# bjkomer/pyratslam

Hardware: AMD Instinct MI355X
Metric: pose-cell steps/sec (64×64×36) + template-compares/sec at 1/2/4/8 GPU (higher is better)
Workload: dtype u8; 1 GPU; configs[1]: 64x64x36 pose-cell grid + 1000 stored 64x32 u8 templates per GPU; a step matches 10 batches of 1024 queries resident in HBM; templates_per_gpu=1000, templates_total=1000, queries_per_batch=1024, parallelism=library sharded over 1 GPU(s), none; pose cells replicated

## Files before the change

### include/ratslam_abi.h

```cpp
#ifndef RATSLAM_ABI_H
#define RATSLAM_ABI_H

#include <stddef.h>
#include <stdint.h>

#ifdef __cplusplus
extern "C" {
#endif

#define RS_OK           0
#define RS_ERR_ARG      1
#define RS_ERR_TYPE     2
#define RS_ERR_LUT_KEY  3
#define RS_ERR_HIP      4
#define RS_ERR_RCCL     5
#define RS_ERR_STATE    6
#define RS_ERR_NOMEM    7
#define RS_ERR_CTL_RANGE 8

#define RS_PREC_F32 0
#define RS_PREC_F64 1

#define RS_FILTER_LEN 7

int rs_version(void);
const char* rs_last_error(void);
int rs_device_count(void);
int rs_dev_malloc(int device, size_t bytes, void** ptr);
int rs_dev_free(void* ptr);
int rs_dev_copy(void* dst, const void* src, size_t bytes);
int rs_host_alloc(size_t bytes, void** ptr);
int rs_host_free(void* ptr);

typedef struct rs_pc rs_pc;

typedef struct rs_pc_params {
    int precision;
    double global_inhibition;
    double ge[RS_FILTER_LEN];
    double gi[RS_FILTER_LEN];
    double k_scale;
    int nfilters;
    const double* xy_filters;
} rs_pc_params;


int rs_pc_create(int X, int Y, int TH, const rs_pc_params* params, int device, rs_pc** out);
int rs_pc_destroy(rs_pc* h);
int rs_pc_shape(const rs_pc* h, int* X, int* Y, int* TH);

int rs_pc_update(rs_pc* h, const int32_t* ox, const int32_t* oy, const int32_t* fidx,
                 const double* zf, int32_t out_xyz[3]);
int rs_pc_run(rs_pc* h, int n, const int32_t* ox, const int32_t* oy, const int32_t* fidx,
              const double* zf, int32_t* out_xyz);
int rs_pc_set_odometry_tables(rs_pc* h, double vtrans_scale, double vrot_scale,
                              const double* cos_a, const double* sin_a, int key_min,
                              int nkeys, const int32_t* key_rows, int zorig_min, int nz,
                              const double* zf_table);
int rs_pc_update_odom(rs_pc* h, double vtrans, double vrot, int32_t out_xyz[3]);
int rs_pc_odom_control(int TH, double vtrans_scale, double vrot_scale, const double* cos_a,
                       const double* sin_a, int key_min, int nkeys, const int32_t* key_rows,
                       int zorig_min, int nz, const double* zf_table, int n, const double* odom,
                       int32_t* ox, int32_t* oy, int32_t* fidx, double* zf, int32_t* status);
int rs_pc_run_odom(rs_pc* h, int n, const double* odom, int32_t* out_xyz, int* first_bad);
int rs_pc_update_odom_read(rs_pc* h, double vtrans, double vrot, int32_t out_xyz[3], double* pinned_xyth);
int rs_pc_excite(rs_pc* h);
int rs_pc_inject(rs_pc* h, double energy, int x, int y, int th);
int rs_pc_get_max(rs_pc* h, int32_t out_xyz[3]);
int rs_pc_set_peak_tables(rs_pc* h, int r, const double* sc_x, const double* sc_y, const double* sc_th);
int rs_pc_get_peak(rs_pc* h, int32_t xyz[3], double sums[6]);
int rs_pc_update_odom_peak(rs_pc* h, double vtrans, double vrot, int32_t out_xyz[3], double sums[6]);
int rs_pc_run_odom_peaks(rs_pc* h, int n, const double* odom, int32_t* out_xyz, double* out_sums,
                         int* first_bad);
int rs_pc_run_peaks(rs_pc* h, int n, const int32_t* ox, const int32_t* oy, const int32_t* fidx,
                    const double* zf, int32_t* out_xyz, double* out_sums);
int rs_pc_peak_host(int X, int Y, int TH, int r, const double* volume_xyth, const int32_t xyz[3],
                    const double* sc_x, const double* sc_y, const double* sc_th, double sums[6]);
#define RS_PC_INJ_AT_PEAK (-1)
#define RS_PC_INJ_SAME_AS (-2)
int rs_pc_run_odom_inject(rs_pc* h, int n, const double* odom, int ni, const int32_t* inj_step,
                          const double* inj_energy, const int32_t* inj_loc, int32_t* out_xyz,
                          int32_t* out_inj_xyz, double* out_sums, int* first_bad);
int rs_pc_run_inject(rs_pc* h, int n, const int32_t* ox, const int32_t* oy, const int32_t* fidx,
                     const double* zf, int ni, const int32_t* inj_step, const double* inj_energy,
                     const int32_t* inj_loc, int32_t* out_xyz, int32_t* out_inj_xyz, double* out_sums);
int rs_pc_read(rs_pc* h, double* host_xyth);
int rs_pc_read_pinned(rs_pc* h, double* pinned_xyth);
int rs_pc_write(rs_pc* h, const double* host_xyth);
int rs_pc_total(rs_pc* h, double* total);
int rs_pc_last_ms(rs_pc* h, double* ms);
int rs_pc_set_profiling(rs_pc* h, int enable);
int rs_pc_kernel_ms(rs_pc* h, double ms[2]);
const char* rs_pc_step_form(const rs_pc* h);
#define RS_PC_DBG_POISON      1
#define RS_PC_DBG_SKIP_EXPORT 2
#define RS_PC_DBG_HALO_SETTLE 3
#define RS_PC_DBG_HALO_AMBIG  4
int rs_pc_debug(rs_pc* h, int op);
int rs_pc_debug_value(rs_pc* h, int op, int64_t* value);

typedef struct rs_vt rs_vt;

int rs_vt_create(int H, int W, int max_offset, uint64_t match_threshold, int64_t capacity,
                 int device, rs_vt** out);
#define RS_VT_METRIC_WRAPPED 0
#define RS_VT_METRIC_SAD     1
int rs_vt_create_metric(int H, int W, int max_offset, uint64_t match_threshold, int64_t capacity,
                        int device, int metric, rs_vt** out);
int rs_vt_metric(const rs_vt* h, int* metric);
int rs_vt_destroy(rs_vt* h);
int rs_vt_count(const rs_vt* h, int64_t* count);
int rs_vt_add(rs_vt* h, int n, const uint8_t* templates, int64_t* first_index);
int rs_vt_read(rs_vt* h, int64_t index, uint8_t* out);

#define RS_VT_FROZEN     0
#define RS_VT_SEQUENTIAL 1

int rs_vt_match_batch(rs_vt* h, int nq, const uint8_t* queries, int mode,
                      uint64_t* best_score, int64_t* best_index, uint8_t* is_new);
int rs_vt_match_stream(rs_vt* h, int nb, int nq, const uint8_t* queries, uint64_t* best_score,
                       int64_t* best_index);
int rs_vt_match(rs_vt* h, const uint8_t* query, uint64_t* best_score, int64_t* best_index,
                int* is_new);
int rs_vt_set_subsample(rs_vt* h, int64_t frame_bytes, const int32_t* pixels);
int rs_vt_match_frames(rs_vt* h, int nf, const uint8_t* frames, int mode, uint64_t* best_score,
                       int64_t* best_index, uint8_t* is_new);
int rs_vt_scores(rs_vt* h, int nq, const uint8_t* queries, int64_t t0, int64_t nt,
                 uint64_t* scores);
int rs_vt_offset_profile(rs_vt* h, int nq, const uint8_t* queries, const int64_t* index,
                         uint32_t* profile, int32_t* offset);
int rs_vt_offset_profile_host(int metric, int H, int W, int max_offset, const uint8_t* tpl,
                              const uint8_t* query, uint32_t* profile, int32_t* offset);
int rs_vt_set_normalise(rs_vt* h, int radius, int gain);
int rs_vt_normalise(const rs_vt* h, int* radius, int* gain);
int rs_vt_normalise_host(int H, int W, int radius, int gain, const uint8_t* src, uint8_t* dst);
int rs_vt_scan_local(rs_vt* h, int nq, const uint8_t* queries, uint64_t* local_keys);
int rs_vt_resolve(rs_vt* h, int nq, const uint64_t* global_keys, int mode, uint64_t* best_score,
                  int64_t* best_index, uint8_t* is_new);
int rs_vt_last_ms(rs_vt* h, double* ms);
int rs_vt_set_timing(rs_vt* h, int enable);
const char* rs_vt_scan_form(const rs_vt* h);
int rs_vt_prune_stats(rs_vt* h, int64_t out[4]);
int rs_vt_prune_verified(rs_vt* h, int64_t* out);

int rs_vt_set_threshold(rs_vt* h, double threshold);

#define RS_DT_F32 0
#define RS_DT_F64 1
int rs_sad_scores(int device, int dtype, int H, int W, int max_offset, int64_t nt,
                  const void* templates, int nq, const void* queries, void* scores);

typedef struct rs_vtf rs_vtf;

int rs_vtf_create(int H, int W, int max_offset, int dtype, int64_t capacity, int device,
                  rs_vtf** out);
int rs_vtf_destroy(rs_vtf* h);
int rs_vtf_count(const rs_vtf* h, int64_t* count);
int rs_vtf_add(rs_vtf* h, int n, const void* templates, int64_t* first_index);
int rs_vtf_read(rs_vtf* h, int64_t index, void* out);
int rs_vtf_scores(rs_vtf* h, int nq, const void* queries, int64_t t0, int64_t nt, void* scores);
int rs_vtf_scan(rs_vtf* h, int nq, const void* queries, int want_inbatch, void* best_score,
                int64_t* best_index, void* inbatch);
int rs_vtf_append_staged(rs_vtf* h, int n, const int32_t* which, int64_t* first_index);
int rs_vtf_set_timing(rs_vtf* h, int enable);
int rs_vtf_last_ms(rs_vtf* h, double* ms);
int rs_sad_plan_sum(int dtype, int64_t n, const void* values, void* out);

typedef struct rs_vo rs_vo;

typedef struct rs_vo_params {
    int trans_y0, trans_y1, trans_x0, trans_x1;
    int rot_y0, rot_y1, rot_x0, rot_x1;
    int max_shift;
    double rad_per_column;
    double vtrans_scale;
    double vtrans_max;
} rs_vo_params;

int rs_vo_create(int im_h, int im_w, const rs_vo_params* params, int device, rs_vo** out);
int rs_vo_destroy(rs_vo* h);
int rs_vo_reset(rs_vo* h);
int rs_vo_run(rs_vo* h, int nf, const uint8_t* frames, double* deltas, uint32_t* tables,
              uint32_t* profiles);
int rs_vo_select(int max_shift, int width, int rows, const uint32_t* table, int* shift,
                 double* mindiff);
int rs_vo_set_timing(rs_vo* h, int enable);
int rs_vo_last_ms(rs_vo* h, double ms[2]);

typedef struct rs_em rs_em;

int rs_em_create(int capacity, double correction, int device, rs_em** out);
int rs_em_destroy(rs_em* h);
int rs_em_count(rs_em* h, int* nexp, int* nlinks);
int rs_em_add_experience(rs_em* h, int from, double d, double heading, double facing, int* id);
int rs_em_add_link(rs_em* h, int from, int to, double d, double heading, double facing, int* id);
int rs_em_relax(rs_em* h, int loops);
int rs_em_read(rs_em* h, int first, int n, double* xyth);
int rs_em_write(rs_em* h, int first, int n, const double* xyth);
int rs_em_set_timing(rs_em* h, int enable);
int rs_em_last_ms(rs_em* h, double* ms);
const char* rs_em_form(rs_em* h);
int rs_em_relax_host(int nexp, int nlinks, const int32_t* from, const int32_t* to, const double* d,
                     const double* heading, const double* facing, double* xyth, int loops,
                     double correction);

#define RS_UNIQUE_ID_BYTES 128
int rs_comm_unique_id(uint8_t id[RS_UNIQUE_ID_BYTES]);
int rs_vt_attach_comm(rs_vt* h, int rank, int nranks, const uint8_t id[RS_UNIQUE_ID_BYTES]);
int rs_vt_set_shard(rs_vt* h, int rank, int nranks);
int rs_vt_rank(const rs_vt* h, int* rank, int* nranks);

#ifdef __cplusplus
}
#endif
#endif
```

### pyratslam_amd/_lib.py

```python
import ctypes
import os
import threading

import numpy as np

HERE = os.path.dirname(os.path.abspath(__file__))
LIB_PATH = os.path.join(HERE, 'libratslam_hip.so')

RS_OK = 0
RS_ERR_ARG = 1
RS_ERR_TYPE = 2
RS_ERR_LUT_KEY = 3
RS_ERR_HIP = 4
RS_ERR_RCCL = 5
RS_ERR_STATE = 6
RS_ERR_NOMEM = 7
RS_ERR_CTL_RANGE = 8
RS_PREC_F32 = 0
RS_PREC_F64 = 1
RS_PC_DBG_POISON = 1
RS_PC_DBG_SKIP_EXPORT = 2
RS_PC_DBG_HALO_SETTLE = 3
RS_PC_DBG_HALO_AMBIG = 4
RS_PC_INJ_AT_PEAK = -1
RS_PC_INJ_SAME_AS = -2
RS_VT_FROZEN = 0
RS_VT_SEQUENTIAL = 1
RS_VT_METRIC_WRAPPED = 0
RS_VT_METRIC_SAD = 1
RS_UNIQUE_ID_BYTES = 128
RS_DT_F32 = 0
RS_DT_F64 = 1
FILTER_LEN = 7

_c_int_p = ctypes.POINTER(ctypes.c_int)
_i32p = ctypes.POINTER(ctypes.c_int32)
_i64p = ctypes.POINTER(ctypes.c_int64)
_u64p = ctypes.POINTER(ctypes.c_uint64)
_u32p = ctypes.POINTER(ctypes.c_uint32)
_u8p = ctypes.POINTER(ctypes.c_uint8)
_f64p = ctypes.POINTER(ctypes.c_double)
_vp = ctypes.c_void_p


class PcParams(ctypes.Structure):
    _fields_ = [
        ('precision', ctypes.c_int),
        ('global_inhibition', ctypes.c_double),
        ('ge', ctypes.c_double * FILTER_LEN),
        ('gi', ctypes.c_double * FILTER_LEN),
        ('k_scale', ctypes.c_double),
        ('nfilters', ctypes.c_int),
        ('xy_filters', _f64p),
    ]


class VoParams(ctypes.Structure):
    _fields_ = [(r + '_' + b, ctypes.c_int) for r in ('trans', 'rot') for b in ('y0', 'y1', 'x0', 'x1')] + [
        ('max_shift', ctypes.c_int),
        ('rad_per_column', ctypes.c_double),
        ('vtrans_scale', ctypes.c_double),
        ('vtrans_max', ctypes.c_double),
    ]


SIGNATURES = {
    'rs_version': (ctypes.c_int, []),
    'rs_last_error': (ctypes.c_char_p, []),
    'rs_device_count': (ctypes.c_int, []),
    'rs_dev_malloc': (ctypes.c_int, [ctypes.c_int, ctypes.c_size_t, ctypes.POINTER(_vp)]),
    'rs_dev_free': (ctypes.c_int, [_vp]),
    'rs_dev_copy': (ctypes.c_int, [_vp, _vp, ctypes.c_size_t]),
    'rs_host_alloc': (ctypes.c_int, [ctypes.c_size_t, ctypes.POINTER(_vp)]),
    'rs_host_free': (ctypes.c_int, [_vp]),
    'rs_pc_create': (ctypes.c_int, [ctypes.c_int, ctypes.c_int, ctypes.c_int,
                                    ctypes.POINTER(PcParams), ctypes.c_int, ctypes.POINTER(_vp)]),
    'rs_pc_destroy': (ctypes.c_int, [_vp]),
    'rs_pc_shape': (ctypes.c_int, [_vp, _c_int_p, _c_int_p, _c_int_p]),
    'rs_pc_update': (ctypes.c_int, [_vp, _i32p, _i32p, _i32p, _f64p, _i32p]),
    'rs_pc_run': (ctypes.c_int, [_vp, ctypes.c_int, _i32p, _i32p, _i32p, _f64p, _i32p]),
    'rs_pc_set_odometry_tables': (ctypes.c_int, [_vp, ctypes.c_double, ctypes.c_double, _f64p, _f64p,
                                                 ctypes.c_int, ctypes.c_int, _i32p, ctypes.c_int,
                                                 ctypes.c_int, _f64p]),
    'rs_pc_update_odom': (ctypes.c_int, [_vp, ctypes.c_double, ctypes.c_double, _i32p]),
    'rs_pc_odom_control': (ctypes.c_int, [ctypes.c_int, ctypes.c_double, ctypes.c_double, _f64p,
                                          _f64p, ctypes.c_int, ctypes.c_int, _i32p, ctypes.c_int,
                                          ctypes.c_int, _f64p, ctypes.c_int, _f64p, _i32p, _i32p,
                                          _i32p, _f64p, _i32p]),
    'rs_pc_run_odom': (ctypes.c_int, [_vp, ctypes.c_int, _f64p, _i32p, _c_int_p]),
    'rs_pc_excite': (ctypes.c_int, [_vp]),
    'rs_pc_inject': (ctypes.c_int, [_vp, ctypes.c_double, ctypes.c_int, ctypes.c_int, ctypes.c_int]),
    'rs_pc_get_max': (ctypes.c_int, [_vp, _i32p]),
    'rs_pc_set_peak_tables': (ctypes.c_int, [_vp, ctypes.c_int, _f64p, _f64p, _f64p]),
    'rs_pc_get_peak': (ctypes.c_int, [_vp, _i32p, _f64p]),
    'rs_pc_update_odom_peak': (ctypes.c_int, [_vp, ctypes.c_double, ctypes.c_double, _i32p, _f64p]),
    'rs_pc_run_odom_peaks': (ctypes.c_int, [_vp, ctypes.c_int, _f64p, _i32p, _f64p, _c_int_p]),
    'rs_pc_run_peaks': (ctypes.c_int, [_vp, ctypes.c_int, _i32p, _i32p, _i32p, _f64p, _i32p, _f64p]),
    'rs_pc_run_odom_inject': (ctypes.c_int, [_vp, ctypes.c_int, _f64p, ctypes.c_int, _i32p, _f64p, _i32p, _i32p,
                                             _i32p, _f64p, _c_int_p]),
    'rs_pc_run_inject': (ctypes.c_int, [_vp, ctypes.c_int, _i32p, _i32p, _i32p, _f64p, ctypes.c_int, _i32p, _f64p,
                                        _i32p, _i32p, _i32p, _f64p]),
    'rs_pc_peak_host': (ctypes.c_int, [ctypes.c_int, ctypes.c_int, ctypes.c_int, ctypes.c_int, _f64p, _i32p,
                                       _f64p, _f64p, _f64p, _f64p]),
    'rs_pc_read': (ctypes.c_int, [_vp, _f64p]),
    'rs_pc_read_pinned': (ctypes.c_int, [_vp, _vp]),
    'rs_pc_update_odom_read': (ctypes.c_int, [_vp, ctypes.c_double, ctypes.c_double, _i32p, _vp]),
    'rs_pc_write': (ctypes.c_int, [_vp, _f64p]),
    'rs_pc_total': (ctypes.c_int, [_vp, _f64p]),
    'rs_pc_last_ms': (ctypes.c_int, [_vp, _f64p]),
    'rs_pc_set_profiling': (ctypes.c_int, [_vp, ctypes.c_int]),
    'rs_pc_kernel_ms': (ctypes.c_int, [_vp, _f64p]),
    'rs_pc_step_form': (ctypes.c_char_p, [_vp]),
    'rs_pc_debug': (ctypes.c_int, [_vp, ctypes.c_int]),
    'rs_pc_debug_value': (ctypes.c_int, [_vp, ctypes.c_int, ctypes.POINTER(ctypes.c_int64)]),
    'rs_vt_create': (ctypes.c_int, [ctypes.c_int, ctypes.c_int, ctypes.c_int, ctypes.c_uint64,
                                    ctypes.c_int64, ctypes.c_int, ctypes.POINTER(_vp)]),
    'rs_vt_create_metric': (ctypes.c_int, [ctypes.c_int, ctypes.c_int, ctypes.c_int, ctypes.c_uint64,
                                           ctypes.c_int64, ctypes.c_int, ctypes.c_int, ctypes.POINTER(_vp)]),
    'rs_vt_metric': (ctypes.c_int, [_vp, _c_int_p]),
    'rs_vt_destroy': (ctypes.c_int, [_vp]),
    'rs_vt_count': (ctypes.c_int, [_vp, _i64p]),
    'rs_vt_add': (ctypes.c_int, [_vp, ctypes.c_int, _u8p, _i64p]),
    'rs_vt_read': (ctypes.c_int, [_vp, ctypes.c_int64, _u8p]),
    'rs_vt_match_batch': (ctypes.c_int, [_vp, ctypes.c_int, _u8p, ctypes.c_int, _u64p, _i64p, _u8p]),
    'rs_vt_match_stream': (ctypes.c_int, [_vp, ctypes.c_int, ctypes.c_int, _vp, _u64p, _i64p]),
    'rs_vt_match': (ctypes.c_int, [_vp, _u8p, _u64p, _i64p, _c_int_p]),
    'rs_vt_scores': (ctypes.c_int, [_vp, ctypes.c_int, _u8p, ctypes.c_int64, ctypes.c_int64, _u64p]),
    'rs_vt_offset_profile': (ctypes.c_int, [_vp, ctypes.c_int, _vp, _i64p, _u32p, _i32p]),
    'rs_vt_offset_profile_host': (ctypes.c_int, [ctypes.c_int, ctypes.c_int, ctypes.c_int, ctypes.c_int, _u8p, _u8p,
                                                 _u32p, _i32p]),
    'rs_vt_set_normalise': (ctypes.c_int, [_vp, ctypes.c_int, ctypes.c_int]),
    'rs_vt_normalise': (ctypes.c_int, [_vp, _c_int_p, _c_int_p]),
    'rs_vt_normalise_host': (ctypes.c_int, [ctypes.c_int, ctypes.c_int, ctypes.c_int, ctypes.c_int, _u8p, _u8p]),
    'rs_vt_set_subsample': (ctypes.c_int, [_vp, ctypes.c_int64, _i32p]),
    'rs_vt_match_frames': (ctypes.c_int, [_vp, ctypes.c_int, _vp, ctypes.c_int, _u64p, _i64p, _u8p]),
    'rs_vt_scan_local': (ctypes.c_int, [_vp, ctypes.c_int, _u8p, _u64p]),
    'rs_vt_resolve': (ctypes.c_int, [_vp, ctypes.c_int, _u64p, ctypes.c_int, _u64p, _i64p, _u8p]),
    'rs_vt_last_ms': (ctypes.c_int, [_vp, _f64p]),
    'rs_vt_set_timing': (ctypes.c_int, [_vp, ctypes.c_int]),
    'rs_vt_scan_form': (ctypes.c_char_p, [_vp]),
    'rs_vt_prune_stats': (ctypes.c_int, [_vp, _i64p]),
    'rs_vt_prune_verified': (ctypes.c_int, [_vp, _i64p]),
    'rs_vt_set_threshold': (ctypes.c_int, [_vp, ctypes.c_double]),
    'rs_sad_scores': (ctypes.c_int, [ctypes.c_int, ctypes.c_int, ctypes.c_int, ctypes.c_int,
                                     ctypes.c_int, ctypes.c_int64, _vp, ctypes.c_int, _vp, _vp]),
    'rs_vtf_create': (ctypes.c_int, [ctypes.c_int, ctypes.c_int, ctypes.c_int, ctypes.c_int,
                                     ctypes.c_int64, ctypes.c_int, ctypes.POINTER(_vp)]),
    'rs_vtf_destroy': (ctypes.c_int, [_vp]),
    'rs_vtf_count': (ctypes.c_int, [_vp, _i64p]),
    'rs_vtf_add': (ctypes.c_int, [_vp, ctypes.c_int, _vp, _i64p]),
    'rs_vtf_read': (ctypes.c_int, [_vp, ctypes.c_int64, _vp]),
    'rs_vtf_scores': (ctypes.c_int, [_vp, ctypes.c_int, _vp, ctypes.c_int64, ctypes.c_int64, _vp]),
    'rs_vtf_scan': (ctypes.c_int, [_vp, ctypes.c_int, _vp, ctypes.c_int, _vp, _i64p, _vp]),
    'rs_vtf_append_staged': (ctypes.c_int, [_vp, ctypes.c_int, _i32p, _i64p]),
    'rs_vtf_set_timing': (ctypes.c_int, [_vp, ctypes.c_int]),
    'rs_vtf_last_ms': (ctypes.c_int, [_vp, _f64p]),
    'rs_sad_plan_sum': (ctypes.c_int, [ctypes.c_int, ctypes.c_int64, _vp, _vp]),
    'rs_vo_create': (ctypes.c_int, [ctypes.c_int, ctypes.c_int, ctypes.POINTER(VoParams), ctypes.c_int,
                                    ctypes.POINTER(_vp)]),
    'rs_vo_destroy': (ctypes.c_int, [_vp]),
    'rs_vo_reset': (ctypes.c_int, [_vp]),
    'rs_vo_run': (ctypes.c_int, [_vp, ctypes.c_int, _vp, _f64p, _u32p, _u32p]),
    'rs_vo_select': (ctypes.c_int, [ctypes.c_int, ctypes.c_int, ctypes.c_int, _u32p, _c_int_p, _f64p]),
    'rs_vo_set_timing': (ctypes.c_int, [_vp, ctypes.c_int]),
    'rs_vo_last_ms': (ctypes.c_int, [_vp, _f64p]),
    'rs_em_create': (ctypes.c_int, [ctypes.c_int, ctypes.c_double, ctypes.c_int, ctypes.POINTER(_vp)]),
    'rs_em_destroy': (ctypes.c_int, [_vp]),
    'rs_em_count': (ctypes.c_int, [_vp, _c_int_p, _c_int_p]),
    'rs_em_add_experience': (ctypes.c_int, [_vp, ctypes.c_int, ctypes.c_double, ctypes.c_double,
                                            ctypes.c_double, _c_int_p]),
    'rs_em_add_link': (ctypes.c_int, [_vp, ctypes.c_int, ctypes.c_int, ctypes.c_double, ctypes.c_double,
                                      ctypes.c_double, _c_int_p]),
    'rs_em_relax': (ctypes.c_int, [_vp, ctypes.c_int]),
    'rs_em_read': (ctypes.c_int, [_vp, ctypes.c_int, ctypes.c_int, _f64p]),
    'rs_em_write': (ctypes.c_int, [_vp, ctypes.c_int, ctypes.c_int, _f64p]),
    'rs_em_set_timing': (ctypes.c_int, [_vp, ctypes.c_int]),
    'rs_em_last_ms': (ctypes.c_int, [_vp, _f64p]),
    'rs_em_form': (ctypes.c_char_p, [_vp]),
    'rs_em_relax_host': (ctypes.c_int, [ctypes.c_int, ctypes.c_int, _i32p, _i32p, _f64p, _f64p, _f64p,
                                        _f64p, ctypes.c_int, ctypes.c_double]),
    'rs_comm_unique_id': (ctypes.c_int, [_u8p]),
    'rs_vt_attach_comm': (ctypes.c_int, [_vp, ctypes.c_int, ctypes.c_int, _u8p]),
    'rs_vt_set_shard': (ctypes.c_int, [_vp, ctypes.c_int, ctypes.c_int]),
    'rs_vt_rank': (ctypes.c_int, [_vp, _c_int_p, _c_int_p]),
}

NEWER_SYMBOLS = {'rs_vt_prune_stats', 'rs_vt_prune_verified', 'rs_vt_create_metric', 'rs_vt_metric',
                 'rs_vt_offset_profile', 'rs_vt_offset_profile_host', 'rs_vt_set_normalise',
                 'rs_vt_normalise', 'rs_vt_normalise_host'}

_lib = None
_lock = threading.Lock()


class HipLibraryError(RuntimeError):
    """The HIP library is missing, failed to load, or reported a runtime error."""


def load(path=LIB_PATH):
    global _lib
    with _lock:
        if _lib is not None:
            return _lib
        if not os.path.exists(path):
            raise HipLibraryError(
                f'{path} not found: build it with `python -m pyratslam_amd._build` '
                '(there is no CPU fallback)')
        lib = ctypes.CDLL(path)
        for name, (res, args) in SIGNATURES.items():
            if name in NEWER_SYMBOLS and not hasattr(lib, name):
                continue
            fn = getattr(lib, name)
            fn.restype = res
            fn.argtypes = args
        _lib = lib
        return lib


def check(status):
    if status == RS_OK:
        return
    msg = (_lib.rs_last_error() or b'').decode(errors='replace') if _lib else ''
    if status == RS_ERR_ARG:
        raise ValueError(msg)
    if status == RS_ERR_TYPE:
        raise TypeError(msg)
    if status == RS_ERR_LUT_KEY:
        raise KeyError(msg)
    if status == RS_ERR_NOMEM:
        raise MemoryError(msg)
    raise HipLibraryError(f'rs status {status}: {msg}')


def require_device():
    lib = load()
    n = lib.rs_device_count()
    if n <= 0:
        raise HipLibraryError('no HIP device visible: the pyratslam_amd hot path runs only on '
                              'an AMD GPU (gfx950); there is no CPU fallback')
    return lib


def ptr(a, ctype):
    if a is None:
        return None
    return a.ctypes.data_as(ctypes.POINTER(ctype))


def as_c(a, dtype):
    return np.ascontiguousarray(a, dtype=dtype)


class DeviceBuffer:

    def __init__(self, nbytes, device=0):
        self._lib = require_device()
        p = ctypes.c_void_p()
        check(self._lib.rs_dev_malloc(int(device), int(nbytes), ctypes.byref(p)))
        self.ptr, self.nbytes = p, int(nbytes)

    def upload(self, array):
        import numpy as np
        a = np.ascontiguousarray(array)
        if a.nbytes > self.nbytes:
            raise ValueError('%d bytes do not fit a %d-byte buffer' % (a.nbytes, self.nbytes))
        check(self._lib.rs_dev_copy(self.ptr, ctypes.c_void_p(a.ctypes.data), a.nbytes))
        return self

    def offset(self, byte_offset):
        if not 0 <= byte_offset <= self.nbytes:
            raise ValueError('offset %d outside the %d-byte buffer' % (byte_offset, self.nbytes))
        return DeviceView(self, int(byte_offset))

    def close(self):
        if getattr(self, 'ptr', None) is not None and self.ptr.value:
            self._lib.rs_dev_free(self.ptr)
        self.ptr = None

    def __del__(self):
        try:
            self.close()
        except Exception:
            pass


class DeviceView:

    def __init__(self, base, byte_offset):
        self._base = base
        self.ptr = ctypes.c_void_p(base.ptr.value + byte_offset)
        self.nbytes = base.nbytes - byte_offset
```

### pyratslam_amd/csrc/view_templates.hip

```cpp
#include <hip/hip_runtime.h>
#include <rccl/rccl.h>

#include <algorithm>
#include <climits>
#include <cstdint>
#include <cstdio>
#include <cstdlib>
#include <cstring>
#include <memory>
#include <vector>

#include "rs_common.h"
#include "vt_norm_rule.h"
#include "vt_offset_rule.h"
#include "vt_plan.h"

namespace {

#include "vt_device.h"
#include "vt_store.h"
#include "vt_carry.h"

static_assert(vt_plan::METRIC_WRAPPED == RS_VT_METRIC_WRAPPED && vt_plan::METRIC_SAD == RS_VT_METRIC_SAD,
              "vt_plan.h restates the ABI's metric codes");
#include "vt_sad.h"
static_assert(rs::VTO_METRIC_WRAPPED == RS_VT_METRIC_WRAPPED && rs::VTO_METRIC_SAD == RS_VT_METRIC_SAD,
              "vt_offset_rule.h restates the ABI's metric codes");
#include "vt_offset.h"
#include "vt_norm.h"

#include "vt_planes.h"
#include "vt_plane_scan.h"
#include "vt_prune.h"

}

struct QueryForms {
    uint32_t *qp = nullptr, *qsum = nullptr, *qsj = nullptr, *qc = nullptr;
};

struct rs_vt {
    int H = 0, W = 0, M = 0, WD = 0, HQ = 0;
    double thr = 0.0;
    int device = 0;
    int rank = 0, nranks = 1;
    ncclComm_t comm = nullptr;
    int64_t count = 0;
    int64_t localCap = 0;
    rs::DevBuf<uint4> dLib;
    hipStream_t stream = nullptr;
    int qCap = 0;
    rs::DevBuf<uint8_t> dQraw;
    rs::PinnedBuf<uint8_t> hQraw;
    bool qrawBusy = false;
    rs::DevBuf<uint2> dQf;
    rs::DevBuf<uint32_t> dQsum;
    rs::DevBuf<unsigned long long> dBest;
    rs::PinnedBuf<unsigned long long> hBest;
    bool stagingBusy = false;
    hipStream_t cstream = nullptr;
    hipEvent_t evScan = nullptr, evComm = nullptr;
    hipStream_t ustream = nullptr;
    hipEvent_t evUp[2] = {nullptr, nullptr}, evUsed[2] = {nullptr, nullptr};
    rs::DevBuf<uint8_t> dUp[2];
    size_t upCap = 0;
    rs::DevBuf<uint32_t> dQpStream;
    rs::DevBuf<uint32_t> dQsumStream;
    size_t qpStreamCap = 0;
    rs::DevBuf<unsigned long long> dStream;
    rs::PinnedBuf<unsigned long long> hStream;
    size_t streamCap = 0;
    bool streamClean = false;
    int bestClean = 0;
    int bestPending = 0;
    int idxCap = 0;
    rs::DevBuf<int32_t> dSrc;
    rs::DevBuf<int64_t> dDst;
    rs::PinnedBuf<int32_t> hSrc;
    rs::PinnedBuf<int64_t> hDst;
    int64_t candCap = 0;
    rs::DevBuf<uint4> dCand;
    size_t matCap = 0;
    rs::DevBuf<uint32_t> dMat;
    rs::PinnedBuf<uint32_t> hMat;
    hipEvent_t ev0 = nullptr, ev1 = nullptr;
    bool timing = false;
    bool timedScan = false;
    float lastMs = 0.f;
    int stagedQ = 0;
    bool planar = false;
    int metric = RS_VT_METRIC_WRAPPED;
    rs::DevBuf<uint32_t> dLibP, dLibTs, dCandP, dCandTs;
    rs::DevBuf<uint32_t> dQp, dQsumRaw;
    int planeSlots = 0;
    rs::DevBuf<unsigned> dCtr;
    rs::DevBuf<unsigned> dDone;
    bool keysFolded = false;
    int prune = 0;
    int front = 1;
    int listNb = VT_LIST_NB;
    rs::DevBuf<uint32_t> dQsj;
    rs::DevBuf<uint32_t> dQsjStream;
    rs::DevBuf<uint32_t> dQc;
    rs::DevBuf<uint32_t> dQcStream;
    bool qpFull = true;
    bool qcValid = false;
    rs::DevBuf<uint32_t> dMinLB;
    rs::DevBuf<uint32_t> dSecond;
    rs::DevBuf<int> dList;
    size_t pruneCap = 0;
    rs::DevBuf<int> dTbStar;
    rs::DevBuf<unsigned> dListCnt;
    int listCntCap = 0;
    rs::DevBuf<unsigned long long> dPruneStat;
    int64_t prunePairs = 0;
    int prunePasses = 0;
    int pruneNtb = 0;
    rs::DevBuf<int32_t> dPix;
    int64_t frameBytes = 0;
    rs::DevBuf<uint8_t> dFrames;
    rs::PinnedBuf<uint8_t> hFrames;
    int frameCap = 0;
    rs::DevBuf<uint8_t> dOffQ;
    rs::PinnedBuf<int64_t> hOffIdx;
    rs::PinnedBuf<uint32_t> hOffProfile;
    rs::PinnedBuf<int32_t> hOffOffset;
    int radius = 0, gain = 0;
    rs::DevBuf<uint8_t> dNormRaw;
    rs::DevBuf<uint8_t> dNormStream;
    rs::DevBuf<uint8_t> dOffRaw;
};

namespace {

size_t tblock_bytes(const rs_vt* h) { return (size_t)h->WD * h->HQ * 64 * 16; }
size_t pblock_bytes(const rs_vt* h) { return (size_t)PL_CG * (h->H / 4) * 128 * 16; }
constexpr size_t TS_BLOCK_BYTES = 16 * 64 * sizeof(uint32_t);
int plane_ns(const rs_vt* h) { return h->H - 2 * h->M + 3; }

template <class T>
int vt_realloc_blocks(rs_vt* h, rs::DevBuf<T>& buf, int64_t keep, int64_t blocks, size_t bb,
                      const char* what = "template buffer growth") {
    rs::DevBuf<T> nb;
    const size_t bytes = (size_t)blocks * bb;
    RS_TRY(nb.reserve(bytes / sizeof(T), what));
    RS_HIP(hipMemsetAsync(nb.get(), 0, bytes, h->stream));
    if (buf.get()) {
        if (keep > 0)
            RS_HIP(hipMemcpyAsync(nb.get(), buf.get(), (size_t)keep * bb, hipMemcpyDeviceToDevice, h->stream));
        RS_HIP(hipStreamSynchronize(h->stream));
    }
    buf = std::move(nb);
    return RS_OK;
}

int64_t local_count_of(const rs_vt* h, int64_t global_count) {
    return vt_plan::local_count_of(h->rank, h->nranks, global_count);
}

int vt_grow_lib(rs_vt* h, int64_t need_slots) {
    if (need_slots <= h->localCap) return RS_OK;
    const int64_t cap = (int64_t)rs::round_up((size_t)rs::grown<int64_t>(h->localCap, need_slots, 64), 64);
    RS_TRY(vt_realloc_blocks(h, h->dLib, h->localCap / 64, cap / 64, tblock_bytes(h), "template library growth"));
    if (h->planar) {
        RS_TRY(vt_realloc_blocks(h, h->dLibP, h->localCap / 64, cap / 64, pblock_bytes(h)));
        RS_TRY(vt_realloc_blocks(h, h->dLibTs, h->localCap / 64, cap / 64, TS_BLOCK_BYTES));
    }
    h->localCap = cap;
    return RS_OK;
}

int vt_qraw_idle(rs_vt* h) {
    if (h->qrawBusy) {
        RS_HIP(hipStreamSynchronize(h->stream));
        h->qrawBusy = false;
    }
    return RS_OK;
}

constexpr unsigned VT_FINE = hipHostMallocMapped | hipHostMallocCoherent;

int vt_grow_queries(rs_vt* h, int nq) {
    if (nq <= h->qCap) return RS_OK;
    const int cap = rs::grown(h->qCap, nq, 64);
    RS_TRY(vt_qraw_idle(h));
    h->qCap = 0;
    h->bestClean = h->bestPending = 0;
    const size_t qb = (size_t)h->H * h->W, n = (size_t)cap;
    if (h->planar) {
        RS_TRY(h->dQp.reserve((size_t)PL_CG * plane_ns(h) * 8 * n));
        RS_TRY(h->dQsumRaw.reserve(n));
        if (h->prune) RS_TRY(h->dQsj.reserve((size_t)PF_NU * 16 * n));
        if (h->prune) RS_TRY(h->dQc.reserve((size_t)QC_Q4 * 4 * n));
    }
    RS_TRY(h->dQraw.reserve(qb * n));
    if (h->radius > 0) RS_TRY(h->dNormRaw.reserve(qb * n));
    RS_TRY(h->hQraw.reserve(qb * n, VT_FINE));
    RS_TRY(h->dQf.reserve((size_t)h->WD * h->H * n));
    RS_TRY(h->dQsum.reserve(n));
    RS_TRY(h->dBest.reserve(n));
    RS_TRY(h->hBest.reserve(n, VT_FINE));
    h->qCap = cap;
    return RS_OK;
}

int vt_grow_index(rs_vt* h, int n) {
    if (n <= h->idxCap) return RS_OK;
    const int cap = rs::grown(h->idxCap, n, 64);
    h->idxCap = 0;
    RS_TRY(h->dSrc.reserve((size_t)cap));
    RS_TRY(h->dDst.reserve((size_t)cap));
    RS_TRY(h->hSrc.reserve((size_t)cap, hipHostMallocDefault));
    RS_TRY(h->hDst.reserve((size_t)cap, hipHostMallocDefault));
    h->idxCap = cap;
    return RS_OK;
}

int vt_grow_matrix(rs_vt* h, size_t elems) {
    if (elems <= h->matCap) return RS_OK;
    const size_t cap = rs::grown<size_t>(h->matCap, elems, 4096);
    h->matCap = 0;
    RS_TRY(h->dMat.reserve(cap));
    RS_TRY(h->hMat.reserve(cap, hipHostMallocDefault));
    h->matCap = cap;
    return RS_OK;
}

int vt_grow_cand(rs_vt* h, int64_t slots) {
    if (slots <= h->candCap) return RS_OK;
    const int64_t cap = rs::grown<int64_t>(h->candCap, slots, 64);
    h->candCap = 0;
    RS_TRY(h->dCand.reserve((size_t)(cap / 64) * tblock_bytes(h) / sizeof(uint4)));
    if (h->planar) {
        RS_TRY(vt_realloc_blocks(h, h->dCandP, 0, cap / 64, pblock_bytes(h)));
        RS_TRY(vt_realloc_blocks(h, h->dCandTs, 0, cap / 64, TS_BLOCK_BYTES));
    }
    h->candCap = cap;
    return RS_OK;
}

QueryForms vt_batch_view(const rs_vt* h) {
    return {h->dQp.get(), h->dQsumRaw.get(), h->dQsj.get(), h->dQc.get()};
}

QueryForms vt_stream_view(const rs_vt* h, size_t q0) {
    const size_t qpq = (size_t)PL_CG * plane_ns(h) * 8;
    QueryForms v{h->dQpStream.get() + qpq * q0, h->dQsumStream.get() + q0, nullptr, nullptr};
    if (h->dQsjStream.get()) v.qsj = h->dQsjStream.get() + (size_t)PF_NU * 16 * q0;
    if (h->dQcStream.get()) v.qc = h->dQcStream.get() + (size_t)QC_Q4 * 4 * q0;
    return v;
}

int vt_build_forms(rs_vt* h, const QueryForms& q, int nq);

bool vt_prunes(const rs_vt* h, const QueryForms& q, bool cand, int64_t tb0, int64_t count, int nq) {
    return vt_plan::prunes(h->H, cand, tb0, q.qsj && q.qc, (count + 63) / 64, h->prune, nq);
}
constexpr int VT_QC_THREADS = 128;
uint32_t* vt_compact_for(rs_vt* h, const QueryForms& q, int nq) {
    const int64_t lc = local_count_of(h, h->count);
    const bool compact = h->planar && lc > 0 && vt_prunes(h, q, false, 0, lc, nq);
    h->qpFull = !compact;
    h->qcValid = compact;
    return compact ? q.qc : nullptr;
}

int vt_normalise(rs_vt* h, const uint8_t* src, uint8_t* dst, size_t n) {
    const int tx = (h->W + VTN_T - 1) / VTN_T, ty = (h->H + VTN_T - 1) / VTN_T;
    hipLaunchKernelGGL(vt_normalise_kernel, dim3((unsigned)(tx * ty), (unsigned)std::min<size_t>(n, 65535)),
                       dim3(VTN_THREADS), 0, h->stream, src, dst, (int)n, h->H, h->W, h->radius, h->gain, tx);
    RS_HIP(hipGetLastError());
    return RS_OK;
}

bool vt_zc_env() { static const bool on = rs::env_on("RS_VT_ZC"); return on; }

int vt_stage_queries(rs_vt* h, int nq, const uint8_t* queries) {
    RS_TRY(vt_grow_queries(h, nq));
    RS_TRY(vt_qraw_idle(h));
    const QueryForms q = vt_batch_view(h);
    const size_t qb = (size_t)h->H * h->W * nq;
    if (h->radius > 0) {
        RS_HIP(hipMemcpyAsync(h->dNormRaw.get(), queries, qb, hipMemcpyHostToDevice, h->stream));
        RS_TRY(vt_normalise(h, h->dNormRaw.get(), h->dQraw.get(), (size_t)nq));
        return vt_build_forms(h, q, nq);
    }
    if (vt_plan::stages_in_place(h->planar, nq, vt_zc_env())) {
        std::memcpy(h->hQraw.get(), queries, qb);
        h->qrawBusy = true;
        uint32_t* const qc = vt_compact_for(h, q, nq);
        hipLaunchKernelGGL(vt_qplane_kernel, dim3(nq), dim3(qc ? VT_QC_THREADS : 256), 0, h->stream, h->hQraw.dev(), h->H,
                           h->M, q.qp, q.qsum, h->dQraw.get(), q.qsj, qc);
        RS_HIP(hipGetLastError());
        return RS_OK;
    }
    RS_HIP(hipMemcpyAsync(h->dQraw.get(), queries, qb, hipMemcpyHostToDevice, h->stream));
    return vt_build_forms(h, q, nq);
}

int vt_build_forms(rs_vt* h, const QueryForms& q, int nq, const uint8_t* src) {
    if (h->metric == RS_VT_METRIC_SAD)
        hipLaunchKernelGGL(vt_qform_sad_kernel, dim3(nq), dim3(256), 0, h->stream, src, h->H, h->W, h->WD,
                           reinterpret_cast<uint32_t*>(h->dQf.get()));
    else if (!h->planar)
        hipLaunchKernelGGL(vt_qform_kernel, dim3(nq), dim3(256), 0, h->stream, src, h->H, h->W,
                           h->WD, h->M, h->dQf.get(), h->dQsum.get());
    else {
        uint32_t* const qc = vt_compact_for(h, q, nq);
        hipLaunchKernelGGL(vt_qplane_kernel, dim3(nq), dim3(qc ? VT_QC_THREADS : 256), 0, h->stream, src, h->H,
                           h->M, q.qp, q.qsum, nullptr, q.qsj, qc);
    }
    RS_HIP(hipGetLastError());
    return RS_OK;
}

int vt_build_forms(rs_vt* h, const QueryForms& q, int nq) { return vt_build_forms(h, q, nq, h->dQraw.get()); }

int vt_stage_frames(rs_vt* h, int nf, const uint8_t* frames) {
    RS_CHECK(h->dPix.get(), RS_ERR_STATE, "no subsampling mask: call rs_vt_set_subsample first");
    RS_TRY(vt_grow_queries(h, nf));
    const bool on_device = rs::on_device(frames);
    const uint8_t* src = frames;
    if (!on_device) {
        if (nf > h->frameCap) {
            const int cap = rs::grown(h->frameCap, nf, 16);
            h->frameCap = 0;
            RS_TRY(h->dFrames.reserve((size_t)h->frameBytes * cap));
            RS_TRY(h->hFrames.reserve((size_t)h->frameBytes * cap, hipHostMallocDefault));
            h->frameCap = cap;
        }
        const size_t fb = (size_t)h->frameBytes * nf;
        std::memcpy(h->hFrames.get(), frames, fb);
        RS_HIP(hipMemcpyAsync(h->dFrames.get(), h->hFrames.get(), fb, hipMemcpyHostToDevice, h->stream));
        src = h->dFrames.get();
    }
    hipLaunchKernelGGL(vt_gather_kernel, dim3(nf), dim3(256), 0, h->stream, src,
                       (size_t)h->frameBytes, h->dPix.get(), h->H * h->W,
                       h->radius > 0 ? h->dNormRaw.get() : h->dQraw.get());
    RS_HIP(hipGetLastError());
    if (h->radius > 0) RS_TRY(vt_normalise(h, h->dNormRaw.get(), h->dQraw.get(), (size_t)nf));
    return vt_build_forms(h, vt_batch_view(h), nf);
}

int vt_store(rs_vt* h, bool cand, const uint8_t* d_raw, int n) {
    if (n == 0) return RS_OK;
    uint4* lib = cand ? h->dCand.get() : h->dLib.get();
    RS_HIP(hipMemcpyAsync(h->dSrc.get(), h->hSrc.get(), sizeof(int32_t) * n, hipMemcpyHostToDevice, h->stream));
    RS_HIP(hipMemcpyAsync(h->dDst.get(), h->hDst.get(), sizeof(int64_t) * n, hipMemcpyHostToDevice, h->stream));
    h->stagingBusy = true;
    const int64_t total = (int64_t)n * h->WD * h->HQ;
    const int grid = (int)std::min<int64_t>((total + 255) / 256, 4096);
    hipLaunchKernelGGL(vt_store_kernel, dim3(grid), dim3(256), 0, h->stream, d_raw, h->dSrc.get(),
                       h->dDst.get(), n, lib, h->H, h->W, h->WD, h->HQ);
    if (h->planar)
        hipLaunchKernelGGL(vt_plane_store_kernel, dim3(n), dim3(256), 0, h->stream, d_raw, h->dSrc.get(),
                           h->dDst.get(), h->H, h->M, cand ? h->dCandP.get() : h->dLibP.get(),
                           cand ? h->dCandTs.get() : h->dLibTs.get());
    RS_HIP(hipGetLastError());
    return RS_OK;
}

template <class F>
__attribute__((always_inline)) inline auto vt_by_h(const rs_vt* h, F&& f) {
    return h->H == 64 ? f(rs::Int<64>{}) : f(rs::Int<32>{});
}

int vt_nqc_env() {
    const char* e = std::getenv("RS_VT_NQC");
    return e ? std::max(1, std::atoi(e)) : 0;
}

int vt_env_switch(const char* name, int* out) {
    const char* e = std::getenv(name);
    if (!e || e[0] == 0 || std::strcmp(e, "1") == 0) *out = 1;
    else if (std::strcmp(e, "force") == 0) *out = 2;
    else {
        RS_CHECK(std::strcmp(e, "0") == 0, RS_ERR_ARG, "%s='%s': expected 0, 1 or force", name, e);
        *out = 0;
    }
    return RS_OK;
}

void vt_launch_keys_export(rs_vt* h, unsigned long long* keys, int n, unsigned long long* host, int max_blocks) {
    hipLaunchKernelGGL(vt_keys_export, dim3((unsigned)vt_plan::export_grid(n, max_blocks)), dim3(256), 0, h->stream,
                       keys, n, host);
}

struct PlaneScan {
    dim3 grid;
    const uint4* planes;
    const uint32_t* ts;
    int ntb;
    int64_t count;
    const QueryForms& q;
    int nq, nqc, rank, nranks;
};
template <int H, bool MATRIX, bool LIST>
void vt_launch_plane_scan(rs_vt* h, const PlaneScan& s, const ScanOut& out, const PlaneList& list) {
    hipLaunchKernelGGL((vt_scan_plane_kernel<H, MATRIX, LIST>), s.grid, dim3(64 * PL_CG * PL_SPLIT), 0, h->stream,
                       s.planes, s.ts, s.ntb, s.count, s.q.qp, s.q.qsum, s.nq, s.nqc, h->dCtr.get(), out, s.rank,
                       s.nranks, list);
}

int vt_ensure_prune_buffers(rs_vt* h, int ntb, int nq) {
    const size_t pairs = (size_t)ntb * nq;
    if (pairs > h->pruneCap) {
        const size_t cap = std::max(pairs, 2 * h->pruneCap);
        h->pruneCap = 0;
        RS_TRY(h->dMinLB.reserve(cap));
        RS_TRY(h->dSecond.reserve(cap));
        RS_TRY(h->dList.reserve(2 * cap));
        h->pruneCap = cap;
    }
    RS_TRY(h->dTbStar.reserve((size_t)nq));
    if (ntb > h->listCntCap) {
        const int cap = std::max(ntb, 2 * h->listCntCap);
        h->listCntCap = 0;
        RS_TRY(h->dListCnt.reserve(2 * (size_t)cap + 1));
        RS_HIP(hipMemsetAsync(h->dListCnt.get(), 0, sizeof(unsigned) * (2 * (size_t)cap + 1), h->stream));
        h->listCntCap = cap;
    }
    if (!h->dPruneStat.get()) {
        RS_TRY(h->dPruneStat.reserve(3));
        RS_HIP(hipMemsetAsync(h->dPruneStat.get(), 0, 3 * sizeof(unsigned long long), h->stream));
    }
    return RS_OK;
}

int vt_launch_pruned(rs_vt* h, const PlaneScan& s, const ScanOut& out) {
    const QueryForms& q = s.q;
    const int ntb = s.ntb, nq = s.nq;
    if (!h->qcValid) {
        hipLaunchKernelGGL(vt_qcompact_kernel, dim3((unsigned)nq), dim3(128), 0, h->stream,
                           reinterpret_cast<const uint4*>(q.qp), reinterpret_cast<uint4*>(q.qc));
        h->qcValid = true;
    }
    RS_TRY(vt_ensure_prune_buffers(h, ntb, nq));
    const size_t pairs = (size_t)ntb * nq;
    unsigned* cnt1 = h->dListCnt.get();
    unsigned* cnt2 = h->dListCnt.get() + h->listCntCap;
    unsigned* verified = h->dListCnt.get() + 2 * (size_t)h->listCntCap;
    int* list1 = h->dList.get();
    int* list2 = h->dList.get() + pairs;
    if (h->front == 2 || (h->front == 1 && vt_plan::front_fused(ntb, PF_WAVES * PF_TPW))) {
        const vt_plan::Grid2 fg = vt_plan::front_grid(nq, PF_NB, VT_PF_GRID_CAP);
        hipLaunchKernelGGL(vt_front_kernel, dim3((unsigned)fg.x, (unsigned)fg.y), dim3(64 * PF_WAVES), 0, h->stream,
                           s.planes, ntb, s.count, reinterpret_cast<const uint4*>(q.qc), q.qsj, nq, h->dMinLB.get(),
                           s.ts, reinterpret_cast<uint4*>(q.qp), q.qsum, out.best, s.rank, s.nranks,
                           h->dTbStar.get());
    } else {
        const vt_plan::Grid2 pf = vt_plan::prefilter_grid(ntb, nq, PF_WAVES * PF_TPW, PF_NB, VT_PF_GRID_CAP);
        hipLaunchKernelGGL(vt_prefilter_kernel, dim3((unsigned)pf.x, (unsigned)pf.y), dim3(64 * PF_WAVES), 0,
                           h->stream, s.planes, ntb, s.count, reinterpret_cast<const uint4*>(q.qc), q.qsj, nq,
                           h->dMinLB.get(), h->dSecond.get());
        hipLaunchKernelGGL(vt_prune_verify_kernel, dim3((unsigned)nq), dim3(64), 0, h->stream, h->dMinLB.get(),
                           h->dSecond.get(), ntb, nq, s.planes, s.ts, reinterpret_cast<const uint4*>(q.qc),
                           reinterpret_cast<uint4*>(q.qp), q.qsum, out.best, s.rank, s.nranks, h->dTbStar.get());
    }
    const dim3 lgrid((unsigned)((nq + VT_LIST_T - 1) / VT_LIST_T), (unsigned)ntb);
    hipLaunchKernelGGL(vt_prune_first_kernel, lgrid, dim3(VT_LIST_T), 0, h->stream, nq, h->dTbStar.get(), cnt1,
                       list1, verified, cnt2, ntb);
    ScanOut po = out;
    po.host = nullptr;
    po.done = nullptr;
    const uint32_t fill = (uint32_t)std::min(65535, std::max(1, h->planeSlots / ntb));
    const uint32_t lnb = (uint32_t)h->listNb;
    vt_launch_plane_scan<64, false, true>(h, s, po,
                                          PlaneList{list1, cnt1, nq, (uint32_t)VT_LIST_PER_B1, lnb, 1u, fill});
    hipLaunchKernelGGL(vt_prune_rest_kernel, lgrid, dim3(VT_LIST_T), 0, h->stream, h->dMinLB.get(), nq,
                       h->dTbStar.get(), out.best, cnt2, list2, cnt1, verified, ntb, h->dPruneStat.get());
#ifdef VT_LIST_PER
    const int per2 = VT_LIST_PER;
#else
    const int per2 = vt_plan::list_per(ntb, h->planeSlots);
#endif
    vt_launch_plane_scan<64, false, true>(h, s, po, PlaneList{list2, cnt2, nq, (uint32_t)per2, lnb, 0u, fill});
    if (out.host) vt_launch_keys_export(h, out.best, nq, out.host, vt_plan::VT_EXPORT_BLOCKS);
    RS_HIP(hipGetLastError());
    h->prunePairs = (int64_t)pairs;
    h->prunePasses = 2;
    h->pruneNtb = ntb;
    return RS_OK;
}

template <bool MATRIX>
int vt_launch_plane(rs_vt* h, const QueryForms& q, bool cand, int64_t count, int nq, ScanOut out, int rank,
                    int nranks, int64_t tb0) {
    const int ntb = (int)((count + 63) / 64);
    const int nqc = vt_plan::plane_split(ntb, (nq + PL_NB - 1) / PL_NB, h->planeSlots, vt_nqc_env());
    if (8 * (size_t)ntb > h->dCtr.capacity()) {
        const size_t cap = std::max(8 * (size_t)ntb, 2 * h->dCtr.capacity());
        RS_TRY(h->dCtr.reserve(cap));
        RS_HIP(hipMemsetAsync(h->dCtr.get(), 0, sizeof(unsigned) * cap, h->stream));
    }
    RS_CHECK((int64_t)ntb * nqc < (1ll << 31), RS_ERR_ARG, "scan grid too large");
    const uint4* planes = reinterpret_cast<const uint4*>(
        reinterpret_cast<const uint8_t*>(cand ? h->dCandP.get() : h->dLibP.get()) + (size_t)tb0 * pblock_bytes(h));
    const uint32_t* ts = (cand ? h->dCandTs.get() : h->dLibTs.get()) + (size_t)tb0 * (TS_BLOCK_BYTES / 4);
    const PlaneScan s{dim3((unsigned)(ntb * nqc)), planes, ts, ntb, count, q, nq, nqc, rank, nranks};
    if constexpr (!MATRIX)
        if (vt_prunes(h, q, cand, tb0, count, nq)) return vt_launch_pruned(h, s, out);
    if (!h->qpFull) {
        hipLaunchKernelGGL(vt_qexpand_kernel, dim3((unsigned)nq), dim3(256), 0, h->stream,
                           reinterpret_cast<const uint4*>(q.qc), reinterpret_cast<uint4*>(q.qp));
        h->qpFull = true;
    }
    vt_by_h(h, [&](auto H) { vt_launch_plane_scan<decltype(H)::value, MATRIX, false>(h, s, out, PlaneList{}); });
    RS_HIP(hipGetLastError());
    return RS_OK;
}

template <bool MATRIX>
int vt_launch_sad(rs_vt* h, const uint4* lib, int ntb, int64_t count, int nq, ScanOut out, int rank, int nranks) {
    const uint32_t* qd = reinterpret_cast<const uint32_t*>(h->dQf.get());
    if (vt_plan::sad_fast(h->H, h->M)) {
        const int nqc = vt_plan::sad_split(ntb, (nq + SAD_NQ - 1) / SAD_NQ);
        RS_CHECK((int64_t)ntb * nqc < (1ll << 31), RS_ERR_ARG, "scan grid too large (%d x %d)", ntb, nqc);
        vt_by_h(h, [&](auto H) {
            hipLaunchKernelGGL((vt_scan_sad_kernel<decltype(H)::value, MATRIX>), dim3((unsigned)(ntb * nqc)),
                               dim3(64 * vt_plan::sad_waves(h->WD)), 0, h->stream, lib, ntb, count, h->WD, qd, nq,
                               nqc, out, rank, nranks);
        });
    } else {
        hipLaunchKernelGGL((vt_scan_sad_generic_kernel<MATRIX>), dim3((unsigned)(ntb * nq)), dim3(64), 0, h->stream,
                           lib, ntb, count, h->H, h->M, h->WD, qd, nq, out, rank, nranks);
    }
    RS_HIP(hipGetLastError());
    return RS_OK;
}

template <bool MATRIX>
int vt_launch_scan(rs_vt* h, const QueryForms& q, bool cand, int64_t count, int nq, ScanOut out, int rank,
                   int nranks, int64_t tb0 = 0) {
    if (count <= 0 || nq <= 0) return RS_OK;
    if (h->planar) return vt_launch_plane<MATRIX>(h, q, cand, count, nq, out, rank, nranks, tb0);
    const uint4* lib = (cand ? h->dCand.get() : h->dLib.get()) + (size_t)tb0 * h->WD * h->HQ * 64;
    const int ntb = (int)((count + 63) / 64);
    const bool fast = h->M == FAST_M && (h->H == 64 || h->H == 32);
    RS_CHECK((int64_t)ntb * nq < (1ll << 31), RS_ERR_ARG, "scan grid too large (%d x %d)", ntb, nq);
    if (h->metric == RS_VT_METRIC_SAD) return vt_launch_sad<MATRIX>(h, lib, ntb, count, nq, out, rank, nranks);
    if (fast && !MATRIX && (int64_t)ntb * nq < 2048 && h->WD <= 8) {
        const dim3 grid((unsigned)((count + 7) / 8), nq);
        vt_by_h(h, [&](auto H) {
            hipLaunchKernelGGL((vt_scan_carry_col_kernel<decltype(H)::value, 1>), grid, dim3(64), 0, h->stream, lib,
                               count, h->WD, h->dQf.get(), h->dQsum.get(), nq, out, rank, nranks);
        });
    } else if (fast) {
        constexpr int NQ = 2;
        const int nqg = (nq + NQ - 1) / NQ;
        const dim3 grid((unsigned)(ntb * ((nqg + 7) / 8) * 8));
        vt_by_h(h, [&](auto H) {
            hipLaunchKernelGGL((vt_scan_carry_kernel<decltype(H)::value, NQ, MATRIX>), grid, dim3(64), 0, h->stream,
                               lib, ntb, count, h->WD, h->dQf.get(), h->dQsum.get(), nq, out, rank, nranks);
        });
    } else {
        hipLaunchKernelGGL((vt_scan_generic_kernel<MATRIX>), dim3((unsigned)(ntb * nq)), dim3(64),
                           0, h->stream, lib, ntb, count, h->H, h->M, h->WD, h->dQf.get(), nq, out, rank,
                           nranks);
    }
    RS_HIP(hipGetLastError());
    return RS_OK;
}

constexpr unsigned long long KEY_PENDING = 0xFFFFFFFF00000000ull;
bool vt_poll_env() { static const bool on = rs::env_on("RS_VT_POLL"); return on; }
bool vt_poll_keys(const unsigned long long* w_, int n) {
    const volatile unsigned long long* w = w_;
    return rs::spin_until(n, [w](int i) { return w[i] != KEY_PENDING; });
}

int vt_staging_idle(rs_vt* h) {
    if (h->stagingBusy) {
        RS_HIP(hipStreamSynchronize(h->stream));
        h->stagingBusy = false;
    }
    return RS_OK;
}

int vt_allreduce_min(rs_vt* h, unsigned long long* buf, size_t n, hipStream_t stream) {
    ncclResult_t r = ncclAllReduce(buf, buf, n, ncclUint64, ncclMin, h->comm, stream);
    RS_CHECK(r == ncclSuccess, RS_ERR_RCCL, "ncclAllReduce(min) failed: %s", ncclGetErrorString(r));
    return RS_OK;
}

template <class Run>
int vt_timed_scan(rs_vt* h, bool timed, Run run) {
    if (timed) RS_HIP(hipEventRecord(h->ev0, h->stream));
    RS_TRY(run());
    if (timed) RS_HIP(hipEventRecord(h->ev1, h->stream));
    h->timedScan = timed;
    return RS_OK;
}

void vt_decode_keys(const unsigned long long* key, size_t n, uint64_t* best_score, int64_t* best_index) {
    for (size_t i = 0; i < n; ++i) {
        const unsigned long long k = key[i];
        if (best_index) best_index[i] = k == NO_KEY ? -1 : (int64_t)(k & 0xFFFFFFFFull);
        if (best_score) best_score[i] = k == NO_KEY ? UINT64_MAX : (k >> 32);
    }
}

int vt_append_staged(rs_vt* h, const std::vector<std::pair<int, int64_t>>& news) {
    int mine = 0;
    RS_TRY(vt_staging_idle(h));
    RS_TRY(vt_grow_index(h, (int)news.size() + 1));
    const int64_t new_count = h->count + (int64_t)news.size();
    RS_TRY(vt_grow_lib(h, local_count_of(h, new_count)));
    for (const auto& p : news) {
        if (p.second % h->nranks != h->rank) continue;
        h->hSrc.get()[mine] = p.first;
        h->hDst.get()[mine] = p.second / h->nranks;
        ++mine;
    }
    RS_TRY(vt_store(h, false, h->dQraw.get(), mine));
    h->count = new_count;
    return RS_OK;
}

int vt_scan_local_impl(rs_vt* h, int nq, const uint8_t* queries, bool frames = false, bool fold_ok = true) {
    RS_CHECK(h, RS_ERR_STATE, "null view-template handle");
    RS_CHECK(nq >= 0, RS_ERR_ARG, "negative query count");
    if (nq == 0) return RS_OK;
    RS_HIP(hipSetDevice(h->device));
    if (frames) {
        RS_CHECK(queries, RS_ERR_ARG, "null frames");
        RS_TRY(vt_stage_frames(h, nq, queries));
    } else if (queries) {
        RS_TRY(vt_stage_queries(h, nq, queries));
    } else {
        RS_CHECK(nq == h->stagedQ, RS_ERR_STATE, "no staged batch of %d queries (have %d)", nq,
                 h->stagedQ);
    }
    if (h->bestClean < nq) {
        RS_HIP(hipMemsetAsync(h->dBest.get(), 0xFF, sizeof(unsigned long long) * nq, h->stream));
        h->bestClean = nq;
    }
    h->bestPending = h->bestClean;
    h->bestClean = 0;
    const int64_t lc = local_count_of(h, h->count);
    ScanOut out{h->dBest.get(), nullptr, 0};
    h->keysFolded = vt_plan::folds_keys(fold_ok, h->planar, lc, vt_poll_env(), h->timing, nq);
    if (h->keysFolded) {
        if (!h->dDone.get()) {
            RS_TRY(h->dDone.reserve(1));
            RS_HIP(hipMemsetAsync(h->dDone.get(), 0, sizeof(unsigned), h->stream));
        }
        for (int i = 0; i < nq; ++i) h->hBest.get()[i] = KEY_PENDING;
        out.host = h->hBest.dev();
        out.done = h->dDone.get();
    }
    RS_TRY(vt_timed_scan(h, h->timing, [&] {
        return vt_launch_scan<false>(h, vt_batch_view(h), false, lc, nq, out, h->rank, h->nranks);
    }));
    h->stagedQ = nq;
    return RS_OK;
}

int vt_resolve_impl(rs_vt* h, int nq, const unsigned long long* keys, int mode,
                    uint64_t* best_score, int64_t* best_index, uint8_t* is_new) {
    RS_CHECK(h, RS_ERR_STATE, "null view-template handle");
    RS_CHECK(mode == RS_VT_FROZEN || mode == RS_VT_SEQUENTIAL, RS_ERR_ARG, "unknown mode %d", mode);
    RS_CHECK(nq == h->stagedQ, RS_ERR_STATE, "resolve of %d queries, %d staged", nq, h->stagedQ);
    if (nq == 0) return RS_OK;
    RS_CHECK(keys, RS_ERR_ARG, "null keys");
    RS_HIP(hipSetDevice(h->device));
    std::vector<unsigned long long> key(keys, keys + nq);
    if (mode == RS_VT_FROZEN) {
        if (is_new) std::memset(is_new, 0, (size_t)nq);
        vt_decode_keys(key.data(), (size_t)nq, best_score, best_index);
        return RS_OK;
    }
    std::vector<int> cand;
    for (int i = 0; i < nq; ++i)
        if (key[i] == NO_KEY || (double)(key[i] >> 32) > h->thr) cand.push_back(i);
    std::vector<int> cpos(nq, -1);
    int64_t ldm = 0;
    if (!cand.empty() && cand.front() < nq - 1) {
        RS_TRY(vt_staging_idle(h));
        const int64_t C = (int64_t)cand.size();
        RS_TRY(vt_grow_cand(h, (int64_t)rs::round_up((size_t)C, 64)));
        RS_TRY(vt_grow_index(h, (int)C));
        for (int64_t j = 0; j < C; ++j) {
            h->hSrc.get()[j] = cand[j];
            h->hDst.get()[j] = j;
            cpos[cand[j]] = (int)j;
        }
        RS_TRY(vt_store(h, true, h->dQraw.get(), (int)C));
        ldm = (int64_t)rs::round_up((size_t)C, 64);
        RS_TRY(vt_grow_matrix(h, (size_t)ldm * nq));
        ScanOut mo{nullptr, h->dMat.get(), ldm};
        RS_TRY(vt_launch_scan<true>(h, vt_batch_view(h), true, C, nq, mo, 0, 1));
        RS_HIP(hipMemcpyAsync(h->hMat.get(), h->dMat.get(), sizeof(uint32_t) * ldm * nq, hipMemcpyDeviceToHost,
                              h->stream));
        RS_HIP(hipStreamSynchronize(h->stream));
        h->stagingBusy = false;
    }
    std::vector<std::pair<int, int64_t>> news;
    for (int i = 0; i < nq; ++i) {
        unsigned long long k = key[i];
        for (size_t a = 0; a < news.size(); ++a) {
            const int j = news[a].first;
            const unsigned long long kj =
                ((unsigned long long)h->hMat.get()[(size_t)i * ldm + cpos[j]] << 32) |
                (unsigned long long)news[a].second;
            k = kj < k ? kj : k;
        }
        if (k == NO_KEY || (double)(k >> 32) > h->thr) {
            const int64_t g = h->count + (int64_t)news.size();
            news.emplace_back(i, g);
            if (is_new) is_new[i] = 1;
            if (best_index) best_index[i] = g;
        } else {
            if (is_new) is_new[i] = 0;
            if (best_index) best_index[i] = (int64_t)(k & 0xFFFFFFFFull);
        }
        if (best_score) best_score[i] = k == NO_KEY ? UINT64_MAX : (k >> 32);
    }
    RS_TRY(vt_append_staged(h, news));
    return RS_OK;
}

int vt_fetch_keys(rs_vt* h, int nq, bool allreduce) {
    if (allreduce && h->nranks > 1) {
        RS_CHECK(h->comm, RS_ERR_STATE, "sharded handle without a communicator: use "
                 "rs_vt_scan_local + an external min-reduction + rs_vt_resolve");
        RS_TRY(vt_allreduce_min(h, h->dBest.get(), (size_t)nq, h->stream));
    }
    const bool poll = vt_plan::polls_keys(vt_poll_env(), h->timedScan, nq);
    if (h->keysFolded) {
        h->keysFolded = false;
    } else {
        if (poll)
            for (int i = 0; i < nq; ++i) h->hBest.get()[i] = KEY_PENDING;
        vt_launch_keys_export(h, h->dBest.get(), nq, h->hBest.dev(), vt_plan::VT_EXPORT_BLOCKS);
        RS_HIP(hipGetLastError());
    }
    if (!(poll && vt_poll_keys(h->hBest.get(), nq))) {
        RS_HIP(hipStreamSynchronize(h->stream));
        h->stagingBusy = false;
    }
    h->qrawBusy = false;
    h->bestClean = h->bestPending;
    if (h->timedScan) RS_HIP(hipEventElapsedTime(&h->lastMs, h->ev0, h->ev1));
    return RS_OK;
}


int vt_grow_stream_forms(rs_vt* h, size_t total) {
    if (total <= h->qpStreamCap) return RS_OK;
    h->qpStreamCap = 0;
    RS_TRY(h->dQpStream.reserve((size_t)PL_CG * plane_ns(h) * 8 * total));
    RS_TRY(h->dQsumStream.reserve(total));
    if (h->prune) RS_TRY(h->dQsjStream.reserve((size_t)PF_NU * 16 * total));
    if (h->prune) RS_TRY(h->dQcStream.reserve((size_t)QC_Q4 * 4 * total));
    h->qpStreamCap = total;
    return RS_OK;
}

int vt_stream_fused(rs_vt* h, size_t total, const uint8_t* queries, int64_t lc) {
    RS_TRY(vt_grow_stream_forms(h, total));
    const QueryForms q = vt_stream_view(h, 0);
    if (h->radius > 0) {
        RS_TRY(h->dNormStream.reserve((size_t)h->H * h->W * total));
        RS_TRY(vt_normalise(h, queries, h->dNormStream.get(), total));
        queries = h->dNormStream.get();
    }
    RS_TRY(vt_build_forms(h, q, (int)total, queries));
    const ScanOut out{h->dStream.get(), nullptr, 0};
    RS_TRY(vt_timed_scan(h, h->timing, [&] {
        return vt_launch_scan<false>(h, q, false, lc, (int)total, out, h->rank, h->nranks);
    }));
    if (h->comm) RS_TRY(vt_allreduce_min(h, h->dStream.get(), total, h->stream));
    return RS_OK;
}

int vt_stream_host_groups(rs_vt* h, int nb, int nq, const uint8_t* queries, int64_t lc) {
    const size_t total = (size_t)nb * nq, qb = (size_t)h->H * h->W * nq;
    RS_TRY(vt_grow_stream_forms(h, total));
    const vt_plan::HostGroups plan = vt_plan::host_groups(nb);
    if (h->radius > 0) RS_TRY(h->dNormStream.reserve(qb * nb));
    if (!h->ustream) {
        RS_HIP(hipStreamCreateWithFlags(&h->ustream, hipStreamNonBlocking));
        for (int i = 0; i < 2; ++i) {
            RS_HIP(hipEventCreateWithFlags(&h->evUp[i], hipEventDisableTiming));
            RS_HIP(hipEventCreateWithFlags(&h->evUsed[i], hipEventDisableTiming));
        }
    }
    if (qb * plan.gb > h->upCap) {
        RS_HIP(hipStreamSynchronize(h->ustream));
        h->upCap = 0;
        for (int i = 0; i < 2; ++i) RS_TRY(h->dUp[i].reserve(qb * plan.gb));
        h->upCap = qb * plan.gb;
    }
    for (int g = 0;; ++g) {
        const vt_plan::HostGroup grp = plan.group(g);
        if (grp.n == 0) break;
        const int bi = grp.buf;
        if (grp.waits) RS_HIP(hipStreamWaitEvent(h->ustream, h->evUsed[bi], 0));
        RS_HIP(hipMemcpyAsync(h->dUp[bi].get(), queries + qb * grp.b0, qb * grp.n, hipMemcpyHostToDevice, h->ustream));
        RS_HIP(hipEventRecord(h->evUp[bi], h->ustream));
        RS_HIP(hipStreamWaitEvent(h->stream, h->evUp[bi], 0));
        const QueryForms q = vt_stream_view(h, (size_t)grp.b0 * nq);
        const uint8_t* src = h->dUp[bi].get();
        if (h->radius > 0) {
            uint8_t* const dn = h->dNormStream.get() + qb * grp.b0;
            RS_TRY(vt_normalise(h, src, dn, (size_t)grp.n * nq));
            src = dn;
        }
        RS_TRY(vt_build_forms(h, q, grp.n * nq, src));
        RS_HIP(hipEventRecord(h->evUsed[bi], h->stream));
        const ScanOut out{h->dStream.get() + (size_t)grp.b0 * nq, nullptr, 0};
        RS_TRY(vt_launch_scan<false>(h, q, false, lc, grp.n * nq, out, h->rank, h->nranks));
    }
    if (h->comm) RS_TRY(vt_allreduce_min(h, h->dStream.get(), total, h->stream));
    return RS_OK;
}

int vt_stream_per_batch(rs_vt* h, int nb, int nq, const uint8_t* queries, bool on_device, int64_t lc) {
    const size_t qb = (size_t)h->H * h->W * nq;
    for (int b = 0; b < nb; ++b) {
        unsigned long long* keys = h->dStream.get() + (size_t)b * nq;
        const ScanOut out{keys, nullptr, 0};
        const uint8_t* src = queries + qb * b;
        if (!on_device) {
            uint8_t* const up = h->radius > 0 ? h->dNormRaw.get() : h->dQraw.get();
            RS_HIP(hipMemcpyAsync(up, src, qb, hipMemcpyHostToDevice, h->stream));
            src = up;
        }
        if (h->radius > 0) {
            RS_TRY(vt_normalise(h, src, h->dQraw.get(), (size_t)nq));
            src = h->dQraw.get();
        }
        RS_TRY(vt_build_forms(h, vt_batch_view(h), nq, src));
        RS_TRY(vt_launch_scan<false>(h, vt_batch_view(h), false, lc, nq, out, h->rank, h->nranks));
        if (h->comm) {
            RS_HIP(hipEventRecord(h->evScan, h->stream));
            RS_HIP(hipStreamWaitEvent(h->cstream, h->evScan, 0));
            RS_TRY(vt_allreduce_min(h, keys, (size_t)nq, h->cstream));
        }
    }
    if (h->comm) {
        RS_HIP(hipEventRecord(h->evComm, h->cstream));
        RS_HIP(hipStreamWaitEvent(h->stream, h->evComm, 0));
    }
    return RS_OK;
}

int vt_match_stream_impl(rs_vt* h, int nb, int nq, const uint8_t* queries, uint64_t* best_score,
                         int64_t* best_index) {
    RS_CHECK(h, RS_ERR_STATE, "null view-template handle");
    RS_CHECK(nb >= 0 && nq >= 0, RS_ERR_ARG, "negative batch or query count");
    if (nb == 0 || nq == 0) return RS_OK;
    RS_CHECK(queries, RS_ERR_ARG, "null queries");
    RS_CHECK(h->nranks == 1 || h->comm, RS_ERR_STATE, "sharded handle without a communicator: "
             "rs_vt_match_stream needs the RCCL reduction (rs_vt_attach_comm)");
    if (h->comm && !h->cstream) {
        RS_HIP(hipStreamCreateWithFlags(&h->cstream, hipStreamNonBlocking));
        RS_HIP(hipEventCreateWithFlags(&h->evScan, hipEventDisableTiming));
        RS_HIP(hipEventCreateWithFlags(&h->evComm, hipEventDisableTiming));
    }
    RS_HIP(hipSetDevice(h->device));
    RS_TRY(vt_grow_queries(h, nq));
    const size_t total = (size_t)nb * nq;
    RS_CHECK(total <= INT32_MAX, RS_ERR_ARG, "too many queries in one stream");
    if (total > h->streamCap) {
        h->streamCap = 0;
        RS_TRY(h->hStream.reserve(total, hipHostMallocDefault));
        RS_TRY(h->dStream.reserve(total));
        h->streamCap = total;
        h->streamClean = false;
    }
    const bool on_device = rs::on_device(queries);
    RS_CHECK(!on_device || reinterpret_cast<uintptr_t>(queries) % 8 == 0, RS_ERR_ARG,
             "device-resident queries must be 8-byte aligned");
    if (!h->streamClean)
        RS_HIP(hipMemsetAsync(h->dStream.get(), 0xFF, sizeof(unsigned long long) * h->streamCap, h->stream));
    h->streamClean = false;
    h->stagedQ = 0;
    h->timedScan = false;
    const int64_t lc = local_count_of(h, h->count);
    switch (vt_plan::stream_path(on_device, h->planar, nb)) {
    case vt_plan::StreamPath::Fused: RS_TRY(vt_stream_fused(h, total, queries, lc)); break;
    case vt_plan::StreamPath::HostGroups: RS_TRY(vt_stream_host_groups(h, nb, nq, queries, lc)); break;
    case vt_plan::StreamPath::PerBatch: RS_TRY(vt_stream_per_batch(h, nb, nq, queries, on_device, lc)); break;
    }
    vt_launch_keys_export(h, h->dStream.get(), (int)total, h->hStream.dev(), vt_plan::VT_EXPORT_BLOCKS_STREAM);
    RS_HIP(hipGetLastError());
    RS_HIP(hipStreamSynchronize(h->stream));
    h->streamClean = true;
    if (h->timedScan) RS_HIP(hipEventElapsedTime(&h->lastMs, h->ev0, h->ev1));
    vt_decode_keys(h->hStream.get(), total, best_score, best_index);
    return RS_OK;
}

int vt_match_impl(rs_vt* h, int nq, const uint8_t* queries, int mode, uint64_t* best_score,
                  int64_t* best_index, uint8_t* is_new, bool frames = false) {
    RS_CHECK(mode == RS_VT_FROZEN || mode == RS_VT_SEQUENTIAL, RS_ERR_ARG, "unknown mode %d", mode);
    RS_TRY(vt_scan_local_impl(h, nq, queries, frames, h->nranks == 1));
    if (nq == 0) return RS_OK;
    RS_TRY(vt_fetch_keys(h, nq, true));
    return vt_resolve_impl(h, nq, h->hBest.get(), mode, best_score, best_index, is_new);
}

}

extern "C" {

int rs_vt_create(int H, int W, int max_offset, uint64_t thr, int64_t capacity, int device,
                 rs_vt** out) {
    return rs_vt_create_metric(H, W, max_offset, thr, capacity, device, RS_VT_METRIC_WRAPPED, out);
}

int rs_vt_create_metric(int H, int W, int max_offset, uint64_t thr, int64_t capacity, int device,
                        int metric, rs_vt** out) {
    rs::clear_error();
    RS_CHECK(out, RS_ERR_ARG, "null output handle pointer");
    *out = nullptr;
    RS_CHECK(vt_plan::metric_known(metric), RS_ERR_ARG, "unknown metric %d: expected RS_VT_METRIC_WRAPPED or "
             "RS_VT_METRIC_SAD", metric);
    RS_CHECK(H > 0 && W > 0 && H <= 4096 && W <= 4096, RS_ERR_ARG, "bad template shape (%d, %d)", H, W);
    RS_CHECK(max_offset >= 1 && max_offset <= 64, RS_ERR_ARG, "max_offset %d outside [1, 64]", max_offset);
    RS_CHECK(capacity >= 0, RS_ERR_ARG, "negative capacity");
    RS_CHECK((uint64_t)H * W * 255u < 0xFFFFFFFFull, RS_ERR_ARG, "template too large");
    int ndev = 0;
    RS_HIP(hipGetDeviceCount(&ndev));
    RS_CHECK(device >= 0 && device < ndev, RS_ERR_ARG, "device %d not in [0, %d)", device, ndev);
    RS_HIP(hipSetDevice(device));
    std::unique_ptr<rs_vt, int (*)(rs_vt*)> owner(new rs_vt(), rs_vt_destroy);
    rs_vt* const h = owner.get();
    h->H = H; h->W = W; h->M = max_offset; h->thr = (double)thr; h->device = device;
    h->WD = (W + 3) / 4;
    h->HQ = (H + 3) / 4;
    h->metric = metric;
    const bool wrapped = metric == RS_VT_METRIC_WRAPPED;
    h->planar = wrapped && W == 8 * PL_CG && (H == 64 || H == 32) && max_offset == FAST_M;
    if (const char* e = wrapped ? std::getenv("RS_VT_SCAN") : nullptr) {
        if (std::strcmp(e, "carry") == 0) h->planar = false;
        else RS_CHECK(std::strcmp(e, "plane") == 0 || e[0] == 0, RS_ERR_ARG, "RS_VT_SCAN='%s': expected plane or carry", e);
    }
    if (h->planar && h->H == 64) {
        RS_TRY(vt_env_switch("RS_VT_PRUNE", &h->prune));
        RS_TRY(vt_env_switch("RS_VT_FRONT", &h->front));
        if (const char* nb = std::getenv("RS_VT_LIST_NB"); nb && nb[0]) {
            RS_CHECK((nb[0] == '1' || nb[0] == '2' || nb[0] == '4') && nb[1] == 0, RS_ERR_ARG,
                     "RS_VT_LIST_NB='%s': expected 1, 2 or 4", nb);
            h->listNb = nb[0] - '0';
        }
    }
    if (h->planar) {
        int per_cu = 0, cus = 0;
        hipFuncAttributes fa{};
        const void* fn = vt_by_h(h, [](auto H) {
            return reinterpret_cast<const void*>(vt_scan_plane_kernel<decltype(H)::value, false>);
        });
        hipError_t oe = hipOccupancyMaxActiveBlocksPerMultiprocessor(&per_cu, fn, 64 * PL_CG * PL_SPLIT, 0);
        if (oe == hipSuccess) oe = hipFuncGetAttributes(&fa, fn);
        if (oe == hipSuccess) oe = hipDeviceGetAttribute(&cus, hipDeviceAttributeMultiprocessorCount, device);
        RS_CHECK(oe == hipSuccess, RS_ERR_HIP, "occupancy query failed: %s", hipGetErrorString(oe));
        const int vg = std::max(8, (fa.numRegs + 7) / 8 * 8);
        const int by_vgpr = (512 / vg) * 4 / (PL_CG * PL_SPLIT);
        const int by_lds = fa.sharedSizeBytes > 0 ? (int)(160 * 1024 / fa.sharedSizeBytes) : per_cu;
        const int api = per_cu;
        per_cu = std::max(1, std::min({api, by_vgpr, by_lds}));
        h->planeSlots = std::max(1, per_cu * cus);
    }
    hipError_t e = hipStreamCreateWithFlags(&h->stream, hipStreamNonBlocking);
    if (e == hipSuccess) e = hipEventCreate(&h->ev0);
    if (e == hipSuccess) e = hipEventCreate(&h->ev1);
    RS_CHECK(e == hipSuccess, RS_ERR_HIP, "stream/event creation failed: %s", hipGetErrorString(e));
    RS_TRY(vt_grow_lib(h, capacity > 0 ? capacity : 64));
    RS_TRY(vt_grow_queries(h, 64));
    RS_TRY(vt_grow_index(h, 64));
    *out = owner.release();
    return RS_OK;
}

int rs_vt_destroy(rs_vt* h) {
    if (!h) return RS_OK;
    (void)hipSetDevice(h->device);
    hipError_t se = hipSuccess;
    for (hipStream_t st : {h->stream, h->cstream, h->ustream})
        if (st) {
            const hipError_t e = hipStreamSynchronize(st);
            if (se == hipSuccess) se = e;
        }
    if (h->comm) (void)ncclCommDestroy(h->comm);
    if (h->ev0) (void)hipEventDestroy(h->ev0);
    if (h->ev1) (void)hipEventDestroy(h->ev1);
    if (h->evScan) (void)hipEventDestroy(h->evScan);
    if (h->evComm) (void)hipEventDestroy(h->evComm);
    if (h->cstream) (void)hipStreamDestroy(h->cstream);
    for (int i = 0; i < 2; ++i) {
        if (h->evUp[i]) (void)hipEventDestroy(h->evUp[i]);
        if (h->evUsed[i]) (void)hipEventDestroy(h->evUsed[i]);
    }
    if (h->ustream) (void)hipStreamDestroy(h->ustream);
    if (h->stream) (void)hipStreamDestroy(h->stream);
    delete h;
    RS_CHECK(se == hipSuccess, RS_ERR_HIP, "work queued before rs_vt_destroy failed: %s", hipGetErrorString(se));
    return RS_OK;
}

int rs_vt_count(const rs_vt* h, int64_t* count) {
    RS_CHECK(h && count, RS_ERR_ARG, "null argument");
    *count = h->count;
    return RS_OK;
}

int rs_vt_add(rs_vt* h, int n, const uint8_t* templates, int64_t* first_index) {
    rs::clear_error();
    RS_CHECK(h, RS_ERR_STATE, "null view-template handle");
    RS_CHECK(n >= 0 && (n == 0 || templates), RS_ERR_ARG, "bad template batch");
    RS_HIP(hipSetDevice(h->device));
    if (first_index) *first_index = h->count;
    if (n == 0) return RS_OK;
    RS_TRY(vt_grow_queries(h, n));
    const size_t qb = (size_t)h->H * h->W * n;
    hipPointerAttribute_t attr{};
    const bool direct_dma = hipPointerGetAttributes(&attr, templates) == hipSuccess &&
                            (attr.type == hipMemoryTypeHost || attr.type == hipMemoryTypeDevice ||
                             attr.type == hipMemoryTypeManaged);
    (void)hipGetLastError();
    RS_HIP(hipMemcpyAsync(h->radius > 0 ? h->dNormRaw.get() : h->dQraw.get(), templates, qb,
                          attr.type == hipMemoryTypeDevice && direct_dma ? hipMemcpyDeviceToDevice
                                                                         : hipMemcpyHostToDevice,
                          h->stream));
    int s = h->radius > 0 ? vt_normalise(h, h->dNormRaw.get(), h->dQraw.get(), (size_t)n) : RS_OK;
    h->stagedQ = 0;
    std::vector<std::pair<int, int64_t>> news;
    news.reserve(n);
    for (int i = 0; i < n; ++i) news.emplace_back(i, h->count + i);
    if (s == RS_OK) s = vt_append_staged(h, news);
    if (direct_dma) {
        const hipError_t e = hipStreamSynchronize(h->stream);
        RS_CHECK(s != RS_OK || e == hipSuccess, RS_ERR_HIP, "hipStreamSynchronize failed: %s", hipGetErrorString(e));
    }
    return s;
}

int rs_vt_read(rs_vt* h, int64_t index, uint8_t* out) {
    rs::clear_error();
    RS_CHECK(h && out, RS_ERR_ARG, "null argument");
    RS_CHECK(index >= 0 && index < h->count, RS_ERR_ARG, "template index %lld outside [0, %lld)",
             (long long)index, (long long)h->count);
    RS_CHECK(index % h->nranks == h->rank, RS_ERR_ARG, "template %lld lives on rank %lld",
             (long long)index, (long long)(index % h->nranks));
    RS_HIP(hipSetDevice(h->device));
    const int64_t slot = index / h->nranks;
    const int64_t tb = slot >> 6, tl = slot & 63;
    std::vector<uint4> chunks((size_t)h->WD * h->HQ);
    for (int c = 0; c < h->WD; ++c)
        for (int q = 0; q < h->HQ; ++q)
            RS_HIP(hipMemcpyAsync(&chunks[(size_t)c * h->HQ + q],
                                  h->dLib.get() + ((tb * h->WD + c) * h->HQ + q) * 64 + tl, sizeof(uint4),
                                  hipMemcpyDeviceToHost, h->stream));
    RS_HIP(hipStreamSynchronize(h->stream));
    for (int r = 0; r < h->H; ++r)
        for (int col = 0; col < h->W; ++col) {
            const uint4& ch = chunks[(size_t)(col / 4) * h->HQ + r / 4];
            const uint32_t w[4] = {ch.x, ch.y, ch.z, ch.w};
            out[(size_t)r * h->W + col] = (uint8_t)(w[r & 3] >> (8 * (col & 3)));
        }
    return RS_OK;
}

int rs_vt_match_batch(rs_vt* h, int nq, const uint8_t* queries, int mode, uint64_t* best_score,
                      int64_t* best_index, uint8_t* is_new) {
    rs::clear_error();
    return vt_match_impl(h, nq, queries, mode, best_score, best_index, is_new);
}

int rs_vt_match_stream(rs_vt* h, int nb, int nq, const uint8_t* queries, uint64_t* best_score,
                       int64_t* best_index) {
    rs::clear_error();
    return vt_match_stream_impl(h, nb, nq, queries, best_score, best_index);
}

int rs_vt_match(rs_vt* h, const uint8_t* query, uint64_t* best_score, int64_t* best_index,
                int* is_new) {
    rs::clear_error();
    uint8_t nw = 0;
    const int s = vt_match_impl(h, 1, query, RS_VT_SEQUENTIAL, best_score, best_index, &nw);
    if (is_new) *is_new = nw;
    return s;
}

int rs_vt_set_subsample(rs_vt* h, int64_t frame_bytes, const int32_t* pixels) {
    rs::clear_error();
    RS_CHECK(h && pixels, RS_ERR_ARG, "null argument");
    RS_CHECK(frame_bytes > 0 && frame_bytes <= INT32_MAX, RS_ERR_ARG, "bad frame size %lld",
             (long long)frame_bytes);
    const int npix = h->H * h->W;
    for (int i = 0; i < npix; ++i)
        RS_CHECK(pixels[i] >= 0 && pixels[i] < frame_bytes, RS_ERR_ARG,
                 "pixel offset %d of entry %d outside the %lld-byte frame", pixels[i], i,
                 (long long)frame_bytes);
    RS_HIP(hipSetDevice(h->device));
    RS_TRY(h->dPix.reserve((size_t)npix));
    RS_HIP(hipMemcpyAsync(h->dPix.get(), pixels, sizeof(int32_t) * npix, hipMemcpyHostToDevice, h->stream));
    RS_HIP(hipStreamSynchronize(h->stream));
    if (frame_bytes != h->frameBytes) {
        h->frameCap = 0;
        h->dFrames.reset();
        h->hFrames.reset();
    }
    h->frameBytes = frame_bytes;
    return RS_OK;
}

int rs_vt_match_frames(rs_vt* h, int nf, const uint8_t* frames, int mode, uint64_t* best_score,
                       int64_t* best_index, uint8_t* is_new) {
    rs::clear_error();
    RS_CHECK(h, RS_ERR_STATE, "null view-template handle");
    return vt_match_impl(h, nf, frames, mode, best_score, best_index, is_new, true);
}

int rs_vt_scan_local(rs_vt* h, int nq, const uint8_t* queries, uint64_t* local_keys) {
    rs::clear_error();
    RS_TRY(vt_scan_local_impl(h, nq, queries));
    if (nq == 0) return RS_OK;
    RS_TRY(vt_fetch_keys(h, nq, false));
    if (local_keys) std::memcpy(local_keys, h->hBest.get(), sizeof(uint64_t) * nq);
    return RS_OK;
}

int rs_vt_resolve(rs_vt* h, int nq, const uint64_t* global_keys, int mode, uint64_t* best_score,
                  int64_t* best_index, uint8_t* is_new) {
    rs::clear_error();
    static_assert(sizeof(uint64_t) == sizeof(unsigned long long), "key width");
    return vt_resolve_impl(h, nq, reinterpret_cast<const unsigned long long*>(global_keys), mode,
                           best_score, best_index, is_new);
}

int rs_vt_set_shard(rs_vt* h, int rank, int nranks) {
    rs::clear_error();
    RS_CHECK(h, RS_ERR_STATE, "null view-template handle");
    RS_CHECK(nranks >= 1 && rank >= 0 && rank < nranks, RS_ERR_ARG, "bad rank %d of %d", rank, nranks);
    RS_CHECK(h->count == 0 && h->comm == nullptr, RS_ERR_STATE,
             "set the shard before adding templates, once");
    h->rank = rank;
    h->nranks = nranks;
    return RS_OK;
}

int rs_vt_set_normalise(rs_vt* h, int radius, int gain) {
    rs::clear_error();
    RS_CHECK(h, RS_ERR_STATE, "null view-template handle");
    RS_CHECK(radius >= 0 && radius <= rs::VTN_MAX_RADIUS, RS_ERR_ARG, "radius %d outside [0, %d]", radius,
             rs::VTN_MAX_RADIUS);
    RS_CHECK(radius == 0 || (gain >= 1 && gain <= rs::VTN_MAX_GAIN), RS_ERR_ARG, "gain %d outside [1, %d]", gain,
             rs::VTN_MAX_GAIN);
    RS_CHECK(h->count == 0 && h->stagedQ == 0, RS_ERR_STATE,
             "set the normalisation before adding templates or staging a batch");
    RS_HIP(hipSetDevice(h->device));
    if (radius > 0) {
        RS_TRY(h->dNormRaw.reserve((size_t)h->H * h->W * h->qCap));
    } else {
        RS_HIP(hipStreamSynchronize(h->stream));
        h->dNormRaw.reset();
        h->dNormStream.reset();
        h->dOffRaw.reset();
    }
    h->radius = radius;
    h->gain = radius > 0 ? gain : 0;
    return RS_OK;
}

int rs_vt_normalise(const rs_vt* h, int* radius, int* gain) {
    RS_CHECK(h, RS_ERR_STATE, "null view-template handle");
    if (radius) *radius = h->radius;
    if (gain) *gain = h->gain;
    return RS_OK;
}

int rs_vt_normalise_host(int H, int W, int radius, int gain, const uint8_t* src, uint8_t* dst) {
    rs::clear_error();
    RS_CHECK(H > 0 && W > 0 && H <= 4096 && W <= 4096, RS_ERR_ARG, "bad image shape (%d, %d)", H, W);
    RS_CHECK(radius >= 1 && radius <= rs::VTN_MAX_RADIUS, RS_ERR_ARG, "radius %d outside [1, %d]", radius,
             rs::VTN_MAX_RADIUS);
    RS_CHECK(gain >= 1 && gain <= rs::VTN_MAX_GAIN, RS_ERR_ARG, "gain %d outside [1, %d]", gain, rs::VTN_MAX_GAIN);
    RS_CHECK(src && dst && src != dst, RS_ERR_ARG, "null or aliased image");
    rs::vtn_normalise_host(H, W, radius, gain, src, dst);
    return RS_OK;
}

int rs_vt_rank(const rs_vt* h, int* rank, int* nranks) {
    RS_CHECK(h, RS_ERR_STATE, "null view-template handle");
    if (rank) *rank = h->rank;
    if (nranks) *nranks = h->nranks;
    return RS_OK;
}

int rs_vt_scores(rs_vt* h, int nq, const uint8_t* queries, int64_t t0, int64_t nt,
                 uint64_t* scores) {
    rs::clear_error();
    RS_CHECK(h, RS_ERR_STATE, "null view-template handle");
    RS_CHECK(h->nranks == 1, RS_ERR_STATE, "rs_vt_scores needs an unsharded library");
    RS_CHECK(nq >= 0 && t0 >= 0 && nt >= 0 && t0 + nt <= h->count, RS_ERR_ARG,
             "template range [%lld, %lld) outside [0, %lld)", (long long)t0,
             (long long)(t0 + nt), (long long)h->count);
    if (nq == 0 || nt == 0) return RS_OK;
    RS_CHECK(queries && scores, RS_ERR_ARG, "null argument");
    RS_HIP(hipSetDevice(h->device));
    RS_TRY(vt_stage_queries(h, nq, queries));
    h->stagedQ = 0;
    const int64_t tb0 = t0 / 64, lo = t0 - tb0 * 64, span = lo + nt;
    const int64_t ld = (int64_t)rs::round_up((size_t)span, 64);
    RS_TRY(vt_grow_matrix(h, (size_t)ld * nq));
    ScanOut mo{nullptr, h->dMat.get(), ld};
    RS_TRY(vt_timed_scan(h, true, [&] {
        return vt_launch_scan<true>(h, vt_batch_view(h), false, span, nq, mo, 0, 1, tb0);
    }));
    RS_HIP(hipMemcpy2DAsync(h->hMat.get(), sizeof(uint32_t) * nt, h->dMat.get() + lo, sizeof(uint32_t) * ld,
                            sizeof(uint32_t) * nt, nq, hipMemcpyDeviceToHost, h->stream));
    RS_HIP(hipStreamSynchronize(h->stream));
    RS_HIP(hipEventElapsedTime(&h->lastMs, h->ev0, h->ev1));
    for (size_t i = 0; i < (size_t)nq * nt; ++i) scores[i] = h->hMat.get()[i];
    return RS_OK;
}

int rs_vt_offset_profile(rs_vt* h, int nq, const uint8_t* queries, const int64_t* index, uint32_t* profile,
                         int32_t* offset) {
    rs::clear_error();
    RS_CHECK(h, RS_ERR_STATE, "null view-template handle");
    RS_CHECK(h->nranks == 1, RS_ERR_STATE, "rs_vt_offset_profile needs an unsharded library");
    RS_CHECK(nq >= 0, RS_ERR_ARG, "negative query count");
    if (nq == 0) return RS_OK;
    RS_CHECK(index && offset, RS_ERR_ARG, "null argument");
    for (int i = 0; i < nq; ++i)
        RS_CHECK(index[i] >= -1 && index[i] < h->count, RS_ERR_ARG,
                 "template index %lld of query %d outside [-1, %lld)", (long long)index[i], i,
                 (long long)h->count);
    RS_CHECK(queries || nq == h->stagedQ, RS_ERR_STATE, "no staged batch of %d queries (have %d)", nq,
             h->stagedQ);
    RS_HIP(hipSetDevice(h->device));
    const size_t n = (size_t)nq, no = (size_t)(2 * h->M - 1), qb = (size_t)h->H * h->W * n;
    RS_TRY(h->hOffIdx.reserve(rs::grown<size_t>(h->hOffIdx.capacity(), n, 64), VT_FINE));
    RS_TRY(h->hOffProfile.reserve(rs::grown<size_t>(h->hOffProfile.capacity(), n * no, 64 * no), VT_FINE));
    RS_TRY(h->hOffOffset.reserve(rs::grown<size_t>(h->hOffOffset.capacity(), n, 64), VT_FINE));
    const uint8_t* src = h->dQraw.get();
    const size_t offq = rs::grown<size_t>(h->dOffQ.capacity(), qb, 64 * (size_t)h->H * h->W);
    if (queries && h->radius > 0) {
        RS_TRY(h->dOffQ.reserve(offq));
        const uint8_t* raw = queries;
        if (!rs::on_device(queries)) {
            RS_TRY(h->dOffRaw.reserve(h->dOffQ.capacity()));
            RS_HIP(hipMemcpyAsync(h->dOffRaw.get(), queries, qb, hipMemcpyHostToDevice, h->stream));
            raw = h->dOffRaw.get();
        }
        RS_TRY(vt_normalise(h, raw, h->dOffQ.get(), n));
        src = h->dOffQ.get();
    } else if (queries && rs::on_device(queries)) {
        src = queries;
    } else if (queries) {
        RS_TRY(h->dOffQ.reserve(offq));
        RS_HIP(hipMemcpyAsync(h->dOffQ.get(), queries, qb, hipMemcpyHostToDevice, h->stream));
        src = h->dOffQ.get();
    }
    std::memcpy(h->hOffIdx.get(), index, sizeof(int64_t) * n);
    const bool sad = h->metric == RS_VT_METRIC_SAD, fast = h->M == FAST_M;
    auto launch = [&](auto kernel) {
        hipLaunchKernelGGL(kernel, dim3(nq), dim3(64), 0, h->stream, h->dLib.get(), h->count, h->H, h->W,
                           h->WD, h->HQ, h->M, src, h->hOffIdx.dev(), h->hOffProfile.dev(),
                           h->hOffOffset.dev());
    };
    if (sad && fast) launch(vt_offset_profile_kernel<rs::VTO_METRIC_SAD, true>);
    else if (sad) launch(vt_offset_profile_kernel<rs::VTO_METRIC_SAD, false>);
    else if (fast) launch(vt_offset_profile_kernel<rs::VTO_METRIC_WRAPPED, true>);
    else launch(vt_offset_profile_kernel<rs::VTO_METRIC_WRAPPED, false>);
    RS_HIP(hipGetLastError());
    RS_HIP(hipStreamSynchronize(h->stream));
    h->stagingBusy = false;
    h->qrawBusy = false;
    if (profile) std::memcpy(profile, h->hOffProfile.get(), sizeof(uint32_t) * n * no);
    std::memcpy(offset, h->hOffOffset.get(), sizeof(int32_t) * n);
    return RS_OK;
}

int rs_vt_offset_profile_host(int metric, int H, int W, int max_offset, const uint8_t* tpl, const uint8_t* query,
                              uint32_t* profile, int32_t* offset) {
    rs::clear_error();
    RS_CHECK(vt_plan::metric_known(metric), RS_ERR_ARG, "unknown metric %d", metric);
    RS_CHECK(H > 0 && W > 0 && max_offset >= 1 && H >= 2 * max_offset, RS_ERR_ARG,
             "bad shape (%d, %d) for max_offset %d", H, W, max_offset);
    RS_CHECK((uint64_t)H * W * 255u < 0xFFFFFFFFull, RS_ERR_ARG, "template too large");
    RS_CHECK(tpl && query && profile && offset, RS_ERR_ARG, "null argument");
    *offset = rs::vto_profile_host(metric, H, W, max_offset, tpl, query, profile);
    return RS_OK;
}

int rs_vt_set_threshold(rs_vt* h, double threshold) {
    rs::clear_error();
    RS_CHECK(h, RS_ERR_STATE, "null view-template handle");
    h->thr = threshold;
    return RS_OK;
}

int rs_vt_metric(const rs_vt* h, int* metric) {
    RS_CHECK(h && metric, RS_ERR_ARG, "null argument");
    *metric = h->metric;
    return RS_OK;
}

const char* rs_vt_scan_form(const rs_vt* h) {
    if (!h) return nullptr;
    if (h->metric == RS_VT_METRIC_SAD) return vt_plan::sad_form(h->H, h->M);
    if (h->planar) return h->prune ? "plane-pruned" : "plane";
    if (h->M != FAST_M || (h->H != 64 && h->H != 32)) return "generic";
    return "carry";
}

int rs_vt_prune_stats(rs_vt* h, int64_t out[4]) {
    rs::clear_error();
    RS_CHECK(h && out, RS_ERR_ARG, "null argument");
    out[0] = out[1] = out[2] = out[3] = 0;
    if (h->prunePasses == 0) return RS_OK;
    RS_HIP(hipSetDevice(h->device));
    unsigned long long s0 = 0ull;
    std::vector<unsigned> c2((size_t)h->pruneNtb);
    RS_HIP(hipMemcpyAsync(&s0, h->dPruneStat.get(), sizeof(s0), hipMemcpyDeviceToHost, h->stream));
    RS_HIP(hipMemcpyAsync(c2.data(), h->dListCnt.get() + h->listCntCap, sizeof(unsigned) * c2.size(), hipMemcpyDeviceToHost,
                          h->stream));
    RS_HIP(hipStreamSynchronize(h->stream));
    out[0] = (int64_t)s0;
    for (const unsigned c : c2) out[1] += (int64_t)c;
    out[2] = h->prunePairs;
    out[3] = h->prunePasses;
    return RS_OK;
}

int rs_vt_prune_verified(rs_vt* h, int64_t* out) {
    rs::clear_error();
    RS_CHECK(h && out, RS_ERR_ARG, "null argument");
    *out = 0;
    if (h->prunePasses == 0) return RS_OK;
    RS_HIP(hipSetDevice(h->device));
    unsigned long long v = 0ull;
    RS_HIP(hipMemcpyAsync(&v, h->dPruneStat.get() + 2, sizeof(v), hipMemcpyDeviceToHost, h->stream));
    RS_HIP(hipStreamSynchronize(h->stream));
    *out = (int64_t)v;
    return RS_OK;
}

int rs_vt_last_ms(rs_vt* h, double* ms) {
    RS_CHECK(h && ms, RS_ERR_ARG, "null argument");
    *ms = h->timedScan ? h->lastMs : -1.0;
    return RS_OK;
}

int rs_vt_set_timing(rs_vt* h, int enable) {
    rs::clear_error();
    RS_CHECK(h, RS_ERR_STATE, "null view-template handle");
    h->timing = enable != 0;
    return RS_OK;
}

int rs_comm_unique_id(uint8_t id[RS_UNIQUE_ID_BYTES]) {
    rs::clear_error();
    RS_CHECK(id, RS_ERR_ARG, "null id buffer");
    static_assert(sizeof(ncclUniqueId) == RS_UNIQUE_ID_BYTES, "ncclUniqueId size");
    ncclUniqueId u;
    ncclResult_t r = ncclGetUniqueId(&u);
    RS_CHECK(r == ncclSuccess, RS_ERR_RCCL, "ncclGetUniqueId failed: %s", ncclGetErrorString(r));
    std::memcpy(id, &u, sizeof(u));
    return RS_OK;
}

int rs_vt_attach_comm(rs_vt* h, int rank, int nranks, const uint8_t id[RS_UNIQUE_ID_BYTES]) {
    rs::clear_error();
    RS_CHECK(h && id, RS_ERR_ARG, "null argument");
    RS_CHECK(nranks >= 1 && rank >= 0 && rank < nranks, RS_ERR_ARG, "bad rank %d of %d", rank, nranks);
    RS_CHECK(h->count == 0 && h->comm == nullptr, RS_ERR_STATE,
             "attach the communicator before adding templates, once");
    RS_HIP(hipSetDevice(h->device));
    {
        ncclUniqueId u;
        std::memcpy(&u, id, sizeof(u));
        ncclComm_t comm = nullptr;
        ncclResult_t r = ncclCommInitRank(&comm, nranks, u, rank);
        RS_CHECK(r == ncclSuccess, RS_ERR_RCCL, "ncclCommInitRank failed: %s", ncclGetErrorString(r));
        h->comm = comm;
    }
    h->rank = rank;
    h->nranks = nranks;
    return RS_OK;
}

}
```

### pyratslam_amd/csrc/vt_plan.h

```cpp
#pragma once

#include <algorithm>
#include <cstdint>

namespace vt_plan {

inline int64_t local_count_of(int rank, int nranks, int64_t global_count) {
    if (global_count <= rank) return 0;
    return (global_count - rank + nranks - 1) / nranks;
}

inline int plane_split(int ntb, int nbatch, int slots, int nqc_override) {
    int nqc = nqc_override;
    if (nqc_override <= 0) {
        const int fill = (slots + ntb - 1) / ntb;
        nqc = std::max(32, std::min(4 * fill, std::max(128, fill)));
    }
    nqc = std::min(nqc, std::max(1, nbatch));
    if (nqc >= 8) nqc &= ~7;
    return nqc;
}

#if defined(__HIPCC__)
#define VT_PLAN_HD __host__ __device__
#else
#define VT_PLAN_HD
#endif
struct Take {
    int nbatch;
    int nstat;
    int sb;
    int ndyn;
    bool takes;
    unsigned last;
};
VT_PLAN_HD inline int take_groups(int nblk) { return nblk >= 8 ? 8 : 1; }
VT_PLAN_HD inline int take_group_of(int l, int nblk) { return nblk >= 8 ? (l & 7) : 0; }
struct BlockId {
    int tb, l;
};
VT_PLAN_HD inline BlockId block_id(unsigned bid, int ntb, int nqc, bool lfirst) {
    if (lfirst) {
        const unsigned l = bid / (unsigned)ntb;
        return {(int)(bid - l * (unsigned)ntb), (int)l};
    }
    const unsigned tb = bid / (unsigned)nqc;
    return {(int)tb, (int)(bid - tb * (unsigned)nqc)};
}
VT_PLAN_HD inline int list_use(int nq, int nb, int per, int nqc) {
    const int use = ((nq + nb - 1) / nb + per - 1) / per;
    if (nqc >= 8) {
        const int u8 = (use + 7) & ~7;
        return u8 < 8 ? 8 : (u8 > nqc ? nqc : u8);
    }
    return use < 1 ? 1 : (use > nqc ? nqc : use);
}
VT_PLAN_HD inline int list_width(int entries, int per, int fill, int nqc) {
    if (list_use(entries, 4, per, nqc) >= fill) return 4;
    if (list_use(entries, 2, per, nqc) >= fill) return 2;
    return 1;
}
VT_PLAN_HD inline int list_round(int use, int fill, int nqc) {
    int cap = fill < 1 ? 1 : fill;
    if (nqc >= 8) cap = (cap + 7) & ~7;
    return use < cap ? use : cap;
}
VT_PLAN_HD inline int spec_width(int lane) { return (lane & 7) < 4 ? 4 : (lane & 7) < 6 ? 2 : 1; }
VT_PLAN_HD inline int spec_entry(int lane) { return (lane & 7) < 4 ? (lane & 7) : (lane & 7) < 6 ? (lane & 7) - 4 : 0; }
VT_PLAN_HD inline int spec_index(int batch, int lane, int ld) {
    const int i = batch * spec_width(lane) + spec_entry(lane);
    return i < ld - 1 ? i : ld - 1;
}
VT_PLAN_HD inline int spec_lane(int w) { return w == 4 ? 0 : w == 2 ? 4 : 6; }
inline int list_per(int ntb, int resident_blocks) { return ntb < resident_blocks ? 4 : 3; }
VT_PLAN_HD inline Take take_plan(int nq, int nb, int l, int nblk) {
    const int G = take_groups(nblk), g = take_group_of(l, nblk);
    Take t;
    t.nbatch = ((nq + nb - 1) / nb - g + G - 1) / G;
    t.nstat = nblk / G;
    t.sb = G == 8 ? (l >> 3) : l;
    t.ndyn = t.nbatch > t.nstat ? t.nbatch - t.nstat : 0;
    t.takes = t.ndyn > 0 && t.sb < t.nbatch;
    t.last = (unsigned)(t.ndyn + (t.nstat < t.nbatch ? t.nstat : t.nbatch) - 1);
    return t;
}
VT_PLAN_HD inline int take_batch(const Take& t, unsigned take) { return t.nstat + (int)take; }

constexpr int VT_PRUNE_MIN_Q = 512;
constexpr int64_t VT_PRUNE_MAX_TB = 65535;

inline bool prunes(int H, bool cand, int64_t tb0, bool forms, int64_t ntb, int prune, int nq) {
    return H == 64 && !cand && tb0 == 0 && forms && ntb <= VT_PRUNE_MAX_TB &&
           (prune == 2 || (prune == 1 && nq >= VT_PRUNE_MIN_Q && ntb >= 2));
}

struct Grid2 {
    int x, y;
};
inline Grid2 prefilter_grid(int ntb, int nq, int tb_per_block, int q_per_batch, int cap) {
    const int nqb = (nq + q_per_batch - 1) / q_per_batch, pfx = (ntb + tb_per_block - 1) / tb_per_block;
    return {pfx, std::min(nqb, std::max(1, cap / pfx))};
}

inline bool front_fused(int ntb, int tb_per_block) { return ntb <= tb_per_block; }
inline Grid2 front_grid(int nq, int q_per_batch, int cap) {
    return {1, std::max(1, std::min((nq + q_per_batch - 1) / q_per_batch, cap))};
}

constexpr int VT_EXPORT_BLOCKS = 64, VT_EXPORT_BLOCKS_STREAM = 256;
inline int export_grid(int64_t n, int max_blocks) { return (int)std::min<int64_t>((n + 255) / 256, max_blocks); }

constexpr int VT_ZC_MAX = 64;
inline bool stages_in_place(bool planar, int nq, bool zc_on) { return planar && nq <= VT_ZC_MAX && zc_on; }

constexpr int VT_POLL_MAX = 4096;
inline bool polls_keys(bool poll_on, bool timed, int nq) { return poll_on && !timed && nq <= VT_POLL_MAX; }
inline bool folds_keys(bool fold_ok, bool planar, int64_t local_count, bool poll_on, bool timing, int nq) {
    return fold_ok && planar && local_count > 0 && polls_keys(poll_on, timing, nq);
}

enum class StreamPath { Fused, HostGroups, PerBatch };
inline StreamPath stream_path(bool on_device, bool planar, int nb) {
    if (!planar) return StreamPath::PerBatch;
    if (!on_device) return StreamPath::HostGroups;
    return nb > 1 ? StreamPath::Fused : StreamPath::PerBatch;
}

constexpr int VT_UP_GROUP = 16;
struct HostGroup {
    int b0, n;
    int buf;
    bool waits;
};
struct HostGroups {
    int gb;
    int first;
    int nb;
    HostGroup group(int g) const {
        const int b0 = g == 0 ? 0 : std::min(nb, first + (g - 1) * gb);
        return {b0, std::min(g == 0 ? first : gb, nb - b0), g & 1, g >= 2};
    }
};
inline HostGroups host_groups(int nb) {
    const int gb = std::min(nb, std::max(2, std::min(VT_UP_GROUP, (nb - 1) / 3)));
    return {gb, nb >= 4 ? 1 : gb, nb};
}

constexpr int METRIC_WRAPPED = 0, METRIC_SAD = 1;
inline bool metric_known(int metric) { return metric == METRIC_WRAPPED || metric == METRIC_SAD; }
inline bool sad_fast(int H, int max_offset) { return max_offset == 8 && (H == 64 || H == 32); }
inline const char* sad_form(int H, int max_offset) { return sad_fast(H, max_offset) ? "sad" : "sad-generic"; }
constexpr int SAD_NQ = 2;
constexpr int SAD_NW = 8;
inline int sad_waves(int WD) { return std::min(WD, SAD_NW); }
constexpr int SAD_TARGET_BLOCKS = 4096, SAD_MIN_GROUPS = 8;
inline int sad_split(int ntb, int ngroups) {
    const int want = (SAD_TARGET_BLOCKS + ntb - 1) / ntb;
    return std::max(1, std::min(want, ngroups / SAD_MIN_GROUPS));
}

}
```

### pyratslam_amd/csrc/vt_plane_scan.h

```cpp
#pragma once

constexpr int PL_SPLIT = 2;

template <int H, int HALF>
struct PlaneRange {
    static constexpr int M = FAST_M, NU = H / 4, S0 = M - 3, S1 = H - M - 1, NS = S1 - S0 + 1;
    static constexpr int NSH = (NS + PL_SPLIT - 1) / PL_SPLIT;
    static constexpr int SA = S0 + HALF * NSH;
    static constexpr int SB = (SA + NSH - 1) < S1 ? SA + NSH - 1 : S1;
    static constexpr int ja(int s) { return (s - (M - 1)) > 0 ? (s - (M - 1) + 3) / 4 : 0; }
    static constexpr int jb(int s) { return (s + (M - 1)) / 4 < NU - 1 ? (s + (M - 1)) / 4 : NU - 1; }
    static constexpr int JLO = ja(SA), JHI = jb(SB), NUH = JHI - JLO + 1;
};

constexpr int PL_NO = 2 * FAST_M - 1;
constexpr int PL_NA = (PL_NO + 3) / 4;
constexpr int pl_class(int x) { return ((FAST_M - 1 - x) % 4 + 4) % 4; }
constexpr int pl_class_n(int rho) {
    const int base = ((FAST_M - 1 - rho) % 4 + 4) % 4;
    return base < PL_NO ? (PL_NO - 1 - base) / 4 + 1 : 0;
}
constexpr int pl_class_slot(int rho) {
    int s = 0;
    for (int r = 0; r < rho; ++r) s += (pl_class_n(r) + 1) / 2;
    return s;
}
constexpr int pl_slot(int x) { return pl_class_slot(pl_class(x)) + x / 8; }
constexpr int pl_half(int x) { return (x / 4) & 1; }

struct QRow {
    uint32_t v[8];
};

template <int H, int HALF>
struct PlaneWalk {
    using R = PlaneRange<H, HALF>;
    static constexpr int NR = R::SB - R::SA + 1;
    static constexpr int first(int rho) { return R::SA + ((rho - R::SA) % 4 + 4) % 4; }
    static constexpr int rows(int rho) { return first(rho) <= R::SB ? (R::SB - first(rho)) / 4 + 1 : 0; }
    static constexpr int row(int i) {
        for (int rho = 0; rho < 4; ++rho) {
            if (i < rows(rho)) return first(rho) + 4 * i;
            i -= rows(rho);
        }
        return -1;
    }
    static constexpr bool last(int i) { return i + 1 == NR || (row(i + 1) & 3) != (row(i) & 3); }
    static constexpr bool units_ok() {
        for (int s = R::SA; s <= R::SB; ++s) {
            const int nj = R::jb(s) - R::ja(s) + 1;
            if (nj < 1 || nj > PL_NA || R::ja(s) < R::JLO || R::jb(s) > R::JHI) return false;
        }
        return true;
    }
    static_assert(units_ok(), "units per query row");
    static_assert(rows(0) && rows(1) && rows(2) && rows(3), "every class has a row");
};

template <int H, int HALF, int S>
__device__ __forceinline__ void plane_row(const uint32_t (&P)[PlaneRange<H, HALF>::NUH][8],
                                          const QRow& q, uint32_t (&a)[PL_NA]) {
    using R = PlaneRange<H, HALF>;
    constexpr int M = FAST_M, JA = R::ja(S), NJ = R::jb(S) - JA + 1;
    uint32_t b[NJ];
#pragma unroll
    for (int k = 0; k < 8; ++k)
#pragma unroll
        for (int j = 0; j < NJ; ++j)
            b[j] = __builtin_amdgcn_bitop3_b32(P[JA - R::JLO + j][k], q.v[k], k ? b[j] : 0u, 0x8E);
#pragma unroll
    for (int j = 0; j < NJ; ++j) {
        uint32_t& c = a[(4 * (JA + j) - S + M - 1) / 4];
        asm("v_bcnt_u32_b32 %0, %1, %2" : "=v"(c) : "v"(b[j]), "v"(c));
    }
}

template <int H, int HALF, int S>
__device__ __forceinline__ QRow plane_read(const uint32_t* sq) {
    using R = PlaneRange<H, HALF>;
    const uint4 lo = *reinterpret_cast<const uint4*>(sq + (S - R::S0) * 8);
    const uint4 hi = *reinterpret_cast<const uint4*>(sq + (S - R::S0) * 8 + 4);
    return QRow{{lo.x, lo.y, lo.z, lo.w, hi.x, hi.y, hi.z, hi.w}};
}

template <int H, int HALF, int I>
__device__ __forceinline__ void plane_walk(const uint32_t (&P)[PlaneRange<H, HALF>::NUH][8],
                                           const uint32_t* sq, const uint32_t* sqn, QRow& q,
                                           uint32_t (&a)[PL_NA], uint32_t (&part)[pl_class_slot(4)][64],
                                           int lane) {
    using WK = PlaneWalk<H, HALF>;
    constexpr int S = WK::row(I);
    constexpr bool wrap = I + 1 == WK::NR;
    const QRow qn = plane_read<H, HALF, WK::row(wrap ? 0 : I + 1)>(wrap ? sqn : sq);
    __builtin_amdgcn_sched_barrier(0);
    plane_row<H, HALF, S>(P, q, a);
    if constexpr (WK::last(I)) {
        constexpr int rho = S & 3, n = pl_class_n(rho);
#pragma unroll
        for (int k = 0; k < (n + 1) / 2; ++k)
            atomicAdd(&part[pl_class_slot(rho) + k][lane], a[2 * k] | (2 * k + 1 < n ? a[2 * k + 1] << 16 : 0u));
#pragma unroll
        for (int k = 0; k < PL_NA; ++k) a[k] = 0u;
    }
    q = qn;
    if constexpr (!wrap) plane_walk<H, HALF, I + 1>(P, sq, sqn, q, a, part, lane);
}


template <int H>
struct PlaneLds {
    static constexpr int M = FAST_M, NS = H - 2 * M + 3, NO = 2 * M - 1, NK = (NO + 1) / 2;
    static constexpr int QW = PL_CG * NS * 8;
    static constexpr int NW = PL_CG * PL_SPLIT;
    static constexpr int QP = (PL_NB * QW / 4 + 63) / 64 * 64;
};

constexpr int PL_NK = PlaneLds<64>::NK;
static_assert(PlaneLds<32>::NK == PL_NK, "partial-count slots independent of H");
static_assert(pl_class_slot(4) == PL_NK, "the classes' u16 pairs fill the same slots");
template <int H>
__shared__ uint4 vt_pl_qa[PlaneLds<H>::QP];
template <int H>
__shared__ uint4 vt_pl_qb[PlaneLds<H>::QP];
__shared__ uint32_t vt_pl_part0[PL_NB][PL_NK][64];
__shared__ uint32_t vt_pl_part1[PL_NB][PL_NK][64];
__shared__ int vt_pl_bidx[3];
alignas(16) __shared__ uint32_t vt_pl_ts[16][64];
template <int H, int CUR>
__device__ __forceinline__ uint4* pl_q() {
    if constexpr (CUR == 0) return vt_pl_qa<H>;
    else return vt_pl_qb<H>;
}
template <int CUR>
__device__ __forceinline__ uint32_t (&pl_part())[PL_NB][PL_NK][64] {
    if constexpr (CUR == 0) return vt_pl_part0;
    else return vt_pl_part1;
}

template <int H, int HALF>
__device__ __forceinline__ void plane_load_units(const uint4* __restrict__ planes, int tb, int cg,
                                                 int lane, uint32_t (&P)[PlaneRange<H, HALF>::NUH][8]) {
    using R = PlaneRange<H, HALF>;
    const uint4* src = planes + ((size_t)(tb * PL_CG + cg) * (H / 4) + R::JLO) * 128 + lane;
#pragma unroll
    for (int j = 0; j < R::NUH; ++j) {
        const uint4 a = src[(2 * j) * 64], b = src[(2 * j + 1) * 64];
        P[j][0] = a.x; P[j][1] = a.y; P[j][2] = a.z; P[j][3] = a.w;
        P[j][4] = b.x; P[j][5] = b.y; P[j][6] = b.z; P[j][7] = b.w;
    }
}

struct PlaneIds {
    int qc[PL_NB];
    int qnv;
};
__device__ __forceinline__ int plane_take(unsigned* __restrict__ ctr, const vt_plan::Take& tk, unsigned& failed) {
    if (!tk.takes) return tk.nbatch;
    const unsigned t = atomicAdd(ctr, 1u);
    const int b = vt_plan::take_batch(tk, t);
    if (b >= tk.nbatch) failed = t;
    return b;
}
template <int H, bool LIST>
__device__ __forceinline__ void plane_stage(const uint4* __restrict__ qp4, int qn, int nbn, const int (&qx)[PL_NB],
                                            uint4* dst, int wave, int lane) {
    using LD = PlaneLds<H>;
    constexpr int NT = 64 * LD::NW;
    const int lim = nbn * LD::QW / 4;
    const uint4* src = qp4 + (size_t)qn * (LD::QW / 4);
#pragma unroll
    for (int k = 0; k < (LD::QP + NT - 1) / NT; ++k) {
        const int i0 = wave * 64 + k * NT;
        if (i0 < lim) {
            const uint4* from;
            if constexpr (LIST) {
                const int i = min(i0 + lane, lim - 1), e = i / (LD::QW / 4);
                const int id = e == 0 ? qx[0] : e == 1 ? qx[1] : e == 2 ? qx[2] : qx[3];
                from = qp4 + (size_t)id * (LD::QW / 4) + (i - e * (LD::QW / 4));
            } else {
                from = src + min(i0 + lane, lim - 1);
            }
            __builtin_amdgcn_global_load_lds((__attribute__((address_space(1))) const void*)from,
                                             (__attribute__((address_space(3))) void*)(dst + i0), 16, 0, 0);
        }
    }
}
template <int H, int HALF, bool MATRIX, int CUR, bool LIST, bool FIRST = false>
__device__ __forceinline__ bool plane_batch(const uint32_t (&P)[PlaneRange<H, HALF>::NUH][8], int it,
                                            int& bi, const vt_plan::Take& tk, int64_t slot, int64_t count,
                                            const uint4* __restrict__ qp4, const uint32_t* __restrict__ qsum,
                                            int nq, unsigned* __restrict__ ctr, int G, int g, ScanOut out,
                                            int rank, int nranks, int wave, int cg, int lane,
                                            unsigned& failed, const int* __restrict__ ids, PlaneIds& pid,
                                            int w) {
    using R = PlaneRange<H, HALF>;
    using LD = PlaneLds<H>;
    constexpr int NO = LD::NO, NK = LD::NK, NS = LD::NS;
    constexpr bool DEFER = FIRST && LIST;
    const int W = LIST ? w : PL_NB;
    const int nbatch = tk.nbatch;
    if (bi >= nbatch) return false;
    const uint4* qcur = pl_q<H, CUR>();
    uint4* qnxt = pl_q<H, CUR ^ 1>();
    uint32_t(&part)[PL_NB][PL_NK][64] = pl_part<CUR>();
    const int tid = wave * 64 + lane;
    const int r1 = (it + 1) % 3, r2 = (it + 2) % 3;
    const int bn = vt_pl_bidx[r1];
    const int qb = (bi * G + g) * W, nb = min(W, nq - qb);
    if (tid == 0)
        vt_pl_bidx[r2] = bn < nbatch ? plane_take(ctr, tk, failed) : nbatch;
    int qnx[PL_NB] = {0, 0, 0, 0};
    auto stage_next = [&]() {
        if (bn < nbatch) {
            const int qn = (bn * G + g) * W, nbn = min(W, nq - qn);
            if constexpr (LIST) {
                static_assert(PL_NB == 4, "four ids per batch");
#pragma unroll
                for (int e = 0; e < PL_NB; ++e) qnx[e] = __builtin_amdgcn_readlane(pid.qnv, e);
            }
            plane_stage<H, LIST>(qp4, qn, nbn, qnx, qnxt, wave, lane);
        }
    };
    if constexpr (!DEFER) stage_next();
    const uint32_t* sq0 = reinterpret_cast<const uint32_t*>(qcur) + cg * NS * 8;
    QRow q = plane_read<H, HALF, PlaneWalk<H, HALF>::row(0)>(sq0);
    auto walk = [&](int b) {
        uint32_t a[PL_NA];
#pragma unroll
        for (int k = 0; k < PL_NA; ++k) a[k] = 0u;
        plane_walk<H, HALF, 0>(P, sq0 + b * (PL_CG * NS * 8), sq0 + min(b + 1, nb - 1) * (PL_CG * NS * 8), q, a,
                               part[b], lane);
    };
    if constexpr (DEFER) {
        walk(0);
        stage_next();
    }
#pragma unroll 1
    for (int b = DEFER ? 1 : 0; b < nb; ++b) walk(b);
    if constexpr (FIRST) VT_STAMP(4);
    __builtin_amdgcn_s_waitcnt(0x0F70);
    __syncthreads();
    if (wave < nb) {
        const int qi = !LIST ? qb + wave
                             : wave == 0 ? pid.qc[0] : wave == 1 ? pid.qc[1] : wave == 2 ? pid.qc[2] : pid.qc[3];
        uint32_t best = 0xFFFFFFFFu, t[NK];
#pragma unroll
        for (int k = 0; k < NK; ++k) {
            t[k] = part[wave][k][lane];
            part[wave][k][lane] = 0u;
        }
#pragma unroll
        for (int x = 0; x < NO; ++x)
            best = min(best, vt_pl_ts[x][lane] + 256u * (pl_half(x) ? t[pl_slot(x)] >> 16 : t[pl_slot(x)] & 0xFFFFu));
        emit_score<MATRIX>(out, slot, count, qi, LIST ? qi + 1 : nq, best - qsum[qi], rank, nranks, lane == 0);
    }
    if constexpr (LIST) {
#pragma unroll
        for (int e = 0; e < PL_NB; ++e) pid.qc[e] = qnx[e];
        const int b2 = vt_pl_bidx[r2];
        pid.qnv = b2 < nbatch ? ids[min((b2 * G + g) * W + (lane & 3), nq - 1)] : 0;
    }
    bi = bn;
    return true;
}

template <int H, int HALF, bool MATRIX, bool LIST>
__device__ __forceinline__ void plane_wave(const uint4* __restrict__ planes, const uint32_t* __restrict__ tsum,
                                           int tb, int64_t count, const uint4* __restrict__ qp4,
                                           const uint32_t* __restrict__ qsum, int nq,
                                           unsigned* __restrict__ ctr, int G, int g, ScanOut out,
                                           int rank, int nranks, int wave, int cg, int lane,
                                           unsigned& failed, const int* __restrict__ ids,
                                           const vt_plan::Take& tk, int v0, int w) {
    using R = PlaneRange<H, HALF>;
    const int nbatch = tk.nbatch, tid = wave * 64 + lane;
    const int W = LIST ? w : PL_NB;
    int bi = tk.sb, b1 = nbatch;
    if (tid == 0) b1 = plane_take(ctr, tk, failed);
    for (int i = tid; i < PL_NB * PL_NK * 64; i += 64 * PL_CG * PL_SPLIT) {
        (&vt_pl_part0[0][0][0])[i] = 0u;
        (&vt_pl_part1[0][0][0])[i] = 0u;
    }
    PlaneIds pid{{0, 0, 0, 0}, 0};
    if constexpr (LIST) {
#pragma unroll
        for (int e = 0; e < PL_NB; ++e) pid.qc[e] = __builtin_amdgcn_readlane(v0, vt_plan::spec_lane(W) + e);
    }
    {
        const int qb = (bi * G + g) * W;
        plane_stage<H, LIST>(qp4, qb, min(W, nq - qb), pid.qc, vt_pl_qa<H>, wave, lane);
    }
    uint32_t P[R::NUH][8];
    plane_load_units<H, HALF>(planes, tb, cg, lane, P);
    static_assert(sizeof(vt_pl_ts) == 4 * 64 * 16, "TS: one 1 KiB DMA piece from each of four waves");
    if (wave < 4)
        __builtin_amdgcn_global_load_lds(
            (__attribute__((address_space(1))) const void*)(reinterpret_cast<const uint4*>(tsum) +
                                                            (size_t)tb * 256 + wave * 64 + lane),
            (__attribute__((address_space(3))) void*)(reinterpret_cast<uint4*>(&vt_pl_ts[0][0]) + wave * 64), 16, 0,
            0);
    if (tid == 0) {
        vt_pl_bidx[0] = bi;
        vt_pl_bidx[1] = b1;
    }
    VT_STAMP(1);
    __builtin_amdgcn_s_waitcnt(0x0F70);
    VT_STAMP(3);
    __syncthreads();
    VT_STAMP(2);
    const int64_t slot = (int64_t)tb * 64 + lane;
    if constexpr (LIST) {
        b1 = vt_pl_bidx[1];
        pid.qnv = b1 < nbatch ? ids[min((b1 * G + g) * W + (lane & 3), nq - 1)] : 0;
    }
    if (plane_batch<H, HALF, MATRIX, 0, LIST, true>(P, 0, bi, tk, slot, count, qp4, qsum, nq, ctr, G, g, out, rank,
                                                    nranks, wave, cg, lane, failed, ids, pid, W))
        for (int it = 1;; it += 2) {
            if (!plane_batch<H, HALF, MATRIX, 1, LIST>(P, it, bi, tk, slot, count, qp4, qsum, nq, ctr, G, g, out,
                                                       rank, nranks, wave, cg, lane, failed, ids, pid, W))
                break;
            if (!plane_batch<H, HALF, MATRIX, 0, LIST>(P, it + 1, bi, tk, slot, count, qp4, qsum, nq, ctr, G, g,
                                                       out, rank, nranks, wave, cg, lane, failed, ids, pid, W))
                break;
        }
    VT_STAMP(5);
}

#ifndef VT_LIST_PER_B1
#define VT_LIST_PER_B1 1
#endif
struct PlaneList {
    const int* ids = nullptr;
    const unsigned* cnt = nullptr;
    int ld = 0;
    uint32_t per : 8;
    uint32_t nb : 7;
    uint32_t lfirst : 1;
    uint32_t fill : 16;
};
static_assert(sizeof(PlaneList) == 24, "the plane scan's kernel arguments keep their layout");
#ifdef VT_LIST_NB
static_assert(VT_LIST_NB == 1 || VT_LIST_NB == 2 || VT_LIST_NB == 4, "entries per batch: 1, 2 or 4");
#else
#define VT_LIST_NB 0
#endif

template <int H, bool MATRIX, bool LIST = false>
__global__ __launch_bounds__(64 * PL_CG * PL_SPLIT) __attribute__((amdgpu_waves_per_eu(4, 4)))
void vt_scan_plane_kernel(const uint4* __restrict__ planes, const uint32_t* __restrict__ tsum,
                          int ntb, int64_t count, const uint32_t* __restrict__ qp,
                          const uint32_t* __restrict__ qsum, int nq, int nqc,
                          unsigned* __restrict__ next_batch, ScanOut out, int rank, int nranks,
                          PlaneList pl) {
    static_assert(PL_SPLIT == 2, "two row ranges");
    static_assert(!(LIST && MATRIX), "lists feed the key scan only");
    VT_STAMP_BEGIN();
    const vt_plan::BlockId bid = vt_plan::block_id(blockIdx.x, ntb, nqc, LIST && pl.lfirst);
    const int tb = bid.tb;
    const int l = bid.l;
    const int G = vt_plan::take_groups(nqc), g = vt_plan::take_group_of(l, nqc);
    unsigned* ctr = next_batch + (size_t)tb * 8 + g;
    const int lane = threadIdx.x & 63;
    const int* ids = nullptr;
    int v0 = 0;
    int W = PL_NB;
    if constexpr (LIST) {
        ids = pl.ids + (size_t)tb * pl.ld;
        v0 = ids[vt_plan::spec_index((G == 8 ? l >> 3 : l) * G + g, lane, pl.ld)];
        nq = (int)pl.cnt[tb];
        if (nq == 0) return;
        W = pl.nb ? (int)pl.nb : vt_plan::list_width(nq, pl.per, pl.fill, nqc);
        int use = vt_plan::list_use(nq, W, pl.per, nqc);
        if (!pl.nb && W < PL_NB) use = vt_plan::list_round(use, pl.fill, nqc);
        if (l >= use) return;
        nqc = use;
    }
    const vt_plan::Take tk = vt_plan::take_plan(nq, W, l, nqc);
    VT_STAMP_KNOWN();
    const int wave = __builtin_amdgcn_readfirstlane(threadIdx.x >> 6);
    const int cg = wave % PL_CG, half = wave / PL_CG;
    unsigned failed = 0u;
    const uint4* qp4 = reinterpret_cast<const uint4*>(qp);
    if (tk.sb >= tk.nbatch) {
    } else if (half == 0)
        plane_wave<H, 0, MATRIX, LIST>(planes, tsum, tb, count, qp4, qsum, nq, ctr, G, g, out, rank, nranks,
                                       wave, cg, lane, failed, ids, tk, v0, W);
    else
        plane_wave<H, 1, MATRIX, LIST>(planes, tsum, tb, count, qp4, qsum, nq, ctr, G, g, out, rank, nranks,
                                       wave, cg, lane, failed, ids, tk, v0, W);
    if (threadIdx.x == 0 && tk.takes && failed == tk.last) *ctr = 0u;
    if constexpr (!MATRIX) {
        if (out.host) {
            __shared__ int s_last;
            asm volatile("s_waitcnt vmcnt(0)" ::: "memory");
            __syncthreads();
            if (threadIdx.x == 0) {
                __builtin_amdgcn_fence(__ATOMIC_RELEASE, "agent");
                s_last = __hip_atomic_fetch_add(out.done, 1u, __ATOMIC_RELAXED, __HIP_MEMORY_SCOPE_AGENT) ==
                         gridDim.x - 1;
                if (s_last) __builtin_amdgcn_fence(__ATOMIC_ACQUIRE, "agent");
            }
            __syncthreads();
            if (s_last) {
                for (int i = threadIdx.x; i < nq; i += blockDim.x) {
                    const unsigned long long k =
                        __hip_atomic_load(out.best + i, __ATOMIC_RELAXED, __HIP_MEMORY_SCOPE_AGENT);
                    __hip_atomic_store(out.best + i, ~0ull, __ATOMIC_RELAXED, __HIP_MEMORY_SCOPE_AGENT);
                    __hip_atomic_store(out.host + i, k, __ATOMIC_RELAXED, __HIP_MEMORY_SCOPE_SYSTEM);
                }
                if (threadIdx.x == 0) __hip_atomic_store(out.done, 0u, __ATOMIC_RELAXED, __HIP_MEMORY_SCOPE_AGENT);
            }
        }
    }
    VT_STAMP(6);
}
```

### pyratslam_amd/csrc/vt_prune.h

```cpp
#pragma once

constexpr int PF_WAVES = 4;
#ifndef VT_PF_TPW
#define VT_PF_TPW (VT_PF_UNITS == 1 ? 8 / (VT_PF_CGS) : 1)
#endif
constexpr int PF_TPW = VT_PF_TPW;
#ifndef VT_PF_CPS
#define VT_PF_CPS (VT_PF_TPW >= 4 ? 1 : 2)
#endif
constexpr int PF_CPS = VT_PF_CPS;
#ifndef VT_PF_GRID_CAP
#define VT_PF_GRID_CAP 4096
#endif
constexpr int PF_NB = 4;
constexpr int PF_QW4 = PF_NU * PF_CGS * PL_NO * 2;
constexpr uint32_t PF_NONE = (1u << 26) - 1u;

constexpr uint32_t PF_BIAS = PF_CGS * 32 * 256;
static_assert(PF_NU * (PF_CGS * 32 * 256 + PF_BIAS) < (1u << 31), "the biased bounds do not wrap");

__device__ __forceinline__ void pf_load(const uint4* __restrict__ planes, int ntb, int64_t count, int tb0, int lane,
                                        uint32_t (&P)[PF_TPW][PF_NU][PF_CGS][8], uint32_t (&tsb)[PF_TPW],
                                        bool (&valid)[PF_TPW]) {
    constexpr int NU = 64 / 4;
#pragma unroll
    for (int t = 0; t < PF_TPW; ++t) {
        const int tbc = min(tb0 + t, ntb - 1);
        valid[t] = tb0 + t < ntb && (int64_t)(tb0 + t) * 64 + lane < count;
        tsb[t] = 0u - PF_NU * PF_BIAS;
#pragma unroll
        for (int u = 0; u < PF_NU; ++u) {
#pragma unroll
            for (int cg = 0; cg < PF_CGS; ++cg) {
                const uint4* src = planes + ((size_t)(tbc * PL_CG + cg) * NU + pf_unit(u)) * 128 + lane;
                const uint4 a = src[0], b = src[64];
                uint32_t(&p)[8] = P[t][u][cg];
                p[0] = a.x; p[1] = a.y; p[2] = a.z; p[3] = a.w;
                p[4] = b.x; p[5] = b.y; p[6] = b.z; p[7] = b.w;
#pragma unroll
                for (int k = 0; k < 8; ++k) tsb[t] += (uint32_t)__builtin_popcount(p[k]) << k;
            }
        }
    }
}

__device__ __forceinline__ void pf_stage(const uint4* __restrict__ qc4, const uint32_t* __restrict__ qsj, int q0, int nb,
                                         uint4 (&s_q)[PF_NB][PF_NU][PF_CGS][PL_NO][2],
                                         uint32_t (&s_qs)[PF_NB][PF_NU][16]) {
    constexpr int M = FAST_M, S0 = M - 3;
    for (int i = threadIdx.x; i < nb * PF_QW4; i += blockDim.x) {
        const int qq = i / PF_QW4, r = i - qq * PF_QW4;
        const int u = r / (PF_CGS * PL_NO * 2), r2 = r - u * (PF_CGS * PL_NO * 2);
        const int cg = r2 / (PL_NO * 2), w = r2 - cg * (PL_NO * 2);
        (&s_q[0][0][0][0][0])[i] = qc_unit(qc4 + (size_t)(q0 + qq) * QC_Q4, cg,
                                           4 * pf_unit(u) - (M - 1) - S0 + (w >> 1), w & 1);
    }
    if ((int)threadIdx.x < nb * PF_NU * 16)
        (&s_qs[0][0][0])[threadIdx.x] = PF_BIAS - qsj[(size_t)q0 * PF_NU * 16 + threadIdx.x];
}

__device__ __forceinline__ void pf_walk(const uint32_t (&P)[PF_TPW][PF_NU][PF_CGS][8], const uint32_t (&tsb)[PF_TPW],
                                        const bool (&valid)[PF_TPW], const uint4 (&sq)[PF_NU][PF_CGS][PL_NO][2],
                                        const uint32_t (&sqs)[PF_NU][16], int lane, uint32_t (&v)[PF_TPW],
                                        uint32_t (&w)[PF_TPW]) {
    uint32_t m[PF_TPW];
#pragma unroll
    for (int t = 0; t < PF_TPW; ++t) m[t] = 0xFFFFFFFFu;
    auto read_q = [&](int x, int u, int cp, uint32_t(&q)[PF_CPS][8]) {
#pragma unroll
        for (int i = 0; i < PF_CPS; ++i) {
            const uint4 lo = sq[u][cp + i][PL_NO - 1 - x][0];
            const uint4 hi = sq[u][cp + i][PL_NO - 1 - x][1];
            q[i][0] = lo.x; q[i][1] = lo.y; q[i][2] = lo.z; q[i][3] = lo.w;
            q[i][4] = hi.x; q[i][5] = hi.y; q[i][6] = hi.z; q[i][7] = hi.w;
        }
    };
#pragma unroll
    for (int x = 0; x < PL_NO; ++x) {
        uint32_t lb[PF_TPW];
#pragma unroll
        for (int t = 0; t < PF_TPW; ++t) lb[t] = 0u;
#pragma unroll
        for (int u = 0; u < PF_NU; ++u) {
            uint32_t c[PF_TPW];
#pragma unroll
            for (int t = 0; t < PF_TPW; ++t) c[t] = 0u;
#pragma unroll
            for (int cp = 0; cp < PF_CGS; cp += PF_CPS) {
                uint32_t q[PF_CPS][8], b[PF_TPW][PF_CPS];
                read_q(x, u, cp, q);
#pragma unroll
                for (int k = 0; k < 8; ++k)
#pragma unroll
                    for (int t = 0; t < PF_TPW; ++t)
#pragma unroll
                        for (int i = 0; i < PF_CPS; ++i)
                            b[t][i] = __builtin_amdgcn_bitop3_b32(P[t][u][cp + i][k], q[i][k],
                                                                  k ? b[t][i] : 0u, 0x8E);
#pragma unroll
                for (int t = 0; t < PF_TPW; ++t)
#pragma unroll
                    for (int i = 0; i < PF_CPS; ++i)
                        asm("v_bcnt_u32_b32 %0, %1, %2" : "=v"(c[t]) : "v"(b[t][i]), "v"(c[t]));
                __builtin_amdgcn_sched_barrier(0);
            }
            const uint32_t qsb = sqs[u][x];
#pragma unroll
            for (int t = 0; t < PF_TPW; ++t) lb[t] += (c[t] << 8) + qsb;
        }
#pragma unroll
        for (int t = 0; t < PF_TPW; ++t) m[t] = min(m[t], lb[t]);
    }
#pragma unroll
    for (int t = 0; t < PF_TPW; ++t) {
        const uint32_t lbt = m[t] + tsb[t];
        v[t] = wave_min_u32_dpp(valid[t] ? (lbt << 6) | (uint32_t)lane : 0xFFFFFFFFu);
        w[t] = wave_min_u32_dpp(valid[t] && lane != (int)(v[t] & 63u) ? lbt : PF_NONE);
    }
}

__global__ __launch_bounds__(64 * PF_WAVES) __attribute__((amdgpu_waves_per_eu(4)))
void vt_prefilter_kernel(const uint4* __restrict__ planes, int ntb,
                                                                    int64_t count,
                                                                    const uint4* __restrict__ qc4,
                                                                    const uint32_t* __restrict__ qsj, int nq,
                                                                    uint32_t* __restrict__ minlb,
                                                                    uint32_t* __restrict__ second) {
    static_assert(PF_CGS % PF_CPS == 0 && PF_CGS >= 1 && PF_CGS <= PL_CG, "whole steps of column groups, of the unit");
    static_assert(PF_NU * PF_CGS * 32 * 255 < (int)PF_NONE, "a bound and a lane fit one word");
    __shared__ uint4 s_q[PF_NB][PF_NU][PF_CGS][PL_NO][2];
    __shared__ uint32_t s_qs[PF_NB][PF_NU][16];
    const int wave = __builtin_amdgcn_readfirstlane(threadIdx.x >> 6), lane = threadIdx.x & 63;
    const int tb0 = (blockIdx.x * PF_WAVES + wave) * PF_TPW;
    const bool live = tb0 < ntb;
    uint32_t P[PF_TPW][PF_NU][PF_CGS][8], tsb[PF_TPW];
    bool valid[PF_TPW];
    pf_load(planes, ntb, count, tb0, lane, P, tsb, valid);
    for (int q0 = blockIdx.y * PF_NB; q0 < nq; q0 += gridDim.y * PF_NB) {
        const int nb = min(PF_NB, nq - q0);
        __syncthreads();
        pf_stage(qc4, qsj, q0, nb, s_q, s_qs);
        __syncthreads();
        if (!live) continue;
#pragma unroll 1
        for (int qq = 0; qq < nb; ++qq) {
            uint32_t v[PF_TPW], w[PF_TPW];
            pf_walk(P, tsb, valid, s_q[qq], s_qs[qq], lane, v, w);
            if (lane == 0) {
#pragma unroll
                for (int t = 0; t < PF_TPW; ++t)
                    if (tb0 + t < ntb) {
                        minlb[(size_t)(tb0 + t) * nq + q0 + qq] = v[t] >> 6;
                        second[(size_t)(tb0 + t) * nq + q0 + qq] = (w[t] << 6) | (v[t] & 63u);
                    }
            }
        }
    }
}

constexpr int VT_LIST_T = 1024;
__device__ __forceinline__ void list_append(bool in, int q, unsigned* __restrict__ cnt, int* __restrict__ list) {
    __shared__ unsigned s_w[VT_LIST_T / 64];
    __shared__ unsigned s_base;
    const int lane = threadIdx.x & 63, wave = threadIdx.x >> 6;
    const unsigned long long mask = __ballot(in);
    if (lane == 0) s_w[wave] = (unsigned)__popcll(mask);
    __syncthreads();
    if (threadIdx.x == 0) {
        unsigned t = 0u;
        for (int w = 0; w < VT_LIST_T / 64; ++w) {
            const unsigned c = s_w[w];
            s_w[w] = t;
            t += c;
        }
        s_base = t ? atomicAdd(cnt, t) : 0u;
    }
    __syncthreads();
    if (in) list[s_base + s_w[wave] + (unsigned)__popcll(mask & ((1ull << lane) - 1ull))] = q;
}

constexpr int VT_VQ4 = PlaneLds<64>::QW / 4;
constexpr int VT_VR = QC_NA + 7;
constexpr int VT_VQS = PL_CG * VT_VR * 2, VT_VTS = PL_CG * (64 / 4) * 2;
template <bool WAVE_LDS, class Pick>
__device__ __forceinline__ void vt_verify_query(int q, int lane, Pick&& pick, int nq,
                                                const uint4* __restrict__ planes,
                                                const uint32_t* __restrict__ tsum,
                                                const uint4* __restrict__ qc4, uint4* __restrict__ qp4,
                                                const uint32_t* __restrict__ qsum,
                                                unsigned long long* __restrict__ best, int rank, int nranks,
                                                int* __restrict__ tbstar, uint4* s_q, uint4* s_t) {
    constexpr int M = FAST_M, NU = 64 / 4, NS = PlaneLds<64>::NS, S0 = M - 3, S1 = 64 - M - 1;
    static_assert(PL_NO * PL_CG <= 64, "one lane per (offset, column group)");
    constexpr int QK = (QC_Q4 + 63) / 64;
    const int x = lane >> 2, cg = lane & 3, o = x - (M - 1);
    uint4 qv[QK];
#pragma unroll
    for (int k = 0; k < QK; ++k) qv[k] = qc4[(size_t)q * QC_Q4 + min(lane + 64 * k, QC_Q4 - 1)];
    const uint32_t qs = qsum[q];
    unsigned long long pk = ~0ull;
    uint32_t sec = 0u, m2 = 0xFFFFFFFFu;
    pick(pk, sec, m2);
#pragma unroll
    for (int k = 0; k < QK; ++k) asm volatile("" : "+v"(qv[k].x), "+v"(qv[k].y), "+v"(qv[k].z), "+v"(qv[k].w));
    const unsigned long long mk = wave_min_u64(pk);
    const int tbs = (int)(unsigned)mk;
    uint32_t other = pk == mk ? m2 : (uint32_t)(pk >> 32);
#pragma unroll
    for (int off = 32; off > 0; off >>= 1) other = min(other, (uint32_t)__shfl_xor((int)other, off));
    sec = (uint32_t)__shfl((int)sec, __ffsll((unsigned long long)__ballot(pk == mk)) - 1);
    const int tl = (int)(sec & 63u);
    const uint32_t ts = x < PL_NO ? tsum[((size_t)tbs * 16 + x) * 64 + tl] : 0u;
    static_assert(PL_CG * NU * 2 == 128, "two template chunks per lane");
    const uint4 t0 = planes[((size_t)tbs * 128 + lane) * 64 + tl];
    const uint4 t1 = planes[((size_t)tbs * 128 + 64 + lane) * 64 + tl];
    s_t[lane] = t0;
    s_t[64 + lane] = t1;
#pragma unroll
    for (int k = 0; k < QK; ++k) {
        const int c = lane + 64 * k, g = c / (QC_NA * 2);
        if (c < QC_Q4) s_q[(g * VT_VR + 3) * 2 + (c - g * (QC_NA * 2))] = qv[k];
    }
    if (lane < 2 * PL_CG) s_q[((lane >> 1) * VT_VR + 3 + QC_NA) * 2 + (lane & 1)] = make_uint4(0u, 0u, 0u, 0u);
    if constexpr (WAVE_LDS) {
        asm volatile("s_waitcnt lgkmcnt(0)" ::: "memory");
        __builtin_amdgcn_wave_barrier();
    } else {
        __syncthreads();
    }
    uint32_t cnt = 0u;
    if (x < PL_NO) {
        const int a = (-o - S0) >> 2;
        const uint32_t sh = 8u * (uint32_t)((-o - S0) & 3);
        const uint4* sq = s_q + (cg * VT_VR + 3 + a) * 2;
        uint4 la = sq[0], lc = sq[1];
#pragma unroll 4
        for (int j = 0; j < NU; ++j) {
            const bool in = 4 * j - o >= S0 && 4 * j - o <= S1;
            const uint4 ta = s_t[(cg * NU + j) * 2], tc = s_t[(cg * NU + j) * 2 + 1];
            const uint4 ha = sq[(j + 1) * 2], hc = sq[(j + 1) * 2 + 1];
            const uint4 qa = qc_shift(la, ha, sh), qc = qc_shift(lc, hc, sh);
            la = ha;
            lc = hc;
            uint32_t b = __builtin_amdgcn_bitop3_b32(ta.x, qa.x, 0u, 0x8E);
            b = __builtin_amdgcn_bitop3_b32(ta.y, qa.y, b, 0x8E);
            b = __builtin_amdgcn_bitop3_b32(ta.z, qa.z, b, 0x8E);
            b = __builtin_amdgcn_bitop3_b32(ta.w, qa.w, b, 0x8E);
            b = __builtin_amdgcn_bitop3_b32(tc.x, qc.x, b, 0x8E);
            b = __builtin_amdgcn_bitop3_b32(tc.y, qc.y, b, 0x8E);
            b = __builtin_amdgcn_bitop3_b32(tc.z, qc.z, b, 0x8E);
            b = __builtin_amdgcn_bitop3_b32(tc.w, qc.w, b, 0x8E);
            cnt += in ? (uint32_t)__builtin_popcount(b) : 0u;
        }
    }
    cnt += __shfl_xor(cnt, 1);
    cnt += __shfl_xor(cnt, 2);
    uint32_t u0 = x < PL_NO ? ts + 256u * cnt : 0xFFFFFFFFu;
#pragma unroll
    for (int off = 32; off > 0; off >>= 1) u0 = min(u0, (uint32_t)__shfl_xor(u0, off));
    u0 -= qs;
    const bool settled = (sec >> 6) > u0;
    if (!settled || other <= u0) {
#pragma unroll
        for (int k = 0; k < (VT_VQ4 + 63) / 64; ++k) {
            const int i = lane + 64 * k, g = i / (NS * 2), r = i - g * (NS * 2), si = r >> 1;
            if (i < VT_VQ4) {
                const uint4* su = s_q + (g * VT_VR + 3 + (si >> 2)) * 2 + (r & 1);
                qp4[(size_t)q * VT_VQ4 + i] = qc_shift(su[0], su[2], 8u * (uint32_t)(si & 3));
            }
        }
    }
    if (lane == 0) {
        if (settled) {
            const unsigned long long g = ((unsigned long long)tbs * 64 + tl) * nranks + rank;
            atomicMin(best + q, ((unsigned long long)u0 << 32) | g);
        }
        tbstar[q] = settled ? ~tbs : tbs;
    }
}

__global__ __launch_bounds__(64) void vt_prune_verify_kernel(const uint32_t* __restrict__ minlb,
                                                             const uint32_t* __restrict__ second, int ntb, int nq,
                                                             const uint4* __restrict__ planes,
                                                             const uint32_t* __restrict__ tsum,
                                                             const uint4* __restrict__ qc4,
                                                             uint4* __restrict__ qp4,
                                                             const uint32_t* __restrict__ qsum,
                                                             unsigned long long* __restrict__ best, int rank,
                                                             int nranks, int* __restrict__ tbstar) {
    __shared__ uint4 s_q[VT_VQS];
    __shared__ uint4 s_t[VT_VTS];
    const int q = blockIdx.x, lane = threadIdx.x;
    vt_verify_query<false>(q, lane, [&](unsigned long long& pk, uint32_t& sec, uint32_t& m2) {
        for (int tb = lane; tb < ntb; tb += 64) {
            const unsigned long long k = ((unsigned long long)minlb[(size_t)tb * nq + q] << 32) | (unsigned)tb;
            const uint32_t s2 = second[(size_t)tb * nq + q];
            const bool lt = k < pk;
            m2 = min(m2, (uint32_t)((lt ? pk : k) >> 32));
            pk = lt ? k : pk;
            sec = lt ? s2 : sec;
        }
    }, nq, planes, tsum, qc4, qp4, qsum, best, rank, nranks, tbstar, s_q, s_t);
}

__global__ __launch_bounds__(64 * PF_WAVES) __attribute__((amdgpu_waves_per_eu(4)))
void vt_front_kernel(const uint4* __restrict__ planes, int ntb, int64_t count, const uint4* __restrict__ qc4,
                     const uint32_t* __restrict__ qsj, int nq, uint32_t* __restrict__ minlb,
                     const uint32_t* __restrict__ tsum, uint4* __restrict__ qp4,
                     const uint32_t* __restrict__ qsum, unsigned long long* __restrict__ best, int rank,
                     int nranks, int* __restrict__ tbstar) {
    constexpr int CH = PF_WAVES * PF_TPW;
    static_assert(PF_WAVES == PF_NB, "one wave per query of the group in the tail");
    static_assert(CH <= 64, "one lane per block of a chunk");
    __shared__ uint4 s_q[PF_NB][PF_NU][PF_CGS][PL_NO][2];
    __shared__ uint32_t s_qs[PF_NB][PF_NU][16];
    __shared__ uint2 s_pick[2][PF_NB][CH];
    __shared__ uint4 s_vq[PF_WAVES][VT_VQS];
    __shared__ uint4 s_vt[PF_WAVES][VT_VTS];
    const int wave = __builtin_amdgcn_readfirstlane(threadIdx.x >> 6), lane = threadIdx.x & 63;
    int par = 0;
    for (int q0 = blockIdx.y * PF_NB; q0 < nq; q0 += gridDim.y * PF_NB) {
        const int nb = min(PF_NB, nq - q0);
        const int qw = min(wave, nb - 1);
        __syncthreads();
        pf_stage(qc4, qsj, q0, nb, s_q, s_qs);
        __syncthreads();
        unsigned long long pk = ~0ull;
        uint32_t sec = 0u, m2 = 0xFFFFFFFFu;
        for (int c0 = 0; c0 < ntb; c0 += CH) {
            const int tb0 = c0 + wave * PF_TPW;
            if (tb0 < ntb) {
                uint32_t P[PF_TPW][PF_NU][PF_CGS][8], tsb[PF_TPW];
                bool valid[PF_TPW];
                pf_load(planes, ntb, count, tb0, lane, P, tsb, valid);
#pragma unroll 1
                for (int qq = 0; qq < nb; ++qq) {
                    uint32_t v[PF_TPW], w[PF_TPW];
                    pf_walk(P, tsb, valid, s_q[qq], s_qs[qq], lane, v, w);
                    if (lane == 0) {
#pragma unroll
                        for (int t = 0; t < PF_TPW; ++t)
                            if (tb0 + t < ntb) {
                                minlb[(size_t)(tb0 + t) * nq + q0 + qq] = v[t] >> 6;
                                s_pick[par][qq][wave * PF_TPW + t] = make_uint2(v[t] >> 6, (w[t] << 6) | (v[t] & 63u));
                            }
                    }
                }
            }
            __syncthreads();
            if (lane < CH && c0 + lane < ntb) {
                const uint2 e = s_pick[par][qw][lane];
                const unsigned long long k = ((unsigned long long)e.x << 32) | (unsigned)(c0 + lane);
                const bool lt = k < pk;
                m2 = min(m2, (uint32_t)((lt ? pk : k) >> 32));
                pk = lt ? k : pk;
                sec = lt ? e.y : sec;
            }
            par ^= 1;
        }
        int vl = lane;
        asm volatile("" : "+v"(vl));
        if (wave < nb)
            vt_verify_query<true>(q0 + wave, vl, [&](unsigned long long& pk_, uint32_t& sec_, uint32_t& m2_) {
                pk_ = pk;
                sec_ = sec;
                m2_ = m2;
            }, nq, planes, tsum, qc4, qp4, qsum, best, rank, nranks, tbstar, s_vq[wave], s_vt[wave]);
    }
}

__global__ __launch_bounds__(VT_LIST_T) void vt_prune_first_kernel(int nq, const int* __restrict__ tbstar,
                                                                   unsigned* __restrict__ cnt,
                                                                   int* __restrict__ list,
                                                                   unsigned* __restrict__ verified,
                                                                   unsigned* __restrict__ cnt2, int ntb) {
    const int q = blockIdx.x * VT_LIST_T + threadIdx.x, tb = blockIdx.y;
    const int ts = q < nq ? tbstar[q] : INT_MAX;
    if (blockIdx.x == 0 && tb == 0)
        for (int b = threadIdx.x; b < ntb; b += VT_LIST_T) cnt2[b] = 0u;
    if (tb == 0) {
        const int n = __syncthreads_count(ts < 0);
        if (threadIdx.x == 0 && n) atomicAdd(verified, (unsigned)n);
    }
    list_append(ts == tb, q, cnt + tb, list + (size_t)tb * nq);
}

__global__ __launch_bounds__(VT_LIST_T) void vt_prune_rest_kernel(const uint32_t* __restrict__ minlb, int nq,
                                                                  const int* __restrict__ tbstar,
                                                                  const unsigned long long* __restrict__ best,
                                                                  unsigned* __restrict__ cnt,
                                                                  int* __restrict__ list,
                                                                  unsigned* __restrict__ cnt1,
                                                                  unsigned* __restrict__ verified, int ntb,
                                                                  unsigned long long* __restrict__ stat) {
    const int q = blockIdx.x * VT_LIST_T + threadIdx.x, tb = blockIdx.y;
    const int ts = q < nq ? tbstar[q] : 0;
    const bool in = q < nq && tb != (ts < 0 ? ~ts : ts) && minlb[(size_t)tb * nq + q] <= (uint32_t)(best[q] >> 32);
    list_append(in, q, cnt + tb, list + (size_t)tb * nq);
    if (blockIdx.x == 0 && tb == 0) {
        __shared__ unsigned long long s_sum;
        if (threadIdx.x == 0) s_sum = 0ull;
        __syncthreads();
        unsigned long long a = 0ull;
        for (int b = threadIdx.x; b < ntb; b += VT_LIST_T) {
            a += cnt1[b];
            cnt1[b] = 0u;
        }
        if (a) atomicAdd(&s_sum, a);
        __syncthreads();
        if (threadIdx.x == 0) {
            const unsigned v = *verified;
            *verified = 0u;
            stat[0] = s_sum + v;
            stat[2] = v;
        }
    }
}

__global__ __launch_bounds__(256) void vt_keys_export(unsigned long long* __restrict__ keys, int n,
                                                      unsigned long long* host) {
    for (int i = blockIdx.x * 256 + threadIdx.x; i < n; i += gridDim.x * 256) {
        __hip_atomic_store(host + i, keys[i], __ATOMIC_RELAXED, __HIP_MEMORY_SCOPE_SYSTEM);
        keys[i] = ~0ull;
    }
}
```

### pyratslam_amd/view_templates.py

```python
import ctypes
import threading

import numpy as np

from . import _lib

MAX_OFFSET = 8
METRICS = {'wrapped': _lib.RS_VT_METRIC_WRAPPED, 'sad': _lib.RS_VT_METRIC_SAD}
_FLOAT_CODES = {np.dtype(np.float32): _lib.RS_DT_F32, np.dtype(np.float64): _lib.RS_DT_F64}


def sad_scores(templates, queries, max_offset=MAX_OFFSET, device=0):
    t = np.asarray(templates)
    q = np.asarray(queries)
    dt = np.result_type(t.dtype, q.dtype)
    if dt not in _FLOAT_CODES:
        raise TypeError('ViewTemplate.match takes uint8 (wrapping) or float32/float64 arrays; '
                        'got %s and %s' % (t.dtype, q.dtype))
    if t.ndim != 3 or q.ndim != 3 or t.shape[1:] != q.shape[1:]:
        raise ValueError('template / query shapes %r, %r differ' % (t.shape[1:], q.shape[1:]))
    t = np.ascontiguousarray(t, dtype=dt)
    q = np.ascontiguousarray(q, dtype=dt)
    out = np.empty((q.shape[0], t.shape[0]), dtype=dt)
    lib = _lib.require_device()
    _lib.check(lib.rs_sad_scores(int(device), _FLOAT_CODES[dt], t.shape[1], t.shape[2], int(max_offset),
                                 t.shape[0], ctypes.c_void_p(t.ctypes.data), q.shape[0],
                                 ctypes.c_void_p(q.ctypes.data), ctypes.c_void_p(out.ctypes.data)))
    return out


def numpy_sad_u8_scores(library, query, max_offset=MAX_OFFSET):
    lib = np.asarray(library)
    q = np.asarray(query)
    if lib.dtype != np.uint8 or q.dtype != np.uint8:
        raise TypeError('numpy_sad_u8_scores takes uint8 arrays, got %s and %s' % (lib.dtype, q.dtype))
    t, h, _ = lib.shape
    if t == 0:
        return np.zeros(0, dtype=np.uint64)
    q = q[max_offset:h - max_offset][None]
    best = None
    for o in range(-max_offset + 1, max_offset):
        a = lib[:, max_offset + o:h - max_offset + o, :]
        d = (np.maximum(a, q) - np.minimum(a, q)).sum(axis=(1, 2), dtype=np.uint64)
        best = d if best is None else np.minimum(best, d)
    return best


def numpy_offset_profile(template, query, max_offset=MAX_OFFSET, metric='wrapped'):
    t = np.asarray(template).astype(np.int64)
    q = np.asarray(query).astype(np.int64)
    h, m = t.shape[0], int(max_offset)
    _metric_code(metric)
    prof = np.zeros(2 * m - 1, dtype=np.uint32)
    for k, o in enumerate(range(-m + 1, m)):
        d = t[m + o:h - m + o] - q[m:h - m]
        prof[k] = (np.abs(d) if metric == 'sad' else d % 256).sum()
    return int(np.argmin(prof)) - (m - 1), prof


def refine_offset(profile):
    p = np.asarray(profile, dtype=np.float64)
    if p.ndim == 2:
        return np.array([refine_offset(row) for row in p], dtype=np.float64)
    if p.ndim != 1 or p.size % 2 != 1:
        raise ValueError('a profile has 2 * max_offset - 1 entries, got shape %r' % (p.shape,))
    k = int(np.argmin(p))
    o = float(k - (p.size - 1) // 2)
    if k == 0 or k == p.size - 1:
        return o
    den = p[k - 1] - 2.0 * p[k] + p[k + 1]
    if not den > 0.0:
        return o
    return o + 0.5 * (p[k - 1] - p[k + 1]) / den


MAX_NORM_RADIUS, MAX_NORM_GAIN = 7, 127


def _normalise_arg(normalise):
    if normalise is None:
        return None
    try:
        radius, gain = normalise
        ok = int(radius) == radius and int(gain) == gain
    except (TypeError, ValueError):
        ok = False
    if not ok or not 1 <= radius <= MAX_NORM_RADIUS or not 1 <= gain <= MAX_NORM_GAIN:
        raise ValueError('normalise=%r: expected None or (radius in [1, %d], gain in [1, %d])'
                         % (normalise, MAX_NORM_RADIUS, MAX_NORM_GAIN))
    return int(radius), int(gain)


def _u8_images(images, what):
    a = np.asarray(images)
    if a.dtype != np.uint8:
        raise TypeError('%s takes uint8 images, got %s' % (what, a.dtype))
    if a.ndim not in (2, 3):
        raise ValueError('%s takes (H, W) or (n, H, W) images, got shape %r' % (what, a.shape))
    return a


def normalise_u8(images, radius, gain):
    R, G = _normalise_arg((radius, gain))
    a = _u8_images(images, 'normalise_u8')
    p = a.reshape((-1,) + a.shape[-2:]).astype(np.int64)
    n_img, h, w = p.shape
    r0, r1 = np.maximum(np.arange(h) - R, 0)[:, None], (np.minimum(np.arange(h) + R, h - 1) + 1)[:, None]
    c0, c1 = np.maximum(np.arange(w) - R, 0)[None, :], (np.minimum(np.arange(w) + R, w - 1) + 1)[None, :]

    def window_sum(x):
        sat = np.zeros((n_img, h + 1, w + 1), dtype=np.int64)
        sat[:, 1:, 1:] = x.cumsum(axis=1).cumsum(axis=2)
        return sat[:, r1, c1] - sat[:, r0, c1] - sat[:, r1, c0] + sat[:, r0, c0]

    n = (r1 - r0) * (c1 - c0)
    S, S2 = window_sum(p), window_sum(p * p)
    D, N = n * S2 - S * S, n * p - S
    s = np.sqrt(D.astype(np.float64)).astype(np.int64)
    s -= s * s > D
    s += (s + 1) * (s + 1) <= D
    q = (G * np.abs(N) + s // 2) // np.maximum(s, 1)
    out = np.where(s == 0, 128, np.clip(128 + np.sign(N) * q, 0, 255))
    return out.astype(np.uint8).reshape(a.shape)


def normalise_host(images, radius, gain):
    R, G = _normalise_arg((radius, gain))
    a = np.ascontiguousarray(_u8_images(images, 'normalise_host'))
    out = np.empty_like(a)
    lib = _lib.load()
    src, dst = a.reshape((-1,) + a.shape[-2:]), out.reshape((-1,) + a.shape[-2:])
    for i in range(src.shape[0]):
        _lib.check(lib.rs_vt_normalise_host(a.shape[-2], a.shape[-1], R, G, _lib.ptr(src[i], ctypes.c_uint8),
                                            _lib.ptr(dst[i], ctypes.c_uint8)))
    return out


def _metric_code(metric):
    if metric not in METRICS:
        raise ValueError('unknown metric %r: expected one of %s' % (metric, sorted(METRICS)))
    return METRICS[metric]


def _u8_scores(templates, queries, device=0, metric='wrapped'):
    t = np.ascontiguousarray(templates, dtype=np.uint8)
    lib = ViewTemplates._from_shape(t.shape[1:], np.inf, device=device, capacity=len(t), metric=metric)
    try:
        lib.add(t)
        return lib.scores(queries)
    finally:
        lib.close()


def py2_mask(x_range, y_range, x_step, y_step, im_x, im_y):
    pix = np.arange(im_x * im_y)
    r, c = np.divmod(pix, im_x)
    keep = (r > y_range[0]) & (r < y_range[1]) & (c > x_range[0]) & (c < x_range[1])
    keep &= ((r - y_range[0]) % y_step != 0) & ((c - x_range[0]) % x_step != 0)
    shape = ((x_range[1] - x_range[0]) // x_step, (y_range[1] - y_range[0]) // y_step)
    return keep.reshape((im_x, im_y)), shape


class ViewTemplate:

    def __init__(self, pc_x, pc_y, pc_th, index, template, _owner=None):
        self.pc_x = pc_x
        self.pc_y = pc_y
        self.pc_th = pc_th
        self.template = template
        self.index = index
        self.max_offset = MAX_OFFSET
        self._owner = _owner
        self._solo = None

    def match(self, new_template):
        if self.template is None:
            owner = self._owner
            raise ValueError('the bytes of template %d live on rank %d (template g is stored on '
                             'rank g %% %d): score it there' % (self.index, self.index % owner.nranks,
                                                                owner.nranks))
        q = np.ascontiguousarray(new_template)
        t = np.asarray(self.template)
        dev = self._owner.device if self._owner is not None else 0
        norm = self._owner.normalise if self._owner is not None else None
        if norm is not None:
            self._owner._normalise_take(q)
        if t.dtype != np.uint8 or q.dtype != np.uint8:
            return sad_scores(t[None], q[None], self.max_offset, dev)[0, 0]
        owner = self._owner
        if owner is not None and owner.nranks == 1 and not owner._float:
            return owner.scores(q[None], self.index, 1)[0, 0]
        if norm is not None:
            q = normalise_host(q, *norm)
        if self._solo is None:
            t = np.ascontiguousarray(t)
            self._solo = ViewTemplates._from_shape(t.shape, np.inf, device=dev,
                                                   metric=owner.metric if owner is not None else 'wrapped')
            self._solo.add(t[None])
        return self._solo.scores(q[None], 0, 1)[0, 0]

    refine_offset = staticmethod(refine_offset)

    def location(self):
        return (self.pc_x, self.pc_y, self.pc_th)

    def get_index(self):
        return self.index


class ViewTemplates:

    def __init__(self, x_range, y_range, x_step, y_step, im_x, im_y, match_threshold,
                 device=0, capacity=1024, metric='wrapped', offsets=False, shift_axis='rows', normalise=None):
        normalise = _normalise_arg(normalise)
        self._set_geometry(x_range, y_range, x_step, y_step, im_x, im_y, shift_axis)
        self._init_device(self.shape, match_threshold, device, capacity, metric, offsets, normalise)

    def _set_geometry(self, x_range, y_range, x_step, y_step, im_x, im_y, shift_axis='rows'):
        if shift_axis not in ('rows', 'cols'):
            raise ValueError("shift_axis %r: expected 'rows' or 'cols'" % (shift_axis,))
        self.mask, shape = py2_mask(x_range, y_range, x_step, y_step, im_x, im_y)
        self.shift_axis = shift_axis
        self._gathered_shape = shape
        self.shape = shape if shift_axis == 'rows' else shape[::-1]
        return self

    @classmethod
    def _from_shape(cls, shape, match_threshold, device=0, capacity=64, metric='wrapped', offsets=False,
                    normalise=None):
        self = cls.__new__(cls)
        self.mask = None
        self.shape = tuple(int(s) for s in shape)
        self._init_device(self.shape, match_threshold, device, capacity, metric, offsets, normalise)
        return self

    shift_axis = 'rows'

    normalise = None

    def _init_device(self, shape, match_threshold, device, capacity, metric='wrapped', offsets=False,
                     normalise=None):
        code = _metric_code(metric)
        normalise = _normalise_arg(normalise)
        self.metric = metric
        self.offsets = bool(offsets)
        self.last_offsets = self.last_profiles = None
        self.shape = (int(shape[0]), int(shape[1]))
        self.match_threshold = match_threshold
        self.templates = []
        self.device = int(device)
        self.rank, self.nranks = 0, 1
        self._float = False
        self._vtf = None
        self._fdtype = None
        self._capacity = int(capacity)
        self._timing = False
        self._mutex = threading.Lock()
        self._h = None
        self._lib = _lib.require_device()
        h = ctypes.c_void_p()
        if code == _lib.RS_VT_METRIC_WRAPPED:
            _lib.check(self._lib.rs_vt_create(self.shape[0], self.shape[1], MAX_OFFSET, 0,
                                              int(capacity), self.device, ctypes.byref(h)))
        else:
            _lib.check(self._lib.rs_vt_create_metric(self.shape[0], self.shape[1], MAX_OFFSET, 0,
                                                     int(capacity), self.device, code, ctypes.byref(h)))
        self._h = h
        _lib.check(self._lib.rs_vt_set_threshold(h, float(match_threshold)))
        if normalise is not None:
            _lib.check(self._lib.rs_vt_set_normalise(h, normalise[0], normalise[1]))
        self.normalise = normalise

    def close(self):
        st = 0
        if getattr(self, '_h', None) is not None and self._h.value:
            st = self._lib.rs_vt_destroy(self._h)
        self._h = None
        sf = self._drop_resident()
        _lib.check(st or sf)

    def __del__(self):
        try:
            self.close()
        except Exception:
            pass

    def __len__(self):
        return len(self.templates)

    def __getitem__(self, index):
        return self.templates[index]

    def subsample(self, image):
        im = np.asarray(image)
        if im.dtype != np.uint8 and im.dtype not in _FLOAT_CODES:
            raise TypeError('ViewTemplates matches uint8 (mono8, ros_simulate.py:100-101) or '
                            'float32/float64 frames; got %s' % im.dtype)
        if im.shape != self.mask.shape:
            raise ValueError('frame shape %r does not match the mask %r' % (im.shape, self.mask.shape))
        cache = getattr(self, '_mask_take', None)
        if cache is None or cache[0] is not self.mask:
            cache = (self.mask, np.flatnonzero(self.mask.ravel()))
            self._mask_take = cache
        if self.shift_axis == 'rows':
            return im.reshape(-1).take(cache[1]).reshape(self.shape)
        return np.ascontiguousarray(im.reshape(-1).take(cache[1]).reshape(self._gathered_shape).T)

    def gather_pixels(self):
        if self.mask is None:
            raise ValueError('no subsampling mask: construct with the frame geometry')
        pix = np.flatnonzero(self.mask.ravel())
        if self.shift_axis == 'cols':
            pix = pix.reshape(self._gathered_shape).T
        return np.ascontiguousarray(pix.reshape(-1), dtype=np.int32)

    def _check_templates(self, t):
        t = np.asarray(t)
        if t.dtype != np.uint8:
            raise TypeError('templates must be uint8, got %s' % t.dtype)
        if t.shape[-2:] != self.shape:
            raise ValueError('template shape %r != %r' % (t.shape[-2:], self.shape))
        return np.ascontiguousarray(t.reshape((-1,) + self.shape))

    def count(self):
        c = ctypes.c_int64()
        if self._vtf is not None:
            _lib.check(self._lib.rs_vtf_count(self._vtf, ctypes.byref(c)))
        else:
            _lib.check(self._lib.rs_vt_count(self._h, ctypes.byref(c)))
        return c.value

    def _normalise_take(self, arrays):
        if self.normalise is not None and np.asarray(arrays).dtype != np.uint8:
            raise TypeError('normalise=%r normalises uint8 frames only; got %s'
                            % (self.normalise, np.asarray(arrays).dtype))

    def _stored(self, t):
        return t if self.normalise is None else normalise_host(t, *self.normalise)

    def _refuse_float(self, what):
        if self._float or self._vtf is not None:
            raise TypeError('this library has matched float frames: %s works on uint8 '
                            'device libraries only; use match() / match_batch()' % what)

    _resident_ok = True

    def _resident_for(self, dtype):
        if self._float or dtype not in _FLOAT_CODES:
            return False
        if self._vtf is not None:
            return dtype == self._fdtype
        with self._mutex:
            if self._vtf is not None:
                return dtype == self._fdtype
            if not self._resident_ok or self.nranks != 1 or self.templates:
                return False
            h = ctypes.c_void_p()
            _lib.check(self._lib.rs_vtf_create(self.shape[0], self.shape[1], MAX_OFFSET,
                                               _FLOAT_CODES[dtype], int(self._capacity), self.device,
                                               ctypes.byref(h)))
            if self._timing:
                _lib.check(self._lib.rs_vtf_set_timing(h, 1))
            self._vtf, self._fdtype = h, dtype
        return True

    def _use_resident(self, arrays):
        return self._vtf is not None or self._resident_for(np.asarray(arrays).dtype)

    def _drop_resident(self):
        st = 0
        if getattr(self, '_vtf', None) is not None and self._vtf.value:
            st = self._lib.rs_vtf_destroy(self._vtf)
        self._vtf = None
        return st

    def _check_float(self, t, what):
        t = np.asarray(t)
        if t.dtype != self._fdtype:
            raise TypeError('this library has matched float frames and holds %s templates: '
                            '%s takes %s arrays, got %s' % (self._fdtype, what, self._fdtype, t.dtype))
        if t.shape[-2:] != self.shape:
            raise ValueError('template shape %r != %r' % (t.shape[-2:], self.shape))
        return np.ascontiguousarray(t.reshape((-1,) + self.shape))

    def _resident_match(self, q, pcs):
        n = q.shape[0]
        best = np.empty(n, dtype=self._fdtype)
        bidx = np.empty(n, dtype=np.int64)
        inb = np.empty((n, n), dtype=self._fdtype) if n > 1 else None
        _lib.check(self._lib.rs_vtf_scan(
            self._vtf, n, ctypes.c_void_p(q.ctypes.data), int(n > 1), ctypes.c_void_p(best.ctypes.data),
            _lib.ptr(bidx, ctypes.c_int64), None if inb is None else ctypes.c_void_p(inb.ctypes.data)))
        base = len(self.templates)
        idx = np.empty(n, dtype=np.int64)
        score = np.empty(n, dtype=self._fdtype)
        new = np.zeros(n, dtype=bool)
        added = []
        for i in range(n):
            m, arg = best[i], int(bidx[i])
            if added:
                s = inb[i, added]
                k = int(np.argmin(s))
                if arg < 0 or s[k] < m:
                    m, arg = s[k], base + k
            score[i] = m
            if arg < 0 or m > self.match_threshold:
                idx[i], new[i] = base + len(added), True
                added.append(i)
            else:
                idx[i] = arg
        if added:
            first = ctypes.c_int64()
            which = np.asarray(added, dtype=np.int32)
            _lib.check(self._lib.rs_vtf_append_staged(self._vtf, len(added), _lib.ptr(which, ctypes.c_int32),
                                                      ctypes.byref(first)))
            assert first.value == base, (first.value, base)
            for k, i in enumerate(added):
                p = pcs[i]
                self.templates.append(ViewTemplate(p[0], p[1], p[2], base + k, q[i].copy(), _owner=self))
        return idx, score, new

    def add(self, templates, locations=None):
        self._offsets_take(templates)
        self._normalise_take(templates)
        if self._use_resident(templates):
            t = self._check_float(templates, 'add()')
            first = ctypes.c_int64()
            with self._mutex:
                _lib.check(self._lib.rs_vtf_add(self._vtf, t.shape[0], ctypes.c_void_p(t.ctypes.data),
                                                ctypes.byref(first)))
                for i in range(t.shape[0]):
                    loc = locations[i] if locations is not None else (0, 0, 0)
                    self.templates.append(ViewTemplate(loc[0], loc[1], loc[2], first.value + i, t[i],
                                                       _owner=self))
            return first.value
        self._refuse_float('add()')
        t = self._check_templates(templates)
        first = ctypes.c_int64()
        with self._mutex:
            _lib.check(self._lib.rs_vt_add(self._h, t.shape[0], _lib.ptr(t, ctypes.c_uint8),
                                           ctypes.byref(first)))
            t = self._stored(t)
            for i in range(t.shape[0]):
                loc = locations[i] if locations is not None else (0, 0, 0)
                self.templates.append(ViewTemplate(loc[0], loc[1], loc[2], first.value + i, t[i],
                                                   _owner=self))
        return first.value

    def scores(self, queries, t0=0, nt=None):
        self._normalise_take(queries)
        if self._use_resident(queries):
            q = self._check_float(queries, 'scores()')
            nt = self.count() - t0 if nt is None else nt
            out = np.empty((q.shape[0], nt), dtype=self._fdtype)
            with self._mutex:
                _lib.check(self._lib.rs_vtf_scores(self._vtf, q.shape[0], ctypes.c_void_p(q.ctypes.data),
                                                   int(t0), int(nt), ctypes.c_void_p(out.ctypes.data)))
            return out
        self._refuse_float('scores()')
        q = self._check_templates(queries)
        nt = self.count() - t0 if nt is None else nt
        out = np.empty((q.shape[0], nt), dtype=np.uint64)
        with self._mutex:
            _lib.check(self._lib.rs_vt_scores(self._h, q.shape[0], _lib.ptr(q, ctypes.c_uint8),
                                              int(t0), int(nt), _lib.ptr(out, ctypes.c_uint64)))
        return out

    def _offset_profile(self, index, qptr):
        index = np.ascontiguousarray(index, dtype=np.int64).reshape(-1)
        n = index.shape[0]
        offset = np.zeros(n, dtype=np.int32)
        profile = np.zeros((n, 2 * MAX_OFFSET - 1), dtype=np.uint32)
        _lib.check(self._lib.rs_vt_offset_profile(self._h, n, qptr, _lib.ptr(index, ctypes.c_int64),
                                                  _lib.ptr(profile, ctypes.c_uint32),
                                                  _lib.ptr(offset, ctypes.c_int32)))
        return offset, profile

    def _refuse_offsets(self, what):
        self._refuse_float(what)
        if self.nranks > 1:
            raise TypeError('%s is not supported by a sharded library: the template of a match '
                            'lives on one rank' % what)

    def offset_profile(self, index, queries=None):
        self._refuse_offsets('offset_profile()')
        index = np.ascontiguousarray(index, dtype=np.int64).reshape(-1)
        keep = None
        if queries is None:
            qptr = None
        elif isinstance(queries, tuple):
            n, keep = int(queries[0]), queries[1]
            if n != index.shape[0]:
                raise ValueError('%d queries for %d indices' % (n, index.shape[0]))
            if n * self.shape[0] * self.shape[1] > keep.nbytes:
                raise ValueError('%d queries exceed the %d-byte device buffer' % (n, keep.nbytes))
            qptr = keep.ptr
        else:
            keep = self._check_templates(queries)
            if keep.shape[0] != index.shape[0]:
                raise ValueError('%d queries for %d indices' % (keep.shape[0], index.shape[0]))
            qptr = ctypes.c_void_p(keep.ctypes.data)
        with self._mutex:
            out = self._offset_profile(index, qptr)
        del keep
        return out

    def _record_offsets(self, idx, new):
        if not self.offsets:
            return
        off, prof = self._offset_profile(idx, None)
        off[np.asarray(new, dtype=bool)] = 0
        self.last_offsets, self.last_profiles = off, prof

    def _record(self, q, pcs, idx, new):
        for i in range(q.shape[0]):
            if new[i]:
                assert idx[i] == len(self.templates), (idx[i], len(self.templates))
                p = pcs[i]
                self.templates.append(ViewTemplate(p[0], p[1], p[2], int(idx[i]), self._stored(q[i]).copy(),
                                                   _owner=self))
        return [self.templates[int(j)] for j in idx]

    def match_templates(self, queries, pcs=None, mode=_lib.RS_VT_SEQUENTIAL):
        self._offsets_take(queries)
        self._normalise_take(queries)
        if self._use_resident(queries):
            q = self._check_float(queries, 'match_templates()')
            n = q.shape[0]
            with self._mutex:
                if mode == _lib.RS_VT_SEQUENTIAL:
                    return self._resident_match(q, pcs if pcs is not None else [(0, 0, 0)] * n)
                score = np.empty(n, dtype=self._fdtype)
                idx = np.empty(n, dtype=np.int64)
                _lib.check(self._lib.rs_vtf_scan(self._vtf, n, ctypes.c_void_p(q.ctypes.data), 0,
                                                 ctypes.c_void_p(score.ctypes.data),
                                                 _lib.ptr(idx, ctypes.c_int64), None))
            return idx, score, np.zeros(n, dtype=bool)
        self._refuse_float('match_templates()')
        q = self._check_templates(queries)
        n = q.shape[0]
        idx = np.empty(n, dtype=np.int64)
        score = np.empty(n, dtype=np.uint64)
        new = np.zeros(n, dtype=np.uint8)
        with self._mutex:
            _lib.check(self._lib.rs_vt_match_batch(
                self._h, n, _lib.ptr(q, ctypes.c_uint8), mode, _lib.ptr(score, ctypes.c_uint64),
                _lib.ptr(idx, ctypes.c_int64), _lib.ptr(new, ctypes.c_uint8)))
            if mode == _lib.RS_VT_SEQUENTIAL:
                self._record(q, pcs if pcs is not None else [(0, 0, 0)] * n, idx, new)
            self._record_offsets(idx, new)
        return idx, score, new.astype(bool)

    def match_stream(self, queries, nq=None):
        self._refuse_float('match_stream()')
        if isinstance(queries, tuple):
            nb, nq, buf = int(queries[0]), int(queries[1]), queries[2]
            if nb * nq * self.shape[0] * self.shape[1] > buf.nbytes:
                raise ValueError('%d x %d queries exceed the %d-byte device buffer'
                                 % (nb, nq, buf.nbytes))
            qptr, keep = buf.ptr, buf
        else:
            q = np.asarray(queries)
            if q.ndim != 4:
                raise ValueError('match_stream takes (nb, nq, H, W) queries, got %r' % (q.shape,))
            nb = q.shape[0]
            q = self._check_templates(q.reshape((-1,) + q.shape[2:])).reshape(q.shape)
            nq = q.shape[1]
            qptr, keep = ctypes.c_void_p(q.ctypes.data), q
        idx = np.empty((nb, nq), dtype=np.int64)
        score = np.empty((nb, nq), dtype=np.uint64)
        with self._mutex:
            _lib.check(self._lib.rs_vt_match_stream(self._h, nb, nq, qptr,
                                                    _lib.ptr(score, ctypes.c_uint64),
                                                    _lib.ptr(idx, ctypes.c_int64)))
        del keep
        return idx, score

    def _offsets_take(self, arrays):
        if self.offsets and np.asarray(arrays).dtype != np.uint8:
            raise TypeError('offsets=True records row offsets of uint8 frames only; got %s'
                            % np.asarray(arrays).dtype)

    def match(self, input, pc_x, pc_y, pc_th):
        t = self.subsample(input)
        self._offsets_take(t)
        self._normalise_take(t)
        if self._resident_for(t.dtype):
            with self._mutex:
                idx, _, _ = self._resident_match(np.ascontiguousarray(t)[None], [(pc_x, pc_y, pc_th)])
            return self.templates[int(idx[0])]
        if t.dtype != np.uint8 or self._float or self._vtf is not None:
            return self._match_float(t, (pc_x, pc_y, pc_th))
        idx, _, _ = self.match_templates(t[None], [(pc_x, pc_y, pc_th)])
        return self.templates[int(idx[0])]

    def match_batch(self, images, pcs):
        q = [self.subsample(im) for im in images]
        if not q:
            return []
        for x in q:
            self._offsets_take(x)
            self._normalise_take(x)
        if all(x.dtype == q[0].dtype for x in q) and self._resident_for(q[0].dtype):
            with self._mutex:
                idx, _, _ = self._resident_match(np.stack(q), pcs)
            return [self.templates[int(i)] for i in idx]
        if self._float or self._vtf is not None or any(x.dtype != np.uint8 for x in q):
            return [self._match_float(x, pc) for x, pc in zip(q, pcs)]
        idx, _, _ = self.match_templates(np.stack(q), pcs)
        return [self.templates[int(i)] for i in idx]

    def _match_float(self, template, pc):
        if self.nranks > 1:
            raise TypeError('float frames are not supported by a sharded library')
        with self._mutex:
            self._float = True
            _lib.check(self._drop_resident())
            match_val = [None] * len(self.templates)
            groups = {}
            for i, tm in enumerate(self.templates):
                groups.setdefault(np.asarray(tm.template).dtype, []).append(i)
            for dt, ids in groups.items():
                lib = np.stack([np.asarray(self.templates[i].template) for i in ids])
                if dt == np.uint8 and template.dtype == np.uint8:
                    sc = _u8_scores(lib, template[None], self.device, self.metric)[0]
                else:
                    sc = sad_scores(lib, template[None], MAX_OFFSET, self.device)[0]
                for i, v in zip(ids, sc):
                    match_val[i] = v
            if len(match_val) == 0 or min(match_val) > self.match_threshold:
                new = ViewTemplate(pc[0], pc[1], pc[2], len(self.templates), np.array(template),
                                   _owner=self)
                self.templates.append(new)
                return new
            return self.templates[int(np.argmin(match_val))]

    def _ensure_gather(self):
        if getattr(self, '_gather_ready', False):
            return
        pix = self.gather_pixels()
        assert pix.size == self.shape[0] * self.shape[1]
        _lib.check(self._lib.rs_vt_set_subsample(self._h, self.mask.size,
                                                 _lib.ptr(pix, ctypes.c_int32)))
        self._gather_ready = True

    def match_frames(self, frames, pcs, mode=_lib.RS_VT_SEQUENTIAL):
        self._refuse_float('match_frames()')
        self._ensure_gather()
        dev = isinstance(frames, tuple)
        if dev:
            n, buf = int(frames[0]), frames[1]
            if n * self.mask.size > buf.nbytes:
                raise ValueError('%d frames of %d bytes exceed the %d-byte device buffer'
                                 % (n, self.mask.size, buf.nbytes))
            fptr = buf.ptr
        else:
            f = np.asarray(frames)
            if f.dtype != np.uint8:
                raise TypeError('ViewTemplates matches uint8 frames (mono8, ros_simulate.py:100-101); '
                                'got %s' % f.dtype)
            if f.shape[1:] != self.mask.shape:
                raise ValueError('frame shape %r does not match the mask %r' % (f.shape[1:], self.mask.shape))
            f = np.ascontiguousarray(f)
            n = f.shape[0]
            fptr = ctypes.c_void_p(f.ctypes.data)
        idx = np.empty(n, dtype=np.int64)
        score = np.empty(n, dtype=np.uint64)
        new = np.zeros(n, dtype=np.uint8)
        with self._mutex:
            _lib.check(self._lib.rs_vt_match_frames(self._h, n, fptr, mode,
                                                    _lib.ptr(score, ctypes.c_uint64),
                                                    _lib.ptr(idx, ctypes.c_int64),
                                                    _lib.ptr(new, ctypes.c_uint8)))
            if mode == _lib.RS_VT_SEQUENTIAL:
                pcs = pcs if pcs is not None else [(0, 0, 0)] * n
                for i in range(n):
                    if new[i]:
                        if dev:
                            t = np.empty(self.shape, dtype=np.uint8)
                            if int(idx[i]) % self.nranks == self.rank:
                                _lib.check(self._lib.rs_vt_read(self._h, int(idx[i]),
                                                                _lib.ptr(t, ctypes.c_uint8)))
                            else:
                                t = None
                        else:
                            t = self._stored(self.subsample(f[i]))
                        p = pcs[i]
                        assert idx[i] == len(self.templates), (idx[i], len(self.templates))
                        self.templates.append(ViewTemplate(p[0], p[1], p[2], int(idx[i]), t,
                                                           _owner=self))
            self._record_offsets(idx, new)
        return idx, score, new.astype(bool)

    def device_ms(self):
        ms = ctypes.c_double()
        if self._vtf is not None:
            _lib.check(self._lib.rs_vtf_last_ms(self._vtf, ctypes.byref(ms)))
        else:
            _lib.check(self._lib.rs_vt_last_ms(self._h, ctypes.byref(ms)))
        return ms.value

    def set_timing(self, enable=True):
        _lib.check(self._lib.rs_vt_set_timing(self._h, int(bool(enable))))
        self._timing = bool(enable)
        if self._vtf is not None:
            _lib.check(self._lib.rs_vtf_set_timing(self._vtf, int(self._timing)))

    def scan_form(self):
        if self._vtf is not None:
            return 'sad-resident'
        return self._lib.rs_vt_scan_form(self._h).decode()

    def prune_stats(self):
        out = (ctypes.c_int64 * 4)()
        _lib.check(self._lib.rs_vt_prune_stats(self._h, out))
        return tuple(int(v) for v in out)

    def prune_verified(self):
        out = ctypes.c_int64(0)
        _lib.check(self._lib.rs_vt_prune_verified(self._h, ctypes.byref(out)))
        return int(out.value)


class ShardedViewTemplates(ViewTemplates):
    _resident_ok = False

    def __init__(self, x_range, y_range, x_step, y_step, im_x, im_y, match_threshold,
                 rank, nranks, reducer='rccl', unique_id=None, device=0, capacity=1024, metric='wrapped',
                 offsets=False, normalise=None):
        self._no_offsets(offsets)
        normalise = _normalise_arg(normalise)
        self.mask, self.shape = py2_mask(x_range, y_range, x_step, y_step, im_x, im_y)
        self._init_device(self.shape, match_threshold, device, capacity, metric, normalise=normalise)
        self._attach(rank, nranks, reducer, unique_id)

    @classmethod
    def from_shape(cls, shape, match_threshold, rank, nranks, reducer='rccl', unique_id=None,
                   device=0, capacity=1024, metric='wrapped', offsets=False, normalise=None):
        cls._no_offsets(offsets)
        normalise = _normalise_arg(normalise)
        self = cls.__new__(cls)
        self.mask = None
        self._init_device(shape, match_threshold, device, capacity, metric, normalise=normalise)
        self._attach(rank, nranks, reducer, unique_id)
        return self

    @staticmethod
    def _no_offsets(offsets):
        if offsets:
            raise TypeError('offsets=True is not supported by a sharded library: the template of '
                            'a match lives on one rank')

    def _attach(self, rank, nranks, reducer, unique_id):
        self.rank, self.nranks = int(rank), int(nranks)
        self.reducer = reducer
        if reducer == 'rccl':
            if unique_id is None or len(unique_id) != _lib.RS_UNIQUE_ID_BYTES:
                raise ValueError('reducer="rccl" needs the %d-byte unique id from rank 0'
                                 % _lib.RS_UNIQUE_ID_BYTES)
            uid = np.frombuffer(bytes(unique_id), dtype=np.uint8).copy()
            _lib.check(self._lib.rs_vt_attach_comm(self._h, self.rank, self.nranks,
                                                   _lib.ptr(uid, ctypes.c_uint8)))
        elif callable(reducer):
            _lib.check(self._lib.rs_vt_set_shard(self._h, self.rank, self.nranks))
        else:
            raise ValueError('reducer must be "rccl" or a callable')

    @staticmethod
    def unique_id():
        lib = _lib.require_device()
        buf = np.zeros(_lib.RS_UNIQUE_ID_BYTES, dtype=np.uint8)
        _lib.check(lib.rs_comm_unique_id(_lib.ptr(buf, ctypes.c_uint8)))
        return buf.tobytes()

    def match_templates(self, queries, pcs=None, mode=_lib.RS_VT_SEQUENTIAL):
        if self.reducer == 'rccl':
            return super().match_templates(queries, pcs, mode)
        self._normalise_take(queries)
        q = self._check_templates(queries)
        n = q.shape[0]
        local = np.empty(n, dtype=np.uint64)
        idx = np.empty(n, dtype=np.int64)
        score = np.empty(n, dtype=np.uint64)
        new = np.zeros(n, dtype=np.uint8)
        with self._mutex:
            _lib.check(self._lib.rs_vt_scan_local(self._h, n, _lib.ptr(q, ctypes.c_uint8),
                                                  _lib.ptr(local, ctypes.c_uint64)))
            glob = np.ascontiguousarray(self.reducer(local), dtype=np.uint64)
            _lib.check(self._lib.rs_vt_resolve(
                self._h, n, _lib.ptr(glob, ctypes.c_uint64), mode, _lib.ptr(score, ctypes.c_uint64),
                _lib.ptr(idx, ctypes.c_int64), _lib.ptr(new, ctypes.c_uint8)))
            if mode == _lib.RS_VT_SEQUENTIAL:
                self._record(q, pcs if pcs is not None else [(0, 0, 0)] * n, idx, new)
        return idx, score, new.astype(bool)

    def add(self, templates, locations=None):
        return super().add(templates, locations)
```

Before: 29.72 billion compares/s.

## Build prune candidate lists in the front kernel and scan in a single pass

The pruned template scan now runs as one pass by default. The front/verify kernels append each query to per-block candidate lists (using the first-pass upper bound) and zero the alternate parity counter buffer, which removes the separate prune_first kernel, the first list scan, and the prune_rest kernel. The list scan also records the upper bound for the starred block. Bookkeeping statistics are moved into an on-demand count kernel. The trade-off is that the candidate lists are looser, because they use the front's bound rather than a bound refined after the first pass, so more pairs may be scanned.

```diff
diff --git a/include/ratslam_abi.h b/include/ratslam_abi.h
--- a/include/ratslam_abi.h
+++ b/include/ratslam_abi.h
@@ -141,6 +141,7 @@
 int rs_vt_set_timing(rs_vt* h, int enable);
 const char* rs_vt_scan_form(const rs_vt* h);
 int rs_vt_prune_stats(rs_vt* h, int64_t out[4]);
+int rs_vt_prune_scanned(rs_vt* h, int64_t* out);
 int rs_vt_prune_verified(rs_vt* h, int64_t* out);
 
 int rs_vt_set_threshold(rs_vt* h, double threshold);
diff --git a/pyratslam_amd/_lib.py b/pyratslam_amd/_lib.py
--- a/pyratslam_amd/_lib.py
+++ b/pyratslam_amd/_lib.py
@@ -141,6 +141,7 @@
     'rs_vt_scan_form': (ctypes.c_char_p, [_vp]),
     'rs_vt_prune_stats': (ctypes.c_int, [_vp, _i64p]),
     'rs_vt_prune_verified': (ctypes.c_int, [_vp, _i64p]),
+    'rs_vt_prune_scanned': (ctypes.c_int, [_vp, _i64p]),
     'rs_vt_set_threshold': (ctypes.c_int, [_vp, ctypes.c_double]),
     'rs_sad_scores': (ctypes.c_int, [ctypes.c_int, ctypes.c_int, ctypes.c_int, ctypes.c_int,
                                      ctypes.c_int, ctypes.c_int64, _vp, ctypes.c_int, _vp, _vp]),
@@ -185,7 +186,7 @@
     'rs_vt_rank': (ctypes.c_int, [_vp, _c_int_p, _c_int_p]),
 }
 
-NEWER_SYMBOLS = {'rs_vt_prune_stats', 'rs_vt_prune_verified', 'rs_vt_create_metric', 'rs_vt_metric',
+NEWER_SYMBOLS = {'rs_vt_prune_stats', 'rs_vt_prune_verified', 'rs_vt_prune_scanned', 'rs_vt_create_metric', 'rs_vt_metric',
                  'rs_vt_offset_profile', 'rs_vt_offset_profile_host', 'rs_vt_set_normalise',
                  'rs_vt_normalise', 'rs_vt_normalise_host'}
 
diff --git a/pyratslam_amd/csrc/view_templates.hip b/pyratslam_amd/csrc/view_templates.hip
--- a/pyratslam_amd/csrc/view_templates.hip
+++ b/pyratslam_amd/csrc/view_templates.hip
@@ -8,6 +8,7 @@
 #include <cstdlib>
 #include <cstring>
 #include <memory>
+#include <type_traits>
 #include <vector>
 
 #include "rs_common.h"
@@ -116,6 +117,13 @@
     int64_t prunePairs = 0;
     int prunePasses = 0;
     int pruneNtb = 0;
+    int passes = 1;
+    int pruneMode = 0;
+    int pruneNq = 0;
+    rs::DevBuf<uint32_t> dUblk;
+    rs::DevBuf<unsigned> dCntPar;
+    vt_plan::ParityCounters cntPar;
+    rs::DevBuf<unsigned long long> dCountAcc;
     rs::DevBuf<int32_t> dPix;
     int64_t frameBytes = 0;
     rs::DevBuf<uint8_t> dFrames;
@@ -396,7 +404,7 @@
     int nq, nqc, rank, nranks;
 };
 template <int H, bool MATRIX, bool LIST>
-void vt_launch_plane_scan(rs_vt* h, const PlaneScan& s, const ScanOut& out, const PlaneList& list) {
+void vt_launch_plane_scan(rs_vt* h, const PlaneScan& s, const ScanOut& out, const PlaneListArg<LIST>& list) {
     hipLaunchKernelGGL((vt_scan_plane_kernel<H, MATRIX, LIST>), s.grid, dim3(64 * PL_CG * PL_SPLIT), 0, h->stream,
                        s.planes, s.ts, s.ntb, s.count, s.q.qp, s.q.qsum, s.nq, s.nqc, h->dCtr.get(), out, s.rank,
                        s.nranks, list);
@@ -413,6 +421,16 @@
         h->pruneCap = cap;
     }
     RS_TRY(h->dTbStar.reserve((size_t)nq));
+    RS_TRY(h->dUblk.reserve((size_t)nq));
+    if (vt_plan::parity_grows(h->cntPar, ntb)) {
+        vt_plan::ParityCounters grown = h->cntPar;
+        vt_plan::parity_grown(grown, ntb);
+        h->cntPar = vt_plan::ParityCounters{};
+        RS_TRY(h->dCntPar.reserve(2 * (size_t)grown.cap));
+        RS_HIP(hipMemsetAsync(h->dCntPar.get(), 0, sizeof(unsigned) * 2 * (size_t)grown.cap, h->stream));
+        grown.par = 0;
+        h->cntPar = grown;
+    }
     if (ntb > h->listCntCap) {
         const int cap = std::max(ntb, 2 * h->listCntCap);
         h->listCntCap = 0;
@@ -442,44 +460,60 @@
     unsigned* verified = h->dListCnt.get() + 2 * (size_t)h->listCntCap;
     int* list1 = h->dList.get();
     int* list2 = h->dList.get() + pairs;
+    const bool single = vt_plan::prune_passes(h->passes, ntb, nq) == 1;
+    FrontLists fl{};
+    if (single) {
+        const vt_plan::ParityCall pc = vt_plan::parity_begin(h->cntPar, ntb);
+        fl = FrontLists{h->dCntPar.get() + pc.mine, list1, h->dUblk.get(), h->dCntPar.get() + pc.other, pc.nzero};
+    }
     if (h->front == 2 || (h->front == 1 && vt_plan::front_fused(ntb, PF_WAVES * PF_TPW))) {
         const vt_plan::Grid2 fg = vt_plan::front_grid(nq, PF_NB, VT_PF_GRID_CAP);
         hipLaunchKernelGGL(vt_front_kernel, dim3((unsigned)fg.x, (unsigned)fg.y), dim3(64 * PF_WAVES), 0, h->stream,
                            s.planes, ntb, s.count, reinterpret_cast<const uint4*>(q.qc), q.qsj, nq, h->dMinLB.get(),
                            s.ts, reinterpret_cast<uint4*>(q.qp), q.qsum, out.best, s.rank, s.nranks,
-                           h->dTbStar.get());
+                           h->dTbStar.get(), fl);
     } else {
         const vt_plan::Grid2 pf = vt_plan::prefilter_grid(ntb, nq, PF_WAVES * PF_TPW, PF_NB, VT_PF_GRID_CAP);
         hipLaunchKernelGGL(vt_prefilter_kernel, dim3((unsigned)pf.x, (unsigned)pf.y), dim3(64 * PF_WAVES), 0,
                            h->stream, s.planes, ntb, s.count, reinterpret_cast<const uint4*>(q.qc), q.qsj, nq,
-                           h->dMinLB.get(), h->dSecond.get());
+                           h->dMinLB.get(), h->dSecond.get(), fl);
         hipLaunchKernelGGL(vt_prune_verify_kernel, dim3((unsigned)nq), dim3(64), 0, h->stream, h->dMinLB.get(),
                            h->dSecond.get(), ntb, nq, s.planes, s.ts, reinterpret_cast<const uint4*>(q.qc),
-                           reinterpret_cast<uint4*>(q.qp), q.qsum, out.best, s.rank, s.nranks, h->dTbStar.get());
-    }
-    const dim3 lgrid((unsigned)((nq + VT_LIST_T - 1) / VT_LIST_T), (unsigned)ntb);
-    hipLaunchKernelGGL(vt_prune_first_kernel, lgrid, dim3(VT_LIST_T), 0, h->stream, nq, h->dTbStar.get(), cnt1,
-                       list1, verified, cnt2, ntb);
+                           reinterpret_cast<uint4*>(q.qp), q.qsum, out.best, s.rank, s.nranks, h->dTbStar.get(), fl);
+    }
     ScanOut po = out;
     po.host = nullptr;
     po.done = nullptr;
     const uint32_t fill = (uint32_t)std::min(65535, std::max(1, h->planeSlots / ntb));
     const uint32_t lnb = (uint32_t)h->listNb;
-    vt_launch_plane_scan<64, false, true>(h, s, po,
-                                          PlaneList{list1, cnt1, nq, (uint32_t)VT_LIST_PER_B1, lnb, 1u, fill});
-    hipLaunchKernelGGL(vt_prune_rest_kernel, lgrid, dim3(VT_LIST_T), 0, h->stream, h->dMinLB.get(), nq,
-                       h->dTbStar.get(), out.best, cnt2, list2, cnt1, verified, ntb, h->dPruneStat.get());
 #ifdef VT_LIST_PER
     const int per2 = VT_LIST_PER;
 #else
     const int per2 = vt_plan::list_per(ntb, h->planeSlots);
 #endif
-    vt_launch_plane_scan<64, false, true>(h, s, po, PlaneList{list2, cnt2, nq, (uint32_t)per2, lnb, 0u, fill});
-    if (out.host) vt_launch_keys_export(h, out.best, nq, out.host, vt_plan::VT_EXPORT_BLOCKS);
-    RS_HIP(hipGetLastError());
     h->prunePairs = (int64_t)pairs;
     h->prunePasses = 2;
     h->pruneNtb = ntb;
+    h->pruneNq = nq;
+    h->pruneMode = single ? 1 : 2;
+    if (single) {
+        const uint32_t fill1 = (uint32_t)vt_plan::single_pass_fill((int)fill);
+        vt_launch_plane_scan<64, false, true>(
+            h, s, po, PlaneListU{{list1, fl.cnt, nq, (uint32_t)per2, lnb, 0u, fill1}, h->dTbStar.get(), h->dUblk.get()});
+        if (out.host) vt_launch_keys_export(h, out.best, nq, out.host, vt_plan::VT_EXPORT_BLOCKS);
+        RS_HIP(hipGetLastError());
+        return RS_OK;
+    }
+    const dim3 lgrid((unsigned)((nq + VT_LIST_T - 1) / VT_LIST_T), (unsigned)ntb);
+    hipLaunchKernelGGL(vt_prune_first_kernel, lgrid, dim3(VT_LIST_T), 0, h->stream, nq, h->dTbStar.get(), cnt1,
+                       list1, verified, cnt2, ntb);
+    vt_launch_plane_scan<64, false, true>(h, s, po,
+                                          PlaneListU{{list1, cnt1, nq, (uint32_t)VT_LIST_PER_B1, lnb, 1u, fill}});
+    hipLaunchKernelGGL(vt_prune_rest_kernel, lgrid, dim3(VT_LIST_T), 0, h->stream, h->dMinLB.get(), nq,
+                       h->dTbStar.get(), out.best, cnt2, list2, cnt1, verified, ntb, h->dPruneStat.get());
+    vt_launch_plane_scan<64, false, true>(h, s, po, PlaneListU{{list2, cnt2, nq, (uint32_t)per2, lnb, 0u, fill}});
+    if (out.host) vt_launch_keys_export(h, out.best, nq, out.host, vt_plan::VT_EXPORT_BLOCKS);
+    RS_HIP(hipGetLastError());
     return RS_OK;
 }
 
@@ -941,6 +975,10 @@
     if (h->planar && h->H == 64) {
         RS_TRY(vt_env_switch("RS_VT_PRUNE", &h->prune));
         RS_TRY(vt_env_switch("RS_VT_FRONT", &h->front));
+        if (const char* ps = std::getenv("RS_VT_PASSES"); ps && ps[0]) {
+            RS_CHECK((ps[0] == '1' || ps[0] == '2') && ps[1] == 0, RS_ERR_ARG, "RS_VT_PASSES='%s': expected 1 or 2", ps);
+            h->passes = ps[0] - '0';
+        }
         if (const char* nb = std::getenv("RS_VT_LIST_NB"); nb && nb[0]) {
             RS_CHECK((nb[0] == '1' || nb[0] == '2' || nb[0] == '4') && nb[1] == 0, RS_ERR_ARG,
                      "RS_VT_LIST_NB='%s': expected 1, 2 or 4", nb);
@@ -1310,12 +1348,35 @@
     return "carry";
 }
 
+namespace {
+int vt_prune_count(rs_vt* h, unsigned long long acc[2]) {
+    if (!h->dCountAcc.get()) RS_TRY(h->dCountAcc.reserve(2));
+    RS_HIP(hipMemsetAsync(h->dCountAcc.get(), 0, 2 * sizeof(unsigned long long), h->stream));
+    hipLaunchKernelGGL(vt_prune_count_kernel, dim3((unsigned)((h->pruneNq + 255) / 256)), dim3(256), 0, h->stream,
+                       h->dMinLB.get(), h->pruneNq, h->pruneNtb, h->dTbStar.get(), h->dUblk.get(),
+                       h->dCountAcc.get());
+    RS_HIP(hipGetLastError());
+    RS_HIP(hipMemcpyAsync(acc, h->dCountAcc.get(), 2 * sizeof(unsigned long long), hipMemcpyDeviceToHost, h->stream));
+    RS_HIP(hipStreamSynchronize(h->stream));
+    return RS_OK;
+}
+}
+
 int rs_vt_prune_stats(rs_vt* h, int64_t out[4]) {
     rs::clear_error();
     RS_CHECK(h && out, RS_ERR_ARG, "null argument");
     out[0] = out[1] = out[2] = out[3] = 0;
     if (h->prunePasses == 0) return RS_OK;
     RS_HIP(hipSetDevice(h->device));
+    out[2] = h->prunePairs;
+    out[3] = h->prunePasses;
+    if (h->pruneMode == 1) {
+        unsigned long long acc[2] = {0ull, 0ull};
+        RS_TRY(vt_prune_count(h, acc));
+        out[0] = h->pruneNq;
+        out[1] = (int64_t)acc[0];
+        return RS_OK;
+    }
     unsigned long long s0 = 0ull;
     std::vector<unsigned> c2((size_t)h->pruneNtb);
     RS_HIP(hipMemcpyAsync(&s0, h->dPruneStat.get(), sizeof(s0), hipMemcpyDeviceToHost, h->stream));
@@ -1324,17 +1385,44 @@
     RS_HIP(hipStreamSynchronize(h->stream));
     out[0] = (int64_t)s0;
     for (const unsigned c : c2) out[1] += (int64_t)c;
-    out[2] = h->prunePairs;
-    out[3] = h->prunePasses;
-    return RS_OK;
-}
-
-int rs_vt_prune_verified(rs_vt* h, int64_t* out) {
+    return RS_OK;
+}
+
+int rs_vt_prune_scanned(rs_vt* h, int64_t* out) {
     rs::clear_error();
     RS_CHECK(h && out, RS_ERR_ARG, "null argument");
     *out = 0;
     if (h->prunePasses == 0) return RS_OK;
     RS_HIP(hipSetDevice(h->device));
+    if (h->pruneMode == 1) {
+        std::vector<unsigned> c((size_t)h->pruneNtb);
+        RS_HIP(hipMemcpyAsync(c.data(), h->dCntPar.get() + vt_plan::parity_last_offset(h->cntPar),
+                              sizeof(unsigned) * c.size(), hipMemcpyDeviceToHost, h->stream));
+        RS_HIP(hipStreamSynchronize(h->stream));
+        for (const unsigned n : c) *out += (int64_t)n;
+        return RS_OK;
+    }
+    int64_t st[4];
+    unsigned long long v = 0ull;
+    RS_TRY(rs_vt_prune_stats(h, st));
+    RS_HIP(hipMemcpyAsync(&v, h->dPruneStat.get() + 2, sizeof(v), hipMemcpyDeviceToHost, h->stream));
+    RS_HIP(hipStreamSynchronize(h->stream));
+    *out = st[0] - (int64_t)v + st[1];
+    return RS_OK;
+}
+
+int rs_vt_prune_verified(rs_vt* h, int64_t* out) {
+    rs::clear_error();
+    RS_CHECK(h && out, RS_ERR_ARG, "null argument");
+    *out = 0;
+    if (h->prunePasses == 0) return RS_OK;
+    RS_HIP(hipSetDevice(h->device));
+    if (h->pruneMode == 1) {
+        unsigned long long acc[2] = {0ull, 0ull};
+        RS_TRY(vt_prune_count(h, acc));
+        *out = (int64_t)acc[1];
+        return RS_OK;
+    }
     unsigned long long v = 0ull;
     RS_HIP(hipMemcpyAsync(&v, h->dPruneStat.get() + 2, sizeof(v), hipMemcpyDeviceToHost, h->stream));
     RS_HIP(hipStreamSynchronize(h->stream));
diff --git a/pyratslam_amd/csrc/vt_plan.h b/pyratslam_amd/csrc/vt_plan.h
--- a/pyratslam_amd/csrc/vt_plan.h
+++ b/pyratslam_amd/csrc/vt_plan.h
@@ -94,6 +94,38 @@
            (prune == 2 || (prune == 1 && nq >= VT_PRUNE_MIN_Q && ntb >= 2));
 }
 
+inline int prune_passes(int passes_switch, int , int ) { return passes_switch == 2 ? 2 : 1; }
+#ifndef VT_SINGLE_ROUNDS
+#define VT_SINGLE_ROUNDS 4
+#endif
+inline int single_pass_fill(int fill) { return std::min(65535, VT_SINGLE_ROUNDS * std::max(1, fill)); }
+struct ParityCounters {
+    int cap = 0;
+    int par = 0;
+    int used[2] = {0, 0};
+    int last = -1;
+};
+struct ParityCall {
+    size_t mine, other;
+    int nzero;
+};
+inline bool parity_grows(const ParityCounters& s, int ntb) { return ntb > s.cap; }
+inline void parity_grown(ParityCounters& s, int ntb) {
+    s.cap = std::max(ntb, 2 * s.cap);
+    s.used[0] = s.used[1] = 0;
+    s.last = -1;
+}
+inline ParityCall parity_begin(ParityCounters& s, int ntb) {
+    const int p = s.par;
+    const ParityCall c{(size_t)p * (size_t)s.cap, (size_t)(p ^ 1) * (size_t)s.cap, s.used[p ^ 1]};
+    s.used[p ^ 1] = 0;
+    s.used[p] = ntb;
+    s.last = p;
+    s.par = p ^ 1;
+    return c;
+}
+inline size_t parity_last_offset(const ParityCounters& s) { return (size_t)s.last * (size_t)s.cap; }
+
 struct Grid2 {
     int x, y;
 };
diff --git a/pyratslam_amd/csrc/vt_plane_scan.h b/pyratslam_amd/csrc/vt_plane_scan.h
--- a/pyratslam_amd/csrc/vt_plane_scan.h
+++ b/pyratslam_amd/csrc/vt_plane_scan.h
@@ -153,6 +153,9 @@
 struct PlaneIds {
     int qc[PL_NB];
     int qnv;
+    const int* tbstar = nullptr;
+    uint32_t* ublk = nullptr;
+    int tb = 0;
 };
 __device__ __forceinline__ int plane_take(unsigned* __restrict__ ctr, const vt_plan::Take& tk, unsigned& failed) {
     if (!tk.takes) return tk.nbatch;
@@ -252,7 +255,17 @@
 #pragma unroll
         for (int x = 0; x < NO; ++x)
             best = min(best, vt_pl_ts[x][lane] + 256u * (pl_half(x) ? t[pl_slot(x)] >> 16 : t[pl_slot(x)] & 0xFFFFu));
-        emit_score<MATRIX>(out, slot, count, qi, LIST ? qi + 1 : nq, best - qsum[qi], rank, nranks, lane == 0);
+        if constexpr (LIST) {
+            const unsigned long long g = (unsigned long long)slot * nranks + rank;
+            const unsigned long long key =
+                wave_min_u64(slot < count ? (((unsigned long long)(best - qsum[qi]) << 32) | g) : NO_KEY);
+            if (lane == 0) {
+                atomicMin(out.best + qi, key);
+                if (pid.tbstar && pid.tbstar[qi] == pid.tb) pid.ublk[qi] = (uint32_t)(key >> 32);
+            }
+        } else {
+            emit_score<MATRIX>(out, slot, count, qi, nq, best - qsum[qi], rank, nranks, lane == 0);
+        }
     }
     if constexpr (LIST) {
 #pragma unroll
@@ -271,7 +284,8 @@
                                            unsigned* __restrict__ ctr, int G, int g, ScanOut out,
                                            int rank, int nranks, int wave, int cg, int lane,
                                            unsigned& failed, const int* __restrict__ ids,
-                                           const vt_plan::Take& tk, int v0, int w) {
+                                           const vt_plan::Take& tk, int v0, int w, const int* tbstar,
+                                           uint32_t* ublk) {
     using R = PlaneRange<H, HALF>;
     const int nbatch = tk.nbatch, tid = wave * 64 + lane;
     const int W = LIST ? w : PL_NB;
@@ -281,7 +295,7 @@
         (&vt_pl_part0[0][0][0])[i] = 0u;
         (&vt_pl_part1[0][0][0])[i] = 0u;
     }
-    PlaneIds pid{{0, 0, 0, 0}, 0};
+    PlaneIds pid{{0, 0, 0, 0}, 0, tbstar, ublk, tb};
     if constexpr (LIST) {
 #pragma unroll
         for (int e = 0; e < PL_NB; ++e) pid.qc[e] = __builtin_amdgcn_readlane(v0, vt_plan::spec_lane(W) + e);
@@ -339,6 +353,12 @@
     uint32_t fill : 16;
 };
 static_assert(sizeof(PlaneList) == 24, "the plane scan's kernel arguments keep their layout");
+struct PlaneListU : PlaneList {
+    const int* tbstar = nullptr;
+    uint32_t* ublk = nullptr;
+};
+template <bool LIST>
+using PlaneListArg = std::conditional_t<LIST, PlaneListU, PlaneList>;
 #ifdef VT_LIST_NB
 static_assert(VT_LIST_NB == 1 || VT_LIST_NB == 2 || VT_LIST_NB == 4, "entries per batch: 1, 2 or 4");
 #else
@@ -351,7 +371,7 @@
                           int ntb, int64_t count, const uint32_t* __restrict__ qp,
                           const uint32_t* __restrict__ qsum, int nq, int nqc,
                           unsigned* __restrict__ next_batch, ScanOut out, int rank, int nranks,
-                          PlaneList pl) {
+                          PlaneListArg<LIST> pl) {
     static_assert(PL_SPLIT == 2, "two row ranges");
     static_assert(!(LIST && MATRIX), "lists feed the key scan only");
     VT_STAMP_BEGIN();
@@ -381,13 +401,19 @@
     const int cg = wave % PL_CG, half = wave / PL_CG;
     unsigned failed = 0u;
     const uint4* qp4 = reinterpret_cast<const uint4*>(qp);
+    const int* tbstar = nullptr;
+    uint32_t* ublk = nullptr;
+    if constexpr (LIST) {
+        tbstar = pl.tbstar;
+        ublk = pl.ublk;
+    }
     if (tk.sb >= tk.nbatch) {
     } else if (half == 0)
         plane_wave<H, 0, MATRIX, LIST>(planes, tsum, tb, count, qp4, qsum, nq, ctr, G, g, out, rank, nranks,
-                                       wave, cg, lane, failed, ids, tk, v0, W);
+                                       wave, cg, lane, failed, ids, tk, v0, W, tbstar, ublk);
     else
         plane_wave<H, 1, MATRIX, LIST>(planes, tsum, tb, count, qp4, qsum, nq, ctr, G, g, out, rank, nranks,
-                                       wave, cg, lane, failed, ids, tk, v0, W);
+                                       wave, cg, lane, failed, ids, tk, v0, W, tbstar, ublk);
     if (threadIdx.x == 0 && tk.takes && failed == tk.last) *ctr = 0u;
     if constexpr (!MATRIX) {
         if (out.host) {
diff --git a/pyratslam_amd/csrc/vt_prune.h b/pyratslam_amd/csrc/vt_prune.h
--- a/pyratslam_amd/csrc/vt_prune.h
+++ b/pyratslam_amd/csrc/vt_prune.h
@@ -119,13 +119,26 @@
     }
 }
 
+struct FrontLists {
+    unsigned* cnt = nullptr;
+    int* list = nullptr;
+    uint32_t* ublk = nullptr;
+    unsigned* zero = nullptr;
+    int nzero = 0;
+};
+__device__ __forceinline__ void front_zero(const FrontLists& fl) {
+    if (blockIdx.x == 0 && blockIdx.y == 0)
+        for (int b = threadIdx.x; b < fl.nzero; b += blockDim.x) fl.zero[b] = 0u;
+}
+
 __global__ __launch_bounds__(64 * PF_WAVES) __attribute__((amdgpu_waves_per_eu(4)))
 void vt_prefilter_kernel(const uint4* __restrict__ planes, int ntb,
                                                                     int64_t count,
                                                                     const uint4* __restrict__ qc4,
                                                                     const uint32_t* __restrict__ qsj, int nq,
                                                                     uint32_t* __restrict__ minlb,
-                                                                    uint32_t* __restrict__ second) {
+                                                                    uint32_t* __restrict__ second, FrontLists fl) {
+    front_zero(fl);
     static_assert(PF_CGS % PF_CPS == 0 && PF_CGS >= 1 && PF_CGS <= PL_CG, "whole steps of column groups, of the unit");
     static_assert(PF_NU * PF_CGS * 32 * 255 < (int)PF_NONE, "a bound and a lane fit one word");
     __shared__ uint4 s_q[PF_NB][PF_NU][PF_CGS][PL_NO][2];
@@ -189,7 +202,8 @@
                                                 const uint4* __restrict__ qc4, uint4* __restrict__ qp4,
                                                 const uint32_t* __restrict__ qsum,
                                                 unsigned long long* __restrict__ best, int rank, int nranks,
-                                                int* __restrict__ tbstar, uint4* s_q, uint4* s_t) {
+                                                int* __restrict__ tbstar, uint4* s_q, uint4* s_t,
+                                                const uint32_t* minlb, int ntb, const FrontLists& fl) {
     constexpr int M = FAST_M, NU = 64 / 4, NS = PlaneLds<64>::NS, S0 = M - 3, S1 = 64 - M - 1;
     static_assert(PL_NO * PL_CG <= 64, "one lane per (offset, column group)");
     constexpr int QK = (QC_Q4 + 63) / 64;
@@ -260,6 +274,9 @@
     for (int off = 32; off > 0; off >>= 1) u0 = min(u0, (uint32_t)__shfl_xor(u0, off));
     u0 -= qs;
     const bool settled = (sec >> 6) > u0;
+    const bool lists = fl.cnt && (!settled || other <= u0);
+    uint32_t mlb0 = 0u;
+    if (lists && lane < ntb) mlb0 = minlb[(size_t)lane * nq + q];
     if (!settled || other <= u0) {
 #pragma unroll
         for (int k = 0; k < (VT_VQ4 + 63) / 64; ++k) {
@@ -270,10 +287,21 @@
             }
         }
     }
+    if (lists) {
+        asm volatile("" : "+v"(mlb0));
+        for (int tb = lane; tb < ntb; tb += 64) {
+            const bool in = tb == tbs ? !settled : (tb < 64 ? mlb0 : minlb[(size_t)tb * nq + q]) <= u0;
+            if (in) {
+                const unsigned p = atomicAdd(fl.cnt + tb, 1u);
+                if (p < (unsigned)nq) fl.list[(size_t)tb * nq + p] = q;
+            }
+        }
+    }
     if (lane == 0) {
         if (settled) {
             const unsigned long long g = ((unsigned long long)tbs * 64 + tl) * nranks + rank;
             atomicMin(best + q, ((unsigned long long)u0 << 32) | g);
+            if (fl.cnt) fl.ublk[q] = u0;
         }
         tbstar[q] = settled ? ~tbs : tbs;
     }
@@ -287,7 +315,8 @@
                                                              uint4* __restrict__ qp4,
                                                              const uint32_t* __restrict__ qsum,
                                                              unsigned long long* __restrict__ best, int rank,
-                                                             int nranks, int* __restrict__ tbstar) {
+                                                             int nranks, int* __restrict__ tbstar,
+                                                             FrontLists fl) {
     __shared__ uint4 s_q[VT_VQS];
     __shared__ uint4 s_t[VT_VTS];
     const int q = blockIdx.x, lane = threadIdx.x;
@@ -300,7 +329,7 @@
             pk = lt ? k : pk;
             sec = lt ? s2 : sec;
         }
-    }, nq, planes, tsum, qc4, qp4, qsum, best, rank, nranks, tbstar, s_q, s_t);
+    }, nq, planes, tsum, qc4, qp4, qsum, best, rank, nranks, tbstar, s_q, s_t, minlb, ntb, fl);
 }
 
 __global__ __launch_bounds__(64 * PF_WAVES) __attribute__((amdgpu_waves_per_eu(4)))
@@ -308,7 +337,8 @@
                      const uint32_t* __restrict__ qsj, int nq, uint32_t* __restrict__ minlb,
                      const uint32_t* __restrict__ tsum, uint4* __restrict__ qp4,
                      const uint32_t* __restrict__ qsum, unsigned long long* __restrict__ best, int rank,
-                     int nranks, int* __restrict__ tbstar) {
+                     int nranks, int* __restrict__ tbstar, FrontLists fl) {
+    front_zero(fl);
     constexpr int CH = PF_WAVES * PF_TPW;
     static_assert(PF_WAVES == PF_NB, "one wave per query of the group in the tail");
     static_assert(CH <= 64, "one lane per block of a chunk");
@@ -365,7 +395,7 @@
                 pk_ = pk;
                 sec_ = sec;
                 m2_ = m2;
-            }, nq, planes, tsum, qc4, qp4, qsum, best, rank, nranks, tbstar, s_vq[wave], s_vt[wave]);
+            }, nq, planes, tsum, qc4, qp4, qsum, best, rank, nranks, tbstar, s_vq[wave], s_vt[wave], minlb, ntb, fl);
     }
 }
 
@@ -417,6 +447,26 @@
     }
 }
 
+__global__ __launch_bounds__(256) void vt_prune_count_kernel(const uint32_t* __restrict__ minlb, int nq, int ntb,
+                                                             const int* __restrict__ tbstar,
+                                                             const uint32_t* __restrict__ ublk,
+                                                             unsigned long long* __restrict__ acc) {
+    __shared__ unsigned s_acc[2];
+    if (threadIdx.x < 2) s_acc[threadIdx.x] = 0u;
+    __syncthreads();
+    const int q = blockIdx.x * 256 + threadIdx.x;
+    if (q < nq) {
+        const int ts = tbstar[q], tbs = ts < 0 ? ~ts : ts;
+        const uint32_t u = ublk[q];
+        unsigned n = 0u;
+        for (int tb = 0; tb < ntb; ++tb) n += tb != tbs && minlb[(size_t)tb * nq + q] <= u;
+        if (n) atomicAdd(&s_acc[0], n);
+        if (ts < 0) atomicAdd(&s_acc[1], 1u);
+    }
+    __syncthreads();
+    if (threadIdx.x < 2 && s_acc[threadIdx.x]) atomicAdd(acc + threadIdx.x, (unsigned long long)s_acc[threadIdx.x]);
+}
+
 __global__ __launch_bounds__(256) void vt_keys_export(unsigned long long* __restrict__ keys, int n,
                                                       unsigned long long* host) {
     for (int i = blockIdx.x * 256 + threadIdx.x; i < n; i += gridDim.x * 256) {
diff --git a/pyratslam_amd/view_templates.py b/pyratslam_amd/view_templates.py
--- a/pyratslam_amd/view_templates.py
+++ b/pyratslam_amd/view_templates.py
@@ -721,6 +721,11 @@
         _lib.check(self._lib.rs_vt_prune_verified(self._h, ctypes.byref(out)))
         return int(out.value)
 
+    def prune_scanned(self):
+        out = ctypes.c_int64(0)
+        _lib.check(self._lib.rs_vt_prune_scanned(self._h, ctypes.byref(out)))
+        return int(out.value)
+
 
 class ShardedViewTemplates(ViewTemplates):
     _resident_ok = False
```

Result: faster. 32.42 billion compares/s, median of 6 (+9.1%).
